# roysubhankar/dwt-domain-adaptation

Measured on NVIDIA H100. Metric: ResNet-50-DWT images/sec fwd+bwd, higher is better.
Workload: dtype f32

## Files before the change

dwt-domain-adaptation_b200/dwt_b200/_native.py:

```python
from __future__ import annotations

import ctypes
import os
import threading

import torch

_HERE = os.path.dirname(os.path.abspath(__file__))
LIB_PATH = os.environ.get("DWT_B200_LIB") or os.path.join(_HERE, "lib", "libdwt_b200.so")

ABI_VERSION = 6
MAX_DOMAINS = 4
MAX_GROUP_SIZE = 64
MODE_TRAIN, MODE_EVAL = 0, 1
EPI_NONE, EPI_AFFINE, EPI_RELU, EPI_RESIDUAL = 0, 1, 2, 4
LAYOUT_NHWC = 0x100
STATUS_NOT_PD, STATUS_BAD_LABEL = 1, 2
KIND_WHITEN, KIND_BN = 0, 1

_c_float_p = ctypes.c_void_p
_PtrArray = ctypes.c_void_p * MAX_DOMAINS


class TailSite(ctypes.Structure):
    _fields_ = [("x", ctypes.c_void_p), ("eps", ctypes.c_float), ("momentum", ctypes.c_float),
                ("update_running", ctypes.c_int), ("running_mean", ctypes.POINTER(ctypes.c_void_p)),
                ("running_cov", ctypes.POINTER(ctypes.c_void_p)), ("gamma", ctypes.c_void_p), ("beta", ctypes.c_void_p),
                ("save_mean", ctypes.c_void_p), ("save_w", ctypes.c_void_p), ("dx", ctypes.c_void_p),
                ("dgamma", ctypes.c_void_p), ("dbeta", ctypes.c_void_p)]

_SIGNATURES = {
    "dwt_abi_version": (ctypes.c_int, []),
    "dwt_last_error": (ctypes.c_char_p, []),
    "dwt_workspace_bytes": (ctypes.c_size_t, [ctypes.c_int64, ctypes.c_int64, ctypes.c_int64, ctypes.c_int, ctypes.c_int]),
    "dwt_whiten_fwd": (ctypes.c_int, [_c_float_p, _c_float_p, ctypes.c_int64, ctypes.c_int64, ctypes.c_int64,
                                      ctypes.c_int, ctypes.c_int, ctypes.c_int, ctypes.c_float, ctypes.c_float,
                                      ctypes.c_int, ctypes.POINTER(ctypes.c_void_p), ctypes.POINTER(ctypes.c_void_p),
                                      _c_float_p, _c_float_p, _c_float_p, ctypes.c_void_p, ctypes.c_int, _c_float_p,
                                      _c_float_p, ctypes.c_void_p, ctypes.c_size_t, ctypes.c_void_p]),
    "dwt_whiten_bwd": (ctypes.c_int, [_c_float_p, _c_float_p, _c_float_p, _c_float_p, ctypes.c_int64, ctypes.c_int64,
                                      ctypes.c_int64, ctypes.c_int, ctypes.c_int, ctypes.c_int, ctypes.c_float,
                                      _c_float_p, _c_float_p, _c_float_p, _c_float_p, ctypes.c_void_p, _c_float_p,
                                      ctypes.c_int, _c_float_p, _c_float_p, ctypes.c_void_p, ctypes.c_size_t,
                                      ctypes.c_void_p]),
    "dwt_bn_fwd": (ctypes.c_int, [_c_float_p, _c_float_p, ctypes.c_int64, ctypes.c_int64, ctypes.c_int64,
                                  ctypes.c_int, ctypes.c_int, ctypes.c_float, ctypes.c_float, ctypes.c_int,
                                  ctypes.POINTER(ctypes.c_void_p), ctypes.POINTER(ctypes.c_void_p), _c_float_p,
                                  _c_float_p, _c_float_p, ctypes.c_void_p, ctypes.c_int, _c_float_p, _c_float_p,
                                  ctypes.c_void_p, ctypes.c_size_t, ctypes.c_void_p]),
    "dwt_bn_bwd": (ctypes.c_int, [_c_float_p, _c_float_p, _c_float_p, _c_float_p, ctypes.c_int64, ctypes.c_int64, ctypes.c_int64,
                                  ctypes.c_int, ctypes.c_int, _c_float_p, _c_float_p, _c_float_p, _c_float_p,
                                  ctypes.c_void_p, _c_float_p, ctypes.c_int, _c_float_p, _c_float_p, ctypes.c_void_p,
                                  ctypes.c_size_t, ctypes.c_void_p]),
    "dwt_tail2_fwd": (ctypes.c_int, [ctypes.c_int, ctypes.POINTER(TailSite), _c_float_p, ctypes.c_void_p, ctypes.c_int64,
                                     ctypes.c_int64, ctypes.c_int64, ctypes.c_int, ctypes.c_int, ctypes.c_void_p,
                                     ctypes.c_size_t, ctypes.c_void_p]),
    "dwt_tail2_bwd": (ctypes.c_int, [ctypes.c_int, ctypes.POINTER(TailSite), _c_float_p, _c_float_p, ctypes.c_void_p,
                                     _c_float_p, ctypes.c_int64, ctypes.c_int64, ctypes.c_int64, ctypes.c_int, ctypes.c_int,
                                     ctypes.c_void_p, ctypes.c_size_t, ctypes.c_void_p]),
    "dwt_mec_fwd_bwd": (ctypes.c_int, [_c_float_p, _c_float_p, ctypes.c_int64, ctypes.c_int64, _c_float_p,
                                       _c_float_p, _c_float_p, ctypes.c_void_p]),
    "dwt_head_loss_fwd_bwd": (ctypes.c_int, [_c_float_p, ctypes.c_void_p, ctypes.c_int64, ctypes.c_int64, ctypes.c_float,
                                             _c_float_p, _c_float_p, ctypes.c_void_p, ctypes.c_void_p]),
    "dwt_augment_pair": (ctypes.c_int, [ctypes.c_void_p, ctypes.c_int64, ctypes.c_int, ctypes.c_int, ctypes.c_int,
                                        ctypes.c_void_p, ctypes.c_void_p, ctypes.c_void_p, _c_float_p,
                                        ctypes.POINTER(ctypes.c_float), ctypes.POINTER(ctypes.c_float), _c_float_p,
                                        _c_float_p, ctypes.c_int, ctypes.c_void_p]),
    "dwt_maxpool_fwd": (ctypes.c_int, [_c_float_p, _c_float_p, ctypes.c_void_p, ctypes.c_int64, ctypes.c_int64, ctypes.c_int64,
                                       ctypes.c_int64, ctypes.c_int, ctypes.c_int, ctypes.c_int, ctypes.c_void_p]),
    "dwt_maxpool_bwd": (ctypes.c_int, [_c_float_p, ctypes.c_void_p, _c_float_p, ctypes.c_int64, ctypes.c_int64, ctypes.c_int64,
                                       ctypes.c_int64, ctypes.c_int, ctypes.c_int, ctypes.c_int, ctypes.c_void_p]),
    "dwt_launch_count": (ctypes.c_int64, []),
    "dwt_profile_begin": (None, []),
    "dwt_profile_end": (ctypes.c_int, [ctypes.c_void_p, ctypes.c_int]),
}


class ProfileEntry(ctypes.Structure):
    _fields_ = [("name", ctypes.c_char * 48), ("launches", ctypes.c_int64), ("ms", ctypes.c_double),
                ("bytes", ctypes.c_double)]


def profile_begin():
    lib().dwt_profile_begin()


def profile_end():
    cap = 1024
    buf = (ProfileEntry * cap)()
    k = lib().dwt_profile_end(ctypes.cast(buf, ctypes.c_void_p), cap)
    return {buf[i].name.decode(): dict(launches=buf[i].launches, ms=buf[i].ms, bytes=buf[i].bytes) for i in range(k)}


def by_family(prof):
    out = {}
    for name, v in prof.items():
        f = out.setdefault(name.split("|")[0], dict(launches=0, ms=0.0, bytes=0.0))
        for k in f:
            f[k] += v[k]
    return out


def launch_count() -> int:
    return int(lib().dwt_launch_count())
EXPORTS = tuple(_SIGNATURES)

_lib = None
_lock = threading.Lock()


class NativeError(RuntimeError):
    pass


def lib() -> ctypes.CDLL:
    global _lib
    if _lib is None:
        with _lock:
            if _lib is None:
                if not os.path.exists(LIB_PATH):
                    raise NativeError(
                        f"{LIB_PATH} is missing: build it with `python {os.path.join(_HERE, 'build.py')}` "
                        "(dwt_b200 has no CPU or PyTorch fallback)")
                handle = ctypes.CDLL(LIB_PATH)
                for name, (res, args) in _SIGNATURES.items():
                    fn = getattr(handle, name)
                    fn.restype, fn.argtypes = res, args
                if handle.dwt_abi_version() != ABI_VERSION:
                    raise NativeError("libdwt_b200.so ABI version mismatch; rebuild it")
                _lib = handle
    return _lib


def channels_last_supported(channels: int, group_size: int) -> bool:
    if group_size not in (1, 2, 4) or channels % 4:
        return False
    c4 = channels // 4
    return c4 & (c4 - 1) == 0


def check(rc: int) -> None:
    if rc != 0:
        raise NativeError(f"libdwt_b200 error {rc}: {lib().dwt_last_error().decode()}")


def ptr(t):
    return None if t is None else ctypes.c_void_p(t.data_ptr())


def ptr_array(tensors):
    arr = _PtrArray()
    for i, t in enumerate(tensors):
        arr[i] = None if t is None else t.data_ptr()
    return ctypes.cast(arr, ctypes.POINTER(ctypes.c_void_p))


def require_cuda(*tensors, any_dtype=False) -> torch.device:
    dev = None
    for t in tensors:
        if t is None:
            continue
        if not t.is_cuda:
            raise NativeError("dwt_b200 runs on CUDA tensors only (no CPU fallback); got a tensor on " + str(t.device))
        if t.dtype != torch.float32 and not any_dtype:
            raise NativeError("dwt_b200 computes in float32; got " + str(t.dtype))
        if dev is None:
            dev = t.device
        elif t.device != dev:
            raise NativeError(f"tensors on different devices: {dev} vs {t.device}")
    return dev


def stream_ptr(device) -> ctypes.c_void_p:
    return ctypes.c_void_p(torch.cuda.current_stream(device).cuda_stream)


_workspaces: dict = {}


def workspace(device, n, c, hw, gs, nd):
    need = lib().dwt_workspace_bytes(n, c, hw, gs, nd)
    if need == 0:
        raise NativeError(f"invalid geometry for workspace: C={c} group_size={gs} domains={nd}")
    key = (device.index, torch.cuda.current_stream(device).cuda_stream)
    buf = _workspaces.get(key)
    if buf is None or buf.numel() < need:
        buf = torch.zeros(max(need, 8 << 20), dtype=torch.uint8, device=device)
        _workspaces[key] = buf
    return buf


def status(device=None) -> int:
    device = torch.device("cuda", torch.cuda.current_device()) if device is None else device
    buf = _workspaces.get((device.index, torch.cuda.current_stream(device).cuda_stream))
    return 0 if buf is None else int(buf[:4].view(torch.int32).item())


def status_all(device=None) -> int:
    device = torch.device("cuda", torch.cuda.current_device()) if device is None else device
    torch.cuda.synchronize(device)
    st = 0
    for (idx, _), buf in _workspaces.items():
        if idx == device.index:
            st |= int(buf[:4].view(torch.int32).item())
    return st


def status_ptr(device):
    return ctypes.c_void_p(workspace(device, 1, 4, 1, 1, 1).data_ptr())


def clear_status(device=None) -> None:
    device = torch.device("cuda", torch.cuda.current_device()) if device is None else device
    buf = _workspaces.get((device.index, torch.cuda.current_stream(device).cuda_stream))
    if buf is not None:
        buf[:4].zero_()


class NotPositiveDefiniteError(torch.linalg.LinAlgError):
    """What the reference's torch.cholesky raises at utils/whitening.py:53, raised late: the kernels never sync the
    host, so the failure is seen at the next poll (raise_on_status) or explicit check_status() call."""


_poll = {"every": 0, "count": 0}


def raise_on_status(every: int = 1) -> None:
    _poll["every"], _poll["count"] = max(0, int(every)), 0


def check_status(device=None) -> None:
    st = status(device)
    if st == 0:
        return
    clear_status(device)
    if st & STATUS_NOT_PD:
        raise NotPositiveDefiniteError(
            "cholesky: a whitening covariance was not positive definite (status word bit 0; the reference raises "
            "from torch.cholesky, utils/whitening.py:53); the affected group's output is NaN and its running-"
            "statistics update was skipped")
    if st & STATUS_BAD_LABEL:
        raise IndexError("head loss: a label was outside [0, num_classes) and is not ignore_index=-100 "
                         "(F.nll_loss asserts here); the row was dropped")
    raise NativeError(f"unknown status bits {st:#x}")


def poll_status(device) -> None:
    if _poll["every"]:
        _poll["count"] += 1
        if _poll["count"] >= _poll["every"]:
            _poll["count"] = 0
            check_status(device)
```

dwt-domain-adaptation_b200/dwt_b200/csrc/api.cu:

```cuda
#include <stdarg.h>
#include <stdio.h>
#include <stdlib.h>

#include <atomic>
#include <mutex>
#include <string>
#include <vector>
#include <string.h>

#include "norm_launch.h"

namespace {

thread_local char g_err[512] = "";

int fail(int code, const char* fmt, ...) {
  va_list ap;
  va_start(ap, fmt);
  vsnprintf(g_err, sizeof(g_err), fmt, ap);
  va_end(ap);
  return code;
}

int check_launch(const char* what) {
  cudaError_t e = cudaPeekAtLastError();
  if (e != cudaSuccess) {
    cudaGetLastError();
    return fail(DWT_E_LAUNCH, "%s: %s", what, cudaGetErrorString(e));
  }
  return DWT_OK;
}

int sm_count() {
  static int n = 0;
  if (n == 0) {
    int dev = 0;
    if (cudaGetDevice(&dev) != cudaSuccess ||
        cudaDeviceGetAttribute(&n, cudaDevAttrMultiProcessorCount, dev) != cudaSuccess || n <= 0)
      n = 132;
  }
  return n;
}

std::atomic<int64_t> g_launches{0};
std::mutex g_prof_mu;
bool g_prof_on = false;
struct ProfRec { char name[48]; cudaEvent_t a, b; double bytes; };
std::vector<ProfRec> g_prof;
std::vector<cudaEvent_t> g_event_pool;

cudaEvent_t take_event() {
  if (!g_event_pool.empty()) { cudaEvent_t e = g_event_pool.back(); g_event_pool.pop_back(); return e; }
  cudaEvent_t e = nullptr;
  cudaEventCreate(&e);
  return e;
}

struct Launch {
  cudaStream_t st; ProfRec rec; bool on;
  Launch(const char* family, const dwt::Geom* gm, double bytes, cudaStream_t s) : st(s), on(false) {
    rec.a = rec.b = nullptr; rec.bytes = bytes;
    if (gm) snprintf(rec.name, sizeof(rec.name), "%s|%d|%d|%d|%d|%d", family, gm->C, gm->HW, gm->GS, gm->D, gm->N);
    else snprintf(rec.name, sizeof(rec.name), "%s", family);
    g_launches.fetch_add(1, std::memory_order_relaxed);
    std::lock_guard<std::mutex> lk(g_prof_mu);
    if (g_prof_on && g_prof.size() < (1u << 18)) {
      on = true; rec.a = take_event(); rec.b = take_event();
      cudaEventRecord(rec.a, st);
    }
  }
  ~Launch() {
    if (!on) return;
    cudaEventRecord(rec.b, st);
    std::lock_guard<std::mutex> lk(g_prof_mu);
    g_prof.push_back(rec);
  }
};

std::once_flag g_tiled_once;
int g_tiled_rc = 0;
int ensure_tiled() {
  std::call_once(g_tiled_once, [] { g_tiled_rc = dwt::tiled_init(); });
  return g_tiled_rc;
}

std::once_flag g_tc_once;
int g_tc_rc = 0;
int ensure_tc() {
  std::call_once(g_tc_once, [] { g_tc_rc = dwt::tc_init(); });
  return g_tc_rc;
}

int tc_chunks(const dwt::Geom& g) {
  const int problems = dwt::tc_superblocks(g) * g.D;
  int n = 2 * sm_count() / problems;
  const int64_t tiles = (int64_t)g.N * ((g.HW + 31) / 32);
  if (n > tiles) n = (int)tiles;
  return n < 1 ? 1 : n;
}

int tc_apply_ctas(const dwt::Geom& g, int per_sm, int tile_px) {
  const int problems = dwt::tc_superblocks(g) * g.D;
  int n = per_sm * sm_count() / problems;
  const int64_t tiles = (int64_t)g.N * ((g.HW + tile_px - 1) / tile_px);
  if (n > tiles) n = (int)tiles;
  return n < 1 ? 1 : n;
}

int env_int(const char* name, int dflt) {
  const char* v = getenv(name);
  return (v && *v) ? atoi(v) : dflt;
}

struct ClPlan { int nred, new_, S, gridy, gz_red, gz_ew; };
ClPlan cl_plan(const dwt::Geom& g, int slots_red, int slots_ew, int unroll_red, int unroll_ew) {
  static const int seq_mb = env_int("DWT_CL_SEQ_MB", 1 << 30);
  const int C4 = g.C / 4, CW = C4 < 256 ? C4 : 256, rpi = 256 / CW, gridy = C4 / CW;
  const long long rows = (long long)g.N * g.HW;
  const double mbytes = 4.0 * (double)g.D * (double)rows * (double)g.C / 1048576.0;
  const bool seq = g.D > 1 && mbytes >= (double)seq_mb;
  ClPlan p;
  p.gridy = gridy;
  p.gz_red = p.gz_ew = seq ? 1 : g.D;
  auto shape = [&](int slots, int unroll, int gz) {
    long long by_work = rows / ((long long)rpi * unroll * 2);
    if (by_work < 1) by_work = 1;
    int cap = slots * sm_count() / (gridy * gz);
    if (cap < 1) cap = 1;
    return (int)(by_work < cap ? by_work : cap);
  };
  p.nred = shape(slots_red, unroll_red, p.gz_red);
  p.new_ = shape(slots_ew, unroll_ew, p.gz_ew);
  p.S = p.nred < 8 ? p.nred : 8;
  return p;
}

inline size_t align_up(size_t v, size_t a) { return (v + a - 1) / a * a; }

enum KernelKind { K_STATS, K_APPLY, K_BWD_REDUCE, K_BWD_APPLY };

int slots_per_sm(KernelKind k, int GS) {
  if (GS > 4) return 2;
  return ((k == K_STATS || k == K_APPLY) && GS < 4) ? 4 : 3;
}

int chunk_cap(int GS, int G, int D) {
  (void)GS;
  const int target = 16 * sm_count();
  int cap = (target + G * D - 1) / (G * D);
  return cap < 1 ? 1 : cap;
}

struct Workspace {
  int* status;
  int* counters;
  int* dom_counter;
  int* dom_counter2;
  float* partial;
  float* save_cov;
  float* coef;
  float* dgb_part;
  float* gram;
  float* shift;
  float* red;
  int* bad;
  size_t bytes;
};

constexpr size_t kMaxGroups = 65536;
constexpr size_t kOffCounters = 256;
constexpr size_t kOffDom1 = kOffCounters + sizeof(int) * DWT_MAX_DOMAINS * kMaxGroups;
constexpr size_t kOffDom2 = kOffDom1 + sizeof(int) * kMaxGroups;
constexpr size_t kOffScratch = kOffDom2 + sizeof(int) * kMaxGroups;

Workspace carve(void* base, int64_t C, int GS, int D, size_t start = kOffScratch) {
  const int G = (int)(C / GS);
  const int cap = chunk_cap(GS, G, D);
  size_t off = start;
  auto take = [&](size_t nbytes) { size_t o = off; off = align_up(off + nbytes, 256); return o; };
  char* b = static_cast<char*>(base);
  Workspace w;
  w.status = reinterpret_cast<int*>(b);
  w.counters = reinterpret_cast<int*>(b + kOffCounters);
  w.dom_counter = reinterpret_cast<int*>(b + kOffDom1);
  w.dom_counter2 = reinterpret_cast<int*>(b + kOffDom2);
  size_t partial_floats = (size_t)D * G * cap * (GS * GS + GS);
  if (GS >= 8 && 64 % GS == 0) {
    const size_t tc = ((size_t)2 * sm_count() + (size_t)((C + 63) / 64) * D) * (64 * 64 + 64);
    if (tc > partial_floats) partial_floats = tc;
  }
  size_t red_floats = 1;
  if (dwt::cl_supports((int)C, GS)) {
    const size_t W = (size_t)dwt::cl_bwd_width((int)C, GS);
    const int C4 = (int)C / 4, gridy = C4 <= 256 ? 1 : C4 / 256;
    const size_t cl = (size_t)D * (3 * sm_count() / gridy + 1) * W;
    if (cl > partial_floats) partial_floats = cl;
    red_floats = (size_t)D * 8 * W;
  }
  w.partial = reinterpret_cast<float*>(b + take(sizeof(float) * partial_floats));
  w.red = reinterpret_cast<float*>(b + take(sizeof(float) * red_floats));
  w.save_cov = reinterpret_cast<float*>(b + take(sizeof(float) * (size_t)D * G * GS * GS));
  w.coef = reinterpret_cast<float*>(b + take(sizeof(float) * (size_t)D * G * dwt::coef_stride(GS)));
  w.dgb_part = reinterpret_cast<float*>(b + take(sizeof(float) * (size_t)D * 2 * C));
  const size_t SBn = (size_t)((C + 63) / 64);
  w.gram = reinterpret_cast<float*>(b + take(sizeof(float) * (size_t)D * SBn * (64 * 64 + 64)));
  w.shift = reinterpret_cast<float*>(b + take(sizeof(float) * (size_t)D * SBn * 64));
  w.bad = reinterpret_cast<int*>(b + take(sizeof(int) * (size_t)D * G));
  w.bytes = off;
  return w;
}

struct Plan {
  dwt::Geom gm;
  dwt::Geom gm_ew;
  int vec;
  int chunks_ew;
  bool small;
};

void shape(dwt::Geom& g, int64_t work_units, KernelKind kind, bool small, int* chunks) {
  const bool reduce = (kind == K_STATS || kind == K_BWD_REDUCE);
  const int slots = slots_per_sm(kind, g.GS) * sm_count();
  const int target = reduce ? slots : 4 * slots;
  g.ppc = 1;
  if (small) {
    while (g.ppc < 8 && (int64_t)((g.G + g.ppc - 1) / g.ppc) * g.D > target) g.ppc <<= 1;
  }
  int n = 1;
  if (g.ppc == 1) {
    n = target / (g.G * g.D);
    const int cap = chunk_cap(g.GS, g.G, g.D);
    if (n > cap) n = cap;
    if (n > work_units) n = (int)work_units;
    if (n < 1) n = 1;
  }
  *chunks = n;
}

int make_plan(Plan& p, KernelKind reduce_kind, KernelKind ew_kind, const void* a0, const void* a1, const void* a2,
              int64_t N, int64_t C, int64_t HW, int GS, int D) {
  if (N <= 0 || C <= 0 || HW <= 0) return fail(DWT_E_INVALID, "empty tensor (N=%lld C=%lld HW=%lld)", (long long)N,
                                               (long long)C, (long long)HW);
  if (GS < 1 || GS > DWT_MAX_GROUP_SIZE) return fail(DWT_E_UNSUPPORTED, "group_size %d outside [1,%d]", GS,
                                                     DWT_MAX_GROUP_SIZE);
  if (C % GS != 0) return fail(DWT_E_INVALID, "channels %lld not divisible by group_size %d", (long long)C, GS);
  if (D < 1 || D > DWT_MAX_DOMAINS) return fail(DWT_E_INVALID, "n_domains %d outside [1,%d]", D, DWT_MAX_DOMAINS);
  if (N * C * HW >= (int64_t)1 << 31 || C / GS > 65535)
    return fail(DWT_E_UNSUPPORTED, "shape too large for 32-bit item indexing");
  dwt::Geom& g = p.gm;
  g.N = (int)N; g.C = (int)C; g.HW = (int)HW; g.GS = GS; g.G = (int)(C / GS); g.D = D;
  g.M = (float)((double)N * (double)HW);
  const uintptr_t bits = (uintptr_t)a0 | (uintptr_t)a1 | (uintptr_t)a2;
  p.vec = (HW % 4 == 0 && bits % 16 == 0) ? 4 : 1;
  p.small = dwt::small_supports(GS);
  int64_t work_units;
  if (p.small) work_units = (N * (HW / p.vec) + dwt::kThreads * 2 - 1) / (dwt::kThreads * 2);
  else work_units = (N * HW + 127) / 128;
  if (work_units < 1) work_units = 1;
  shape(g, work_units, reduce_kind, p.small, &g.nchunks);
  p.gm_ew = g;
  shape(p.gm_ew, work_units, ew_kind, p.small, &p.chunks_ew);
  p.gm_ew.nchunks = g.nchunks;
  return DWT_OK;
}

int check_running(bool need_running, float* const* rmean, float* const* rcov, int D) {
  if (!need_running) return DWT_OK;
  if (!rmean || !rcov) return fail(DWT_E_INVALID, "running buffers required");
  for (int d = 0; d < D; ++d)
    if (!rmean[d] || !rcov[d]) return fail(DWT_E_INVALID, "running buffer of domain %d is null", d);
  return DWT_OK;
}

dwt::FwdFin make_fwd_fin(float a, float b, float momentum, float unbias, int update_running, bool need_running,
                         float* const* rmean, float* const* rcov, float* save_mean, float* save_w, const Workspace& w, int D) {
  dwt::FwdFin fin{};
  fin.a = a; fin.b = b; fin.momentum = momentum; fin.unbias = unbias;
  fin.update_running = update_running;
  fin.save_mean = save_mean; fin.save_w = save_w; fin.save_cov = w.save_cov;
  for (int d = 0; d < D; ++d) { fin.rmean[d] = need_running ? rmean[d] : nullptr; fin.rcov[d] = need_running ? rcov[d] : nullptr; }
  fin.dom_counter = w.dom_counter; fin.status = w.status; fin.bad = w.bad;
  if (need_running && D > 1) {
    bool all_same = true, all_distinct = true;
    for (int d = 1; d < D; ++d) {
      if (rmean[d] != rmean[0] || rcov[d] != rcov[0]) all_same = false;
      for (int e = 0; e < d; ++e)
        if (rmean[d] == rmean[e] || rcov[d] == rcov[e]) all_distinct = false;
    }
    fin.aliased = all_same ? 1 : (all_distinct ? 0 : -1);
  }
  return fin;
}

dwt::BwdFin make_bwd_fin(float a, int mode, int epi, const float* save_mean, const float* save_w, const float* gamma,
                         float* dgamma, float* dbeta, const Workspace& w) {
  dwt::BwdFin fin{};
  fin.a = a; fin.mode = mode; fin.epi = epi;
  fin.save_mean = save_mean; fin.save_w = save_w; fin.gamma = gamma;
  fin.coef = w.coef; fin.dgb_part = w.dgb_part;
  fin.dgamma = (epi & DWT_EPI_AFFINE) ? dgamma : nullptr;
  fin.dbeta = (epi & DWT_EPI_AFFINE) ? dbeta : nullptr;
  fin.dom_counter = w.dom_counter2;
  return fin;
}

int whiten_like_fwd(const float* x, float* y, int64_t N, int64_t C, int64_t HW, int GS, int D, int mode, float a,
                    float b, float momentum, float unbias, int update_running, float* const* rmean,
                    float* const* rcov, const float* gamma, const float* beta, const float* residual,
                    uint8_t* relu_mask, int epi, float* save_mean, float* save_w, void* ws, size_t ws_bytes,
                    cudaStream_t st) {
  const bool nhwc = (mode & DWT_LAYOUT_NHWC) != 0;
  mode &= 0xFF;
  Plan p;
  if (int rc = make_plan(p, K_STATS, K_APPLY, x, y, nullptr, N, C, HW, GS, D)) return rc;
  if (!x || !y || !save_mean || !save_w || !ws) return fail(DWT_E_INVALID, "null pointer argument");
  if (nhwc && !dwt::cl_supports((int)C, GS))
    return fail(DWT_E_UNSUPPORTED, "channels-last layout is built for group_size 1, 2, 4 with C/4 a power of two (C=%lld gs=%d)", (long long)C, GS);
  if (nhwc && (((uintptr_t)x | (uintptr_t)y) % 16 != 0)) return fail(DWT_E_INVALID, "channels-last tensors must be 16-byte aligned");
  if (mode != DWT_MODE_TRAIN && mode != DWT_MODE_EVAL) return fail(DWT_E_INVALID, "bad mode %d", mode);
  if ((epi & DWT_EPI_RELU) && !(epi & DWT_EPI_AFFINE)) return fail(DWT_E_INVALID, "RELU epilogue needs AFFINE");
  if ((epi & DWT_EPI_AFFINE) && (!gamma || !beta)) return fail(DWT_E_INVALID, "AFFINE epilogue needs gamma and beta");
  if ((epi & DWT_EPI_RESIDUAL) && ((epi & 3) != 3 || !residual)) return fail(DWT_E_INVALID, "RESIDUAL epilogue needs AFFINE|RELU and a residual tensor");
  if ((epi & DWT_EPI_RESIDUAL) && (uintptr_t)residual % 16 != 0) return fail(DWT_E_INVALID, "residual must be 16-byte aligned");
  if (relu_mask && !((epi & DWT_EPI_RESIDUAL) && nhwc))
    return fail(DWT_E_UNSUPPORTED, "the ReLU byte map is written by the channels-last RESIDUAL epilogue only");
  if (epi != 0 && !p.small)
    return fail(DWT_E_UNSUPPORTED, "fused gamma/beta/ReLU epilogue is built for group_size 1, 2, 4 (got %d)", GS);
  const bool need_running = (mode == DWT_MODE_EVAL) || update_running;
  if (int rc = check_running(need_running, rmean, rcov, D)) return rc;
  Workspace w = carve(ws, C, GS, D);
  if (w.bytes > ws_bytes) return fail(DWT_E_WORKSPACE, "workspace too small: need %zu bytes, got %zu", w.bytes, ws_bytes);
  if ((uintptr_t)ws % 256 != 0) return fail(DWT_E_WORKSPACE, "workspace must be 256-byte aligned");
  if (!p.small && ensure_tiled() != 0) return fail(DWT_E_LAUNCH, "cudaFuncSetAttribute failed (%d)", g_tiled_rc);

  const dwt::FwdFin fin = make_fwd_fin(a, b, momentum, unbias, mode == DWT_MODE_TRAIN ? update_running : 0, need_running,
                                       rmean, rcov, save_mean, save_w, w, D);

  const double E = 4.0 * (double)D * (double)N * (double)C * (double)HW;
  if (nhwc) {
    const ClPlan cp = cl_plan(p.gm, 3, 3, 8, (epi & DWT_EPI_RESIDUAL) ? 4 : 8);
    if (mode == DWT_MODE_TRAIN) {
      {
        Launch l("cl_stats", &p.gm, E, st);
        dwt::cl_stats(x, p.gm, cp.nred, cp.gz_red, w.partial, w.shift, st);
      }
      if (int rc = check_launch("channels-last statistics kernel")) return rc;
      Launch l("cl_fwd_finalize", &p.gm, 0.0, st);
      dwt::cl_fwd_finalize(w.partial, cp.nred, w.shift, p.gm, fin, st);
    } else {
      Launch l("eval_prep", &p.gm, 0.0, st);
      dwt::small_eval_prep(p.gm, fin, st);
    }
    if (int rc = check_launch("channels-last finalize kernel")) return rc;
    {
      Launch l("cl_apply", &p.gm, ((epi & DWT_EPI_RESIDUAL) ? (relu_mask ? 3.0625 : 3.0) : 2.0) * E, st);
      dwt::cl_apply(x, y, p.gm, cp.new_, cp.gz_ew, epi, save_mean, save_w, gamma, beta, residual, relu_mask, st);
    }
    return check_launch("channels-last apply kernel");
  }
  const bool tc = !p.small && dwt::tc_supports(p.gm, p.vec) && ensure_tc() == 0;
  if (mode == DWT_MODE_TRAIN) {
    Launch l(p.small ? "small_stats" : (tc ? "tc_stats" : "tiled_stats"), &p.gm, E, st);
    if (p.small) dwt::small_stats(x, p.gm, p.vec, fin, w.partial, w.counters, st);
    else if (tc) {
      if (int cr = dwt::tc_stats(x, p.gm, tc_chunks(p.gm), w.shift, w.partial, st))
        return fail(DWT_E_LAUNCH, "cuTensorMapEncodeTiled failed (CUresult %d) x=%p N=%d C=%d HW=%d D=%d", cr, (const void*)x, p.gm.N, p.gm.C, p.gm.HW, p.gm.D);
    } else dwt::tiled_stats(x, p.gm, p.vec, fin, w.partial, w.counters, st);
  } else {
    Launch l("eval_prep", &p.gm, 0.0, st);
    if (p.small) dwt::small_eval_prep(p.gm, fin, st);
    else if (tc) dwt::dense_fwd_factor(nullptr, nullptr, p.gm, fin, st);
    else dwt::tiled_eval_prep(p.gm, fin, st);
  }
  if (tc && mode == DWT_MODE_TRAIN) {
    if (int rc = check_launch("tensor-core statistics kernel")) return rc;
    Launch l("dense_fwd_finalize", &p.gm, 0.0, st);
    dwt::dense_partial_reduce(w.partial, tc_chunks(p.gm), dwt::tc_superblocks(p.gm) * D, w.gram, st);
    dwt::dense_fwd_factor(w.gram, w.shift, p.gm, fin, st);
  }
  if (int rc = check_launch("whitening statistics kernel")) return rc;
  {
    Launch l(p.small ? "small_apply" : (tc ? "tc_apply" : "tiled_apply"), &p.gm, ((epi & DWT_EPI_RESIDUAL) ? 3 : 2) * E, st);
    if (p.small) dwt::small_apply(x, y, p.gm_ew, p.vec, p.chunks_ew, epi, save_mean, save_w, gamma, beta, residual, st);
    else if (tc) {
      if (int cr = dwt::tc_apply(x, y, p.gm, tc_apply_ctas(p.gm, 1, 64), save_mean, save_w, st))
        return fail(DWT_E_LAUNCH, "cuTensorMapEncodeTiled failed (CUresult %d)", cr);
    } else dwt::tiled_apply(x, y, p.gm_ew, p.vec, p.chunks_ew, save_mean, save_w, st);
  }
  return check_launch("whitening apply kernel");
}

int whiten_like_bwd(const float* x, const float* dout, const float* dout2, float* dx, int64_t N, int64_t C, int64_t HW, int GS, int D,
                    int mode, float a, const float* save_mean, const float* save_w, const float* gamma,
                    const float* beta, const uint8_t* relu_mask, float* dresidual, int epi, float* dgamma,
                    float* dbeta, void* ws, size_t ws_bytes, cudaStream_t st) {
  const bool nhwc = (mode & DWT_LAYOUT_NHWC) != 0;
  mode &= 0xFF;
  Plan p;
  if (int rc = make_plan(p, K_BWD_REDUCE, K_BWD_APPLY, x, dout, dx, N, C, HW, GS, D)) return rc;
  if (!x || !dout || !dx || !save_mean || !save_w || !ws) return fail(DWT_E_INVALID, "null pointer argument");
  if (dout2 && (!nhwc || (uintptr_t)dout2 % 16 != 0))
    return fail(nhwc ? DWT_E_INVALID : DWT_E_UNSUPPORTED, "a second gradient addend (dout2) is built for the channels-last "
                "kernels (16-byte aligned tensor); add it to dout otherwise");
  if (nhwc && !dwt::cl_supports((int)C, GS))
    return fail(DWT_E_UNSUPPORTED, "channels-last layout is built for group_size 1, 2, 4 with C/4 a power of two (C=%lld gs=%d)", (long long)C, GS);
  if (nhwc && (((uintptr_t)x | (uintptr_t)dout | (uintptr_t)dx) % 16 != 0)) return fail(DWT_E_INVALID, "channels-last tensors must be 16-byte aligned");
  if (mode != DWT_MODE_TRAIN && mode != DWT_MODE_EVAL) return fail(DWT_E_INVALID, "bad mode %d", mode);
  if ((epi & DWT_EPI_RELU) && !(epi & DWT_EPI_AFFINE)) return fail(DWT_E_INVALID, "RELU epilogue needs AFFINE");
  if ((epi & DWT_EPI_AFFINE) && (!gamma || !beta)) return fail(DWT_E_INVALID, "AFFINE epilogue needs gamma and beta");
  if (epi & DWT_EPI_RESIDUAL) {
    if (!nhwc || !relu_mask || (epi & 3) != 3 || !dresidual)
      return fail(DWT_E_INVALID, "backward of a RESIDUAL forward needs the channels-last layout, AFFINE|RELU, the forward's "
                                 "ReLU byte map and dresidual (or pass dout already masked by (out > 0) with epilogue AFFINE)");
    if ((uintptr_t)dresidual % 16 != 0) return fail(DWT_E_INVALID, "dresidual must be 16-byte aligned");
  } else if (relu_mask || dresidual) {
    return fail(DWT_E_INVALID, "relu_mask / dresidual belong to the RESIDUAL epilogue");
  }
  if ((dgamma == nullptr) != (dbeta == nullptr)) return fail(DWT_E_INVALID, "dgamma and dbeta go together");
  if (epi != 0 && !p.small)
    return fail(DWT_E_UNSUPPORTED, "fused gamma/beta/ReLU epilogue is built for group_size 1, 2, 4 (got %d)", GS);
  Workspace w = carve(ws, C, GS, D);
  if (w.bytes > ws_bytes) return fail(DWT_E_WORKSPACE, "workspace too small: need %zu bytes, got %zu", w.bytes, ws_bytes);
  if ((uintptr_t)ws % 256 != 0) return fail(DWT_E_WORKSPACE, "workspace must be 256-byte aligned");
  if (!p.small && ensure_tiled() != 0) return fail(DWT_E_LAUNCH, "cudaFuncSetAttribute failed (%d)", g_tiled_rc);

  const dwt::BwdFin fin = make_bwd_fin(a, mode, epi, save_mean, save_w, gamma, dgamma, dbeta, w);
  const bool masked = nhwc && (epi & DWT_EPI_RESIDUAL) != 0;

  const bool need_reduce = (mode == DWT_MODE_TRAIN) || (fin.dgamma != nullptr) || masked;
  const double E = 4.0 * (double)D * (double)N * (double)C * (double)HW;
  if (nhwc) {
    const ClPlan cp = cl_plan(p.gm, 2, 2, 4, 4);
    if (need_reduce) {
      {
        Launch l("cl_bwd_reduce", &p.gm, ((masked ? 3.0625 : 2.0) + (dout2 ? 1.0 : 0.0)) * E, st);
        dwt::cl_bwd_reduce(x, dout, dout2, p.gm, cp.nred, cp.gz_red, epi, save_mean, save_w, gamma, beta, relu_mask, dresidual, w.partial, st);
      }
      if (int rc = check_launch("channels-last backward reduction kernel")) return rc;
      Launch l("cl_bwd_finalize", &p.gm, 0.0, st);
      dwt::cl_bwd_finalize(w.partial, cp.nred, p.gm, fin, st);
    } else {
      Launch l("bwd_prep", &p.gm, 0.0, st);
      dwt::small_bwd_prep(p.gm, fin, st);
    }
    if (int rc = check_launch("channels-last backward finalize kernel")) return rc;
    {
      Launch l("cl_bwd_apply", &p.gm, (3.0 + (dout2 && !masked ? 1.0 : 0.0)) * E, st);
      if (masked) dwt::cl_bwd_apply(x, dresidual, nullptr, dx, p.gm, cp.new_, cp.gz_ew, DWT_EPI_AFFINE, w.coef, save_mean, save_w, gamma, beta, st);
      else dwt::cl_bwd_apply(x, dout, dout2, dx, p.gm, cp.new_, cp.gz_ew, epi, w.coef, save_mean, save_w, gamma, beta, st);
    }
    return check_launch("channels-last backward apply kernel");
  }
  const bool tc = !p.small && dwt::tc_supports(p.gm, p.vec) && ensure_tc() == 0;
  if (need_reduce) {
    Launch l(p.small ? "small_bwd_reduce" : (tc ? "tc_bwd_reduce" : "tiled_bwd_reduce"), &p.gm, 2 * E, st);
    if (p.small) dwt::small_bwd_reduce(x, dout, p.gm, p.vec, fin, beta, w.partial, w.counters, st);
    else if (tc) {
      if (int cr = dwt::tc_bwd_reduce(x, dout, p.gm, tc_chunks(p.gm), save_mean, w.partial, st))
        return fail(DWT_E_LAUNCH, "cuTensorMapEncodeTiled failed (CUresult %d) x=%p dout=%p N=%d C=%d HW=%d D=%d", cr, (const void*)x, (const void*)dout, p.gm.N, p.gm.C, p.gm.HW, p.gm.D);
    } else dwt::tiled_bwd_reduce(x, dout, p.gm, p.vec, fin, w.partial, w.counters, st);
  } else {
    Launch l("bwd_prep", &p.gm, 0.0, st);
    if (p.small) dwt::small_bwd_prep(p.gm, fin, st);
    else if (tc) dwt::dense_bwd_coef(nullptr, p.gm, fin, w.shift, st);
    else dwt::tiled_bwd_prep(p.gm, fin, st);
  }
  if (tc && need_reduce) {
    if (int rc = check_launch("tensor-core backward reduction kernel")) return rc;
    Launch l("dense_bwd_finalize", &p.gm, 0.0, st);
    dwt::dense_partial_reduce(w.partial, tc_chunks(p.gm), dwt::tc_superblocks(p.gm) * D, w.gram, st);
    dwt::dense_bwd_coef(w.gram, p.gm, fin, w.shift, st);
  }
  if (int rc = check_launch("whitening backward reduction kernel")) return rc;
  {
    Launch l(p.small ? "small_bwd_apply" : (tc ? "tc_bwd_apply" : "tiled_bwd_apply"), &p.gm, 3 * E, st);
    if (p.small) dwt::small_bwd_apply(x, dout, dx, p.gm_ew, p.vec, p.chunks_ew, epi, w.coef, save_mean, save_w, gamma, beta, st);
    else if (tc) {
      if (int cr = dwt::tc_bwd_apply(x, dout, dx, p.gm, tc_apply_ctas(p.gm, 1, 64), w.coef, save_mean, w.shift, st))
        return fail(DWT_E_LAUNCH, "cuTensorMapEncodeTiled failed (CUresult %d)", cr);
    } else dwt::tiled_bwd_apply(x, dout, dx, p.gm_ew, p.vec, p.chunks_ew, w.coef, st);
  }
  return check_launch("whitening backward apply kernel");
}

struct SiteConst { float a, b, unbias; };
SiteConst site_const(int kind, float eps, int64_t N, int64_t HW) {
  if (kind == DWT_KIND_BN) {
    const double M = (double)N * (double)HW;
    return {1.f, eps, M > 1.0 ? (float)(M / (M - 1.0)) : 1.f};
  }
  return {1.f - eps, eps, 1.f};
}

int tail2_plan(Plan& p, int kind, const dwt_tail_site* s, const void* out, int64_t N, int64_t C, int64_t HW, int GS, int D) {
  if (kind != DWT_KIND_WHITEN && kind != DWT_KIND_BN) return fail(DWT_E_INVALID, "bad kind %d", kind);
  if (kind == DWT_KIND_BN && GS != 1) return fail(DWT_E_INVALID, "batch norm has group_size 1 (got %d)", GS);
  if (!s) return fail(DWT_E_INVALID, "null pointer argument");
  if (int rc = make_plan(p, K_STATS, K_APPLY, s[0].x, s[1].x, out, N, C, HW, GS, D)) return rc;
  if (!dwt::cl_supports((int)C, GS))
    return fail(DWT_E_UNSUPPORTED, "the two-site tail runs on the channels-last kernels: group_size 1, 2, 4 with C/4 a power of two (C=%lld gs=%d)",
                (long long)C, GS);
  for (int k = 0; k < 2; ++k)
    if (!s[k].x || !s[k].gamma || !s[k].beta || !s[k].save_mean || !s[k].save_w || !out) return fail(DWT_E_INVALID, "null pointer argument");
  if ((((uintptr_t)s[0].x | (uintptr_t)s[1].x | (uintptr_t)out) % 16) != 0) return fail(DWT_E_INVALID, "channels-last tensors must be 16-byte aligned");
  return DWT_OK;
}

int tail2_workspace(Workspace (&w)[2], void* ws, size_t ws_bytes, int64_t C, int GS, int D) {
  if (!ws) return fail(DWT_E_INVALID, "null pointer argument");
  w[0] = carve(ws, C, GS, D);
  w[1] = carve(ws, C, GS, D, w[0].bytes);
  if (w[1].bytes > ws_bytes) return fail(DWT_E_WORKSPACE, "workspace too small: need %zu bytes, got %zu", w[1].bytes, ws_bytes);
  if ((uintptr_t)ws % 256 != 0) return fail(DWT_E_WORKSPACE, "workspace must be 256-byte aligned");
  return DWT_OK;
}

int tail2_fwd(int kind, const dwt_tail_site* s, float* y, uint8_t* relu_mask, int64_t N, int64_t C, int64_t HW, int GS, int D,
              void* ws, size_t ws_bytes, cudaStream_t st) {
  Plan p;
  if (int rc = tail2_plan(p, kind, s, y, N, C, HW, GS, D)) return rc;
  if (!relu_mask) return fail(DWT_E_INVALID, "the two-site tail writes the ReLU byte map its backward reads");
  for (int k = 0; k < 2; ++k)
    if (int rc = check_running(s[k].update_running != 0, s[k].running_mean, s[k].running_cov, D)) return rc;
  Workspace w[2];
  if (int rc = tail2_workspace(w, ws, ws_bytes, C, GS, D)) return rc;
  dwt::FwdFin fin[2];
  for (int k = 0; k < 2; ++k) {
    const SiteConst sc = site_const(kind, s[k].eps, N, HW);
    fin[k] = make_fwd_fin(sc.a, sc.b, s[k].momentum, sc.unbias, s[k].update_running, s[k].update_running != 0, s[k].running_mean,
                          s[k].running_cov, s[k].save_mean, s[k].save_w, w[k], D);
  }
  const double E = 4.0 * (double)D * (double)N * (double)C * (double)HW;
  const ClPlan cp = cl_plan(p.gm, 3, 3, 8, 4);
  for (int k = 0; k < 2; ++k) {
    Launch l("cl_stats", &p.gm, E, st);
    dwt::cl_stats(s[k].x, p.gm, cp.nred, cp.gz_red, w[k].partial, w[k].shift, st);
  }
  if (int rc = check_launch("channels-last statistics kernel")) return rc;
  {
    Launch l("cl_tail2_fwd_finalize", &p.gm, 0.0, st);
    dwt::cl_fwd_finalize(w[0].partial, cp.nred, w[0].shift, p.gm, fin[0], st, &fin[1], (size_t)(w[1].partial - w[0].partial),
                         (size_t)(w[1].shift - w[0].shift));
  }
  if (int rc = check_launch("channels-last finalize kernel")) return rc;
  {
    Launch l("cl_tail2_apply", &p.gm, 3.0625 * E, st);
    dwt::cl_tail2_apply(s[0].x, s[1].x, y, p.gm, cp.new_, cp.gz_ew, s[0].save_mean, s[0].save_w, s[0].gamma, s[0].beta,
                        s[1].save_mean, s[1].save_w, s[1].gamma, s[1].beta, relu_mask, st);
  }
  return check_launch("channels-last two-site apply kernel");
}

int tail2_bwd(int kind, const dwt_tail_site* s, const float* dout, const float* dout2, const uint8_t* relu_mask, float* dz,
              int64_t N, int64_t C, int64_t HW, int GS, int D, void* ws, size_t ws_bytes, cudaStream_t st) {
  Plan p;
  if (int rc = tail2_plan(p, kind, s, dz, N, C, HW, GS, D)) return rc;
  if (!dout || !relu_mask || !s[0].dx || !s[1].dx) return fail(DWT_E_INVALID, "null pointer argument");
  if ((((uintptr_t)dout | (uintptr_t)dout2 | (uintptr_t)s[0].dx | (uintptr_t)s[1].dx) % 16) != 0)
    return fail(DWT_E_INVALID, "channels-last tensors must be 16-byte aligned");
  for (int k = 0; k < 2; ++k)
    if ((s[k].dgamma == nullptr) != (s[k].dbeta == nullptr)) return fail(DWT_E_INVALID, "dgamma and dbeta go together");
  Workspace w[2];
  if (int rc = tail2_workspace(w, ws, ws_bytes, C, GS, D)) return rc;
  dwt::BwdFin fin[2];
  for (int k = 0; k < 2; ++k)
    fin[k] = make_bwd_fin(site_const(kind, s[k].eps, N, HW).a, DWT_MODE_TRAIN, k ? DWT_EPI_AFFINE : (DWT_EPI_AFFINE | DWT_EPI_RELU | DWT_EPI_RESIDUAL),
                          s[k].save_mean, s[k].save_w, s[k].gamma, s[k].dgamma, s[k].dbeta, w[k]);
  const double E = 4.0 * (double)D * (double)N * (double)C * (double)HW;
  const ClPlan cp = cl_plan(p.gm, 2, 2, 4, 4);
  {
    Launch l("cl_tail2_bwd_reduce", &p.gm, (4.0625 + (dout2 ? 1.0 : 0.0)) * E, st);
    dwt::cl_tail2_bwd_reduce(s[0].x, s[1].x, dout, dout2, p.gm, cp.nred, cp.gz_red, s[0].save_mean, s[1].save_mean, relu_mask, dz,
                             w[0].partial, (size_t)(w[1].partial - w[0].partial), st);
  }
  if (int rc = check_launch("channels-last two-site backward reduction kernel")) return rc;
  {
    Launch l("cl_tail2_bwd_finalize", &p.gm, 0.0, st);
    dwt::cl_bwd_finalize(w[0].partial, cp.nred, p.gm, fin[0], st, &fin[1], (size_t)(w[1].partial - w[0].partial));
  }
  if (int rc = check_launch("channels-last backward finalize kernel")) return rc;
  {
    Launch l("cl_tail2_bwd_apply", &p.gm, 5.0 * E, st);
    dwt::cl_tail2_bwd_apply(s[0].x, s[1].x, dz, s[0].dx, s[1].dx, p.gm, cp.new_, cp.gz_ew, w[0].coef, w[1].coef, st);
  }
  return check_launch("channels-last two-site backward apply kernel");
}

}

extern "C" {

int dwt_abi_version(void) { return DWT_B200_ABI_VERSION; }

const char* dwt_last_error(void) { return g_err; }

size_t dwt_workspace_bytes(int64_t N, int64_t C, int64_t HW, int group_size, int n_domains) {
  (void)N; (void)HW;
  if (C <= 0 || group_size < 1 || group_size > DWT_MAX_GROUP_SIZE || C % group_size != 0 || n_domains < 1 ||
      n_domains > DWT_MAX_DOMAINS)
    return 0;
  return carve(nullptr, C, group_size, n_domains, carve(nullptr, C, group_size, n_domains).bytes).bytes;
}

int dwt_whiten_fwd(const float* x, float* y, int64_t N, int64_t C, int64_t HW, int group_size, int n_domains,
                   int mode, float eps, float momentum, int update_running, float* const* running_mean,
                   float* const* running_cov, const float* gamma, const float* beta, const float* residual,
                   uint8_t* relu_mask, int epilogue, float* save_mean, float* save_w, void* workspace,
                   size_t workspace_bytes, dwt_stream_t stream) {
  return whiten_like_fwd(x, y, N, C, HW, group_size, n_domains, mode, 1.f - eps, eps, momentum, 1.f, update_running,
                         running_mean, running_cov, gamma, beta, residual, relu_mask, epilogue, save_mean, save_w,
                         workspace, workspace_bytes, (cudaStream_t)stream);
}

int dwt_whiten_bwd(const float* x, const float* dout, const float* dout2, float* dx, int64_t N, int64_t C, int64_t HW, int group_size,
                   int n_domains, int mode, float eps, const float* save_mean, const float* save_w,
                   const float* gamma, const float* beta, const uint8_t* relu_mask, float* dresidual, int epilogue,
                   float* dgamma, float* dbeta, void* workspace, size_t workspace_bytes, dwt_stream_t stream) {
  return whiten_like_bwd(x, dout, dout2, dx, N, C, HW, group_size, n_domains, mode, 1.f - eps, save_mean, save_w, gamma,
                         beta, relu_mask, dresidual, epilogue, dgamma, dbeta, workspace, workspace_bytes,
                         (cudaStream_t)stream);
}

int dwt_bn_fwd(const float* x, float* y, int64_t N, int64_t C, int64_t HW, int n_domains, int mode, float eps,
               float factor, int update_running, float* const* running_mean, float* const* running_var,
               const float* weight, const float* bias, const float* residual, uint8_t* relu_mask, int epilogue,
               float* save_mean, float* save_invstd, void* workspace, size_t workspace_bytes, dwt_stream_t stream) {
  const double M = (double)N * (double)HW;
  const float unbias = M > 1.0 ? (float)(M / (M - 1.0)) : 1.f;
  return whiten_like_fwd(x, y, N, C, HW, 1, n_domains, mode, 1.f, eps, factor, unbias, update_running, running_mean,
                         running_var, weight, bias, residual, relu_mask, epilogue, save_mean, save_invstd, workspace,
                         workspace_bytes, (cudaStream_t)stream);
}

int dwt_bn_bwd(const float* x, const float* dout, const float* dout2, float* dx, int64_t N, int64_t C, int64_t HW, int n_domains,
               int mode, const float* save_mean, const float* save_invstd, const float* weight, const float* bias,
               const uint8_t* relu_mask, float* dresidual, int epilogue, float* dweight, float* dbias, void* workspace,
               size_t workspace_bytes, dwt_stream_t stream) {
  return whiten_like_bwd(x, dout, dout2, dx, N, C, HW, 1, n_domains, mode, 1.f, save_mean, save_invstd, weight, bias,
                         relu_mask, dresidual, epilogue, dweight, dbias, workspace, workspace_bytes,
                         (cudaStream_t)stream);
}

int dwt_tail2_fwd(int kind, const dwt_tail_site* sites, float* y, uint8_t* relu_mask, int64_t N, int64_t C, int64_t HW,
                  int group_size, int n_domains, void* workspace, size_t workspace_bytes, dwt_stream_t stream) {
  return tail2_fwd(kind, sites, y, relu_mask, N, C, HW, group_size, n_domains, workspace, workspace_bytes, (cudaStream_t)stream);
}

int dwt_tail2_bwd(int kind, const dwt_tail_site* sites, const float* dout, const float* dout2, const uint8_t* relu_mask, float* dz,
                  int64_t N, int64_t C, int64_t HW, int group_size, int n_domains, void* workspace, size_t workspace_bytes,
                  dwt_stream_t stream) {
  return tail2_bwd(kind, sites, dout, dout2, relu_mask, dz, N, C, HW, group_size, n_domains, workspace, workspace_bytes,
                   (cudaStream_t)stream);
}

int dwt_mec_fwd_bwd(const float* x, const float* y, int64_t N, int64_t K, float* loss, float* gx, float* gy,
                    dwt_stream_t stream) {
  if (!x || !y || !loss || !gx || !gy) return fail(DWT_E_INVALID, "null pointer argument");
  if (N <= 0 || K <= 0 || N >= (1 << 24) || K >= (1 << 24)) return fail(DWT_E_INVALID, "bad logits shape [%lld,%lld]", (long long)N, (long long)K);
  {
    Launch l("mec", nullptr, 16.0 * (double)N * (double)K, (cudaStream_t)stream);
    dwt::mec_launch(x, y, (int)N, (int)K, loss, gx, gy, (cudaStream_t)stream);
  }
  return check_launch("MEC kernel");
}

int dwt_head_loss_fwd_bwd(const float* logits, const int64_t* labels, int64_t B, int64_t K, float lambda, float* losses,
                          float* grad, int* status, dwt_stream_t stream) {
  if (!logits || !labels || !losses || !grad) return fail(DWT_E_INVALID, "null pointer argument");
  if (B <= 0 || K <= 0 || B >= (1 << 22) || K >= (1 << 24)) return fail(DWT_E_INVALID, "bad logits shape [3*%lld,%lld]", (long long)B, (long long)K);
  {
    Launch l("head_loss", nullptr, 4.0 * 3 * (double)B * (double)K * 2, (cudaStream_t)stream);
    dwt::head_loss_launch(logits, reinterpret_cast<const long long*>(labels), (int)B, (int)K, lambda, losses, grad, status,
                          (cudaStream_t)stream);
  }
  return check_launch("head loss kernel");
}

int dwt_augment_pair(const uint8_t* images, int64_t B, int src_h, int src_w, int crop, const int32_t* crop_plain,
                     const int32_t* crop_aug, const uint8_t* flip, const float* affine, const float* mean,
                     const float* stdv, float* out_plain, float* out_aug, int layout, dwt_stream_t stream) {
  if (!images || !mean || !stdv) return fail(DWT_E_INVALID, "null pointer argument");
  if (!out_plain && !out_aug) return fail(DWT_E_INVALID, "at least one of out_plain / out_aug is needed");
  if (out_plain && !crop_plain) return fail(DWT_E_INVALID, "out_plain needs crop_plain");
  if (out_aug && (!crop_aug || !flip || !affine)) return fail(DWT_E_INVALID, "out_aug needs crop_aug, flip and affine");
  if (B <= 0 || B > 65535 || src_h <= 0 || src_w <= 0 || src_h > 16384 || src_w > 16384)
    return fail(DWT_E_INVALID, "bad image batch [%lld,%d,%d,3]", (long long)B, src_h, src_w);
  if (crop <= 0 || crop > src_h || crop > src_w) return fail(DWT_E_INVALID, "crop %d does not fit %dx%d", crop, src_h, src_w);
  if (layout != 0 && layout != DWT_LAYOUT_NHWC) return fail(DWT_E_INVALID, "layout must be 0 (NCHW) or DWT_LAYOUT_NHWC");
  for (int c = 0; c < 3; ++c)
    if (!(stdv[c] != 0.f)) return fail(DWT_E_INVALID, "std[%d] must be non-zero", c);
  {
    const double px = (double)B * crop * crop;
    Launch l("augment_pair", nullptr, px * 3 * ((out_plain ? 5.0 : 0.0) + (out_aug ? 5.0 : 0.0)), (cudaStream_t)stream);
    dwt::augment_pair_launch(images, (int)B, src_h, src_w, crop, crop_plain, crop_aug, flip, affine, mean, stdv, out_plain,
                             out_aug, layout != 0, (cudaStream_t)stream);
  }
  return check_launch("augmentation kernel");
}

namespace {
int pool_check(int64_t N, int64_t H, int64_t W, int64_t C, int k, int s, int p, int* OH, int* OW) {
  if (N <= 0 || H <= 0 || W <= 0 || C <= 0 || C % 4 != 0) return fail(DWT_E_INVALID, "bad pooling input [%lld,%lld,%lld,%lld] (C must be a multiple of 4)", (long long)N, (long long)H, (long long)W, (long long)C);
  if (k < 1 || k > 15 || s < 1 || p < 0 || 2 * p > k) return fail(DWT_E_INVALID, "bad pooling window k=%d s=%d p=%d (k <= 15, pad <= k/2)", k, s, p);
  if (H + 2 * p < k || W + 2 * p < k) return fail(DWT_E_INVALID, "pooling window larger than the padded image");
  *OH = (int)((H + 2 * p - k) / s + 1);
  *OW = (int)((W + 2 * p - k) / s + 1);
  if (N * H * W * C >= ((int64_t)1 << 40)) return fail(DWT_E_UNSUPPORTED, "tensor too large");
  return DWT_OK;
}
}

int dwt_maxpool_fwd(const float* x, float* y, uint8_t* argmax, int64_t N, int64_t H, int64_t W, int64_t C, int kernel,
                    int stride, int padding, dwt_stream_t stream) {
  int OH = 0, OW = 0;
  if (int rc = pool_check(N, H, W, C, kernel, stride, padding, &OH, &OW)) return rc;
  if (!x || !y || !argmax) return fail(DWT_E_INVALID, "null pointer argument");
  if ((((uintptr_t)x | (uintptr_t)y) % 16) != 0 || (uintptr_t)argmax % 4 != 0) return fail(DWT_E_INVALID, "pooling tensors must be 16-byte aligned");
  {
    const double in = (double)N * H * W * C, out = (double)N * OH * OW * C;
    Launch l("maxpool_fwd", nullptr, 4.0 * (in + out) + out, (cudaStream_t)stream);
    dwt::maxpool_fwd_launch(x, y, argmax, (int)N, (int)H, (int)W, (int)C, OH, OW, kernel, stride, padding, (cudaStream_t)stream);
  }
  return check_launch("max-pool forward kernel");
}

int dwt_maxpool_bwd(const float* dy, const uint8_t* argmax, float* dx, int64_t N, int64_t H, int64_t W, int64_t C, int kernel,
                    int stride, int padding, dwt_stream_t stream) {
  int OH = 0, OW = 0;
  if (int rc = pool_check(N, H, W, C, kernel, stride, padding, &OH, &OW)) return rc;
  if (!dy || !dx || !argmax) return fail(DWT_E_INVALID, "null pointer argument");
  if ((((uintptr_t)dy | (uintptr_t)dx) % 16) != 0 || (uintptr_t)argmax % 4 != 0) return fail(DWT_E_INVALID, "pooling tensors must be 16-byte aligned");
  {
    const double in = (double)N * H * W * C, out = (double)N * OH * OW * C;
    Launch l("maxpool_bwd", nullptr, 4.0 * (in + out) + out, (cudaStream_t)stream);
    dwt::maxpool_bwd_launch(dy, argmax, dx, (int)N, (int)H, (int)W, (int)C, OH, OW, kernel, stride, padding, (cudaStream_t)stream);
  }
  return check_launch("max-pool backward kernel");
}

int64_t dwt_launch_count(void) { return g_launches.load(); }

void dwt_profile_begin(void) {
  std::lock_guard<std::mutex> lk(g_prof_mu);
  for (auto& r : g_prof) { g_event_pool.push_back(r.a); g_event_pool.push_back(r.b); }
  g_prof.clear();
  g_prof_on = true;
}

int dwt_profile_end(dwt_profile_entry* out, int max_entries) {
  std::vector<ProfRec> recs;
  {
    std::lock_guard<std::mutex> lk(g_prof_mu);
    g_prof_on = false;
    recs.swap(g_prof);
  }
  int n = 0;
  for (auto& r : recs) {
    float ms = 0.f;
    if (cudaEventSynchronize(r.b) == cudaSuccess && cudaEventElapsedTime(&ms, r.a, r.b) == cudaSuccess) {
      int k = 0;
      for (; k < n; ++k)
        if (strcmp(out[k].name, r.name) == 0) break;
      if (k == n && n < max_entries) {
        memset(&out[n], 0, sizeof(out[n]));
        strncpy(out[n].name, r.name, sizeof(out[n].name) - 1);
        ++n;
      }
      if (k < n) { out[k].launches += 1; out[k].ms += ms; out[k].bytes += r.bytes; }
    }
    std::lock_guard<std::mutex> lk(g_prof_mu);
    g_event_pool.push_back(r.a); g_event_pool.push_back(r.b);
  }
  return n;
}

}
```

dwt-domain-adaptation_b200/dwt_b200/csrc/norm_cl.cu:

```cuda
#include <stdlib.h>

#include "dwt_common.cuh"
#include "norm_launch.h"
#include "small_algebra.cuh"

namespace dwt {
namespace {

constexpr int kT = 256;

__device__ __forceinline__ void pdl_wait() { asm volatile("griddepcontrol.wait;" ::: "memory"); }
__device__ __forceinline__ void pdl_launch_dependents() { asm volatile("griddepcontrol.launch_dependents;" ::: "memory"); }

template <int GS> struct ClShape {
  static constexpr int NSUB = 4 / GS;
  static constexpr int NM = GS * (GS + 1) / 2;
  static constexpr int FWD1 = GS + NM;
  static constexpr int BWD1 = GS * GS + GS;
  static constexpr int FWD = NSUB * FWD1;
  static constexpr int BWD = NSUB * BWD1;
};

struct ClThread {
  int C4, CW, rpi, col, rsub, q;
  __device__ __forceinline__ ClThread(const Geom& gm) {
    C4 = gm.C >> 2;
    CW = C4 < kT ? C4 : kT;
    rpi = kT / CW;
    col = threadIdx.x % CW;
    rsub = threadIdx.x / CW;
    q = blockIdx.y * CW + col;
  }
};

template <int UNROLL, bool DESC, class F>
__device__ __forceinline__ void sweep_rows(const ClThread& t, unsigned rows, F&& body) {
  const unsigned krows = (unsigned)t.rpi * UNROLL, nch = (rows + krows - 1) / krows;
  for (unsigned i = blockIdx.x; i < nch; i += gridDim.x) body((DESC ? nch - 1 - i : i) * krows + t.rsub);
}
#define CL_FOR_DOMAINS(d, gm, DESC) \
  for (int di_ = blockIdx.z, d = (DESC) ? (gm).D - 1 - di_ : di_; di_ < (gm).D; di_ += gridDim.z, d = (DESC) ? (gm).D - 1 - di_ : di_)

__device__ __forceinline__ float4 ldg4(const float* p) { return __ldg(reinterpret_cast<const float4*>(p)); }

template <int NACC>
__device__ __forceinline__ void column_reduce(const ClThread& t, float (&acc)[NACC], float* sRed) {
  if (t.rpi == 1) return;
#pragma unroll
  for (int i = 0; i < NACC; ++i) sRed[i * kT + threadIdx.x] = acc[i];
  __syncthreads();
  if (t.rsub == 0) {
#pragma unroll
    for (int i = 0; i < NACC; ++i) {
      float s = acc[i];
      for (int r = 1; r < t.rpi; ++r) s += sRed[i * kT + r * t.CW + t.col];
      acc[i] = s;
    }
  }
}

template <int GS>
__global__ void __launch_bounds__(kT, 3) cl_stats_kernel(const float* __restrict__ x, const Geom gm,
                                                         float* __restrict__ partial, float* __restrict__ shift) {
  using S = ClShape<GS>;
  constexpr int UNROLL = 8;
  __shared__ float sRed[kT * S::FWD];
  const ClThread t(gm);
  const unsigned rows = (unsigned)gm.N * gm.HW;
  pdl_launch_dependents();
  CL_FOR_DOMAINS(d, gm, true) {
    const float* xd = x + (size_t)d * rows * gm.C + 4 * t.q;
    float K[4] = {0.f, 0.f, 0.f, 0.f};
    {
      const unsigned np = rows < 8 ? rows : 8;
      for (unsigned r = 0; r < np; ++r) {
        const float4 v = ldg4(xd + (size_t)r * gm.C);
        K[0] += v.x; K[1] += v.y; K[2] += v.z; K[3] += v.w;
      }
#pragma unroll
      for (int c = 0; c < 4; ++c) K[c] /= (float)np;
      if (blockIdx.x == 0 && t.rsub == 0) *reinterpret_cast<float4*>(shift + (size_t)d * gm.C + 4 * t.q) = make_float4(K[0], K[1], K[2], K[3]);
    }
    float acc[S::FWD];
#pragma unroll
    for (int i = 0; i < S::FWD; ++i) acc[i] = 0.f;
    sweep_rows<UNROLL, true>(t, rows, [&](unsigned r) {
      float4 v[UNROLL];
#pragma unroll
      for (int u = 0; u < UNROLL; ++u) {
        const unsigned rr = r + u * t.rpi;
        v[u] = rr < rows ? ldg4(xd + (size_t)rr * gm.C) : make_float4(K[0], K[1], K[2], K[3]);
      }
#pragma unroll
      for (int u = 0; u < UNROLL; ++u) {
        const float e[4] = {v[u].x - K[0], v[u].y - K[1], v[u].z - K[2], v[u].w - K[3]};
#pragma unroll
        for (int s = 0; s < S::NSUB; ++s) {
#pragma unroll
          for (int c = 0; c < GS; ++c) {
            acc[s * S::FWD1 + c] += e[s * GS + c];
#pragma unroll
            for (int j = 0; j <= c; ++j)
              acc[s * S::FWD1 + GS + c * (c + 1) / 2 + j] = fmaf(e[s * GS + c], e[s * GS + j], acc[s * S::FWD1 + GS + c * (c + 1) / 2 + j]);
          }
        }
      }
    });
    column_reduce<S::FWD>(t, acc, sRed);
    if (t.rsub == 0) {
      float* dst = partial + (((size_t)d * gridDim.x + blockIdx.x) * t.C4 + t.q) * S::FWD;
#pragma unroll
      for (int i = 0; i < S::FWD; ++i) dst[i] = acc[i];
    }
    if (gridDim.z == 1) __syncthreads();
  }
}

template <int GS, int PER>
__device__ __forceinline__ int acc_index(int g, int a) {
  constexpr int NSUB = 4 / GS;
  return (g / NSUB) * (NSUB * PER) + (g % NSUB) * PER + a;
}

constexpr int kFinQ = 2;

template <int NACC>
__device__ __forceinline__ void column_row_sum(const float* __restrict__ col, int nrows, int W, float (&a)[NACC]) {
  static_assert(NACC % 2 == 0, "accumulators are read as float2");
#pragma unroll
  for (int i = 0; i < NACC; ++i) a[i] = 0.f;
#pragma unroll 4
  for (int r = threadIdx.x; r < nrows; r += 32) {
    const float2* p = reinterpret_cast<const float2*>(col + (size_t)r * W);
#pragma unroll
    for (int i = 0; i < NACC / 2; ++i) {
      const float2 v = __ldcg(p + i);
      a[2 * i] += v.x; a[2 * i + 1] += v.y;
    }
  }
#pragma unroll
  for (int o = 1; o < 32; o <<= 1)
#pragma unroll
    for (int i = 0; i < NACC; ++i) a[i] += __shfl_xor_sync(0xffffffffu, a[i], o);
}

template <int NSUB, int PER>
__device__ __forceinline__ void take_group(const float (&a)[NSUB * PER], int s, float (&v)[PER]) {
#pragma unroll
  for (int i = 0; i < PER; ++i) {
    v[i] = a[i];
#pragma unroll
    for (int k = 1; k < NSUB; ++k)
      if (s == k) v[i] = a[k * PER + i];
  }
}

template <int GS>
__device__ __forceinline__ void cl_fwd_finalize_site(const float* __restrict__ partial, int nrows, const float* __restrict__ shift,
                                                     const Geom& gm, const FwdFin& fin) {
  using SH = ClShape<GS>;
  constexpr int NST = GS + GS * GS;
  __shared__ float sStat[DWT_MAX_DOMAINS][kFinQ][SH::NSUB][NST + 1];
  __shared__ unsigned char sBad[DWT_MAX_DOMAINS][kFinQ][SH::NSUB];
  const int s = threadIdx.x, ql = threadIdx.y, d = threadIdx.z, q = blockIdx.x * blockDim.y + ql;
  const int W = (gm.C >> 2) * SH::FWD;
  const float invM = 1.f / gm.M;
  const bool lead = s < SH::NSUB;
  const int g = q * SH::NSUB + (lead ? s : 0);
  const bool direct = gm.D == 1 || fin.aliased == 0;
  const int dbuf = direct ? d : 0;
  const bool upd = fin.update_running && lead && (direct || (fin.aliased == 1 && d == 0));
  float rc_old[GS * GS], rm_old[GS];
  if (upd) {
#pragma unroll
    for (int e = 0; e < GS * GS; ++e) rc_old[e] = fin.rcov[dbuf][(size_t)g * GS * GS + e];
#pragma unroll
    for (int e = 0; e < GS; ++e) rm_old[e] = fin.rmean[dbuf][g * GS + e];
  }
  pdl_launch_dependents();
  pdl_wait();
  float a[SH::FWD];
  column_row_sum<SH::FWD>(partial + (size_t)d * nrows * W + (size_t)q * SH::FWD, nrows, W, a);
  if (lead) {
    float v[SH::FWD1];
    take_group<SH::NSUB, SH::FWD1>(a, s, v);
    float mean[GS], cov[GS][GS];
#pragma unroll
    for (int i = 0; i < GS; ++i) mean[i] = shift[(size_t)d * gm.C + g * GS + i] + v[i] * invM;
#pragma unroll
    for (int i = 0; i < GS; ++i)
#pragma unroll
      for (int j = 0; j <= i; ++j) {
        const float c = v[GS + i * (i + 1) / 2 + j] * invM - (v[i] * invM) * (v[j] * invM);
        cov[i][j] = c; cov[j][i] = c;
      }
    const bool bad = factor_thread<GS>(gm, fin, d, g, mean, cov, false);
    if (fin.update_running) {
      if (direct) {
        if (!bad) {
          const float m = fin.momentum, kk = 1.f - fin.momentum;
#pragma unroll
          for (int i = 0; i < GS; ++i) {
            fin.rmean[d][g * GS + i] = m * mean[i] + kk * rm_old[i];
#pragma unroll
            for (int j = 0; j < GS; ++j)
              fin.rcov[d][(size_t)g * GS * GS + i * GS + j] = m * (cov[i][j] * fin.unbias) + kk * rc_old[i * GS + j];
          }
        }
      } else {
        sBad[d][ql][s] = bad ? 1 : 0;
#pragma unroll
        for (int i = 0; i < GS; ++i) {
          sStat[d][ql][s][i] = mean[i];
#pragma unroll
          for (int j = 0; j < GS; ++j) sStat[d][ql][s][GS + i * GS + j] = cov[i][j];
        }
      }
    }
  }
  if (!fin.update_running || direct) return;
  __syncthreads();
  if (!(lead && d == 0)) return;
  if (fin.aliased == 1) {
    const float m = fin.momentum, kk = 1.f - fin.momentum;
    float* rc = fin.rcov[0] + (size_t)g * GS * GS;
    float* rm = fin.rmean[0] + g * GS;
    for (int dd = 0; dd < gm.D; ++dd) {
      if (sBad[dd][ql][s]) continue;
#pragma unroll
      for (int e = 0; e < GS * GS; ++e) rc_old[e] = m * (sStat[dd][ql][s][GS + e] * fin.unbias) + kk * rc_old[e];
#pragma unroll
      for (int e = 0; e < GS; ++e) rm_old[e] = m * sStat[dd][ql][s][e] + kk * rm_old[e];
    }
#pragma unroll
    for (int e = 0; e < GS * GS; ++e) rc[e] = rc_old[e];
#pragma unroll
    for (int e = 0; e < GS; ++e) rm[e] = rm_old[e];
  } else {
    for (int dd = 0; dd < gm.D; ++dd)
      if (!sBad[dd][ql][s]) ema_direct<GS>(gm, fin, dd, g, &sStat[dd][ql][s][0], &sStat[dd][ql][s][GS]);
  }
}

template <int GS>
__global__ void __launch_bounds__(32 * kFinQ * DWT_MAX_DOMAINS) cl_fwd_finalize_kernel(const float* __restrict__ partial, size_t pstride, int nrows,
                                                                                      const float* __restrict__ shift, size_t sstride, const Geom gm,
                                                                                      const __grid_constant__ FwdFin fin, const __grid_constant__ FwdFin fin2) {
  const bool second = blockIdx.y != 0;
  cl_fwd_finalize_site<GS>(partial + (second ? pstride : 0), nrows, shift + (second ? sstride : 0), gm, second ? fin2 : fin);
}

template <int GS, int EPI, bool DS>
__global__ void __launch_bounds__(kT, 3) cl_apply_kernel(const float* __restrict__ x, float* __restrict__ y, const Geom gm,
                                                         const float* __restrict__ save_mean, const float* __restrict__ save_w,
                                                         const float* __restrict__ gamma, const float* __restrict__ beta,
                                                         const float* __restrict__ res, uint8_t* __restrict__ mask,
                                                         const float* __restrict__ save_mean_d, const float* __restrict__ save_w_d,
                                                         const float* __restrict__ gamma_d, const float* __restrict__ beta_d) {
  using S = ClShape<GS>;
  constexpr bool RES = (EPI & DWT_EPI_RESIDUAL) != 0;
  static_assert(!DS || RES, "the two-site tail is a residual epilogue");
  constexpr int UNROLL = DS ? 2 : (RES ? 4 : 8);
  const ClThread t(gm);
  const unsigned rows = (unsigned)gm.N * gm.HW;
  pdl_wait();
  CL_FOR_DOMAINS(d, gm, false) {
    float Wp[S::NSUB][S::NM], bp[S::NSUB][GS], Wd[DS ? S::NSUB : 1][S::NM], bd[DS ? S::NSUB : 1][GS];
#pragma unroll
    for (int s = 0; s < S::NSUB; ++s) {
      const int g = t.q * S::NSUB + s;
      load_forward_map<GS, EPI>(save_w + ((size_t)d * gm.G + g) * GS * GS, save_mean + (size_t)d * gm.C + g * GS,
                                gamma + g * GS, beta + g * GS, Wp[s], bp[s]);
      if constexpr (DS)
        load_forward_map<GS, DWT_EPI_AFFINE>(save_w_d + ((size_t)d * gm.G + g) * GS * GS, save_mean_d + (size_t)d * gm.C + g * GS,
                                             gamma_d + g * GS, beta_d + g * GS, Wd[s], bd[s]);
    }
    const size_t base = (size_t)d * rows * gm.C + 4 * t.q;
    const float* xd = x + base;
    const float* rd = res + base;
    float* yd = y + base;
    uint8_t* md = mask + (size_t)d * rows * t.C4 + t.q;
    sweep_rows<UNROLL, false>(t, rows, [&](unsigned r) {
      float4 v[UNROLL], rs[UNROLL];
#pragma unroll
      for (int u = 0; u < UNROLL; ++u) {
        const unsigned rr = r + u * t.rpi;
        if (rr < rows) {
          v[u] = ldg4(xd + (size_t)rr * gm.C);
          if constexpr (RES) rs[u] = ldg4(rd + (size_t)rr * gm.C);
        }
      }
#pragma unroll
      for (int u = 0; u < UNROLL; ++u) {
        const unsigned rr = r + u * t.rpi;
        if (rr < rows) {
          const float e[4] = {v[u].x, v[u].y, v[u].z, v[u].w};
          float o[4], ra[4] = {0.f, 0.f, 0.f, 0.f};
          if constexpr (RES) { ra[0] = rs[u].x; ra[1] = rs[u].y; ra[2] = rs[u].z; ra[3] = rs[u].w; }
          unsigned bits = 0;
#pragma unroll
          for (int s = 0; s < S::NSUB; ++s) {
            float xi[GS], oi[GS];
            if constexpr (DS) {
              float xdi[GS], odi[GS];
#pragma unroll
              for (int c = 0; c < GS; ++c) xdi[c] = ra[s * GS + c];
              apply_group<GS>(Wd[s], bd[s], xdi, odi);
#pragma unroll
              for (int c = 0; c < GS; ++c) ra[s * GS + c] = odi[c];
            }
#pragma unroll
            for (int c = 0; c < GS; ++c) xi[c] = e[s * GS + c];
            apply_group<GS>(Wp[s], bp[s], xi, oi);
#pragma unroll
            for (int c = 0; c < GS; ++c) {
              const float z = RES ? oi[c] + ra[s * GS + c] : oi[c];
              if constexpr (RES) bits |= (z > 0.f ? 1u : 0u) << (s * GS + c);
              o[s * GS + c] = (EPI & DWT_EPI_RELU) ? fmaxf(z, 0.f) : z;
            }
          }
          *reinterpret_cast<float4*>(yd + (size_t)rr * gm.C) = make_float4(o[0], o[1], o[2], o[3]);
          if constexpr (RES) { if (mask != nullptr) md[(size_t)rr * t.C4] = (uint8_t)bits; }
        }
      }
    });
  }
}

template <int GS>
__device__ __forceinline__ void bwd_accumulate(float* acc, const float (&dz)[GS], const float (&xi)[GS], const float* mu) {
#pragma unroll
  for (int i = 0; i < GS; ++i) {
    acc[GS * GS + i] += dz[i];
#pragma unroll
    for (int j = 0; j < GS; ++j) acc[i * GS + j] = fmaf(dz[i], xi[j] - mu[j], acc[i * GS + j]);
  }
}

template <int GS, int EPI, bool D2, bool DS>
__global__ void __launch_bounds__(kT, 2) cl_bwd_reduce_kernel(const float* __restrict__ x, const float* __restrict__ dout, const float* __restrict__ dout2,
                                                              const Geom gm, const float* __restrict__ save_mean,
                                                              const float* __restrict__ save_w, const float* __restrict__ gamma,
                                                              const float* __restrict__ beta, const uint8_t* __restrict__ mask,
                                                              float* __restrict__ dzout, float* __restrict__ partial,
                                                              const float* __restrict__ xds, const float* __restrict__ save_mean_d,
                                                              size_t pstride) {
  using S = ClShape<GS>;
  constexpr int UNROLL = 4;
  constexpr bool MASK = (EPI & DWT_EPI_RESIDUAL) != 0;
  constexpr bool RELU = (EPI & DWT_EPI_RELU) != 0 && !MASK;
  static_assert(!DS || MASK, "the two-site tail is a residual epilogue");
  constexpr int NS = DS ? 2 : 1;
  __shared__ float sRed[kT * S::BWD];
  const ClThread t(gm);
  const unsigned rows = (unsigned)gm.N * gm.HW;
  pdl_launch_dependents();
  CL_FOR_DOMAINS(d, gm, true) {
    float Wp[S::NSUB][S::NM], bp[S::NSUB][GS], mu[NS][4];
#pragma unroll
    for (int s = 0; s < S::NSUB; ++s) {
      const int g = t.q * S::NSUB + s;
      if constexpr (RELU)
        load_forward_map<GS, EPI>(save_w + ((size_t)d * gm.G + g) * GS * GS, save_mean + (size_t)d * gm.C + g * GS,
                                  gamma + g * GS, beta + g * GS, Wp[s], bp[s]);
    }
#pragma unroll
    for (int k = 0; k < NS; ++k) {
      const float4 m4 = ldg4((k ? save_mean_d : save_mean) + (size_t)d * gm.C + 4 * t.q);
      mu[k][0] = m4.x; mu[k][1] = m4.y; mu[k][2] = m4.z; mu[k][3] = m4.w;
    }
    float acc[NS][S::BWD];
#pragma unroll
    for (int k = 0; k < NS; ++k)
#pragma unroll
      for (int i = 0; i < S::BWD; ++i) acc[k][i] = 0.f;
    const size_t base = (size_t)d * rows * gm.C + 4 * t.q;
    const float* xp[NS];
    xp[0] = x + base;
    if constexpr (DS) xp[NS - 1] = xds + base;
    const float* gd = dout + base;
    const float* gd2 = D2 ? dout2 + base : nullptr;
    float* zd = MASK ? dzout + base : nullptr;
    const uint8_t* md = mask + (size_t)d * rows * t.C4 + t.q;
    constexpr int H = DS ? UNROLL / 2 : UNROLL;
    sweep_rows<UNROLL, true>(t, rows, [&](unsigned r0) {
#pragma unroll
     for (int h = 0; h < UNROLL; h += H) {
      const unsigned r = r0 + h * t.rpi;
      float4 v[NS][H], q[H], q2[D2 ? H : 1];
      unsigned mb[H];
#pragma unroll
      for (int u = 0; u < H; ++u) {
        const unsigned rr = r + u * t.rpi;
        if (rr < rows) {
#pragma unroll
          for (int k = 0; k < NS; ++k) v[k][u] = ldg4(xp[k] + (size_t)rr * gm.C);
          q[u] = ldg4(gd + (size_t)rr * gm.C);
          if constexpr (MASK) mb[u] = __ldg(md + (size_t)rr * t.C4);
          if constexpr (D2) q2[u] = ldg4(gd2 + (size_t)rr * gm.C);
        } else {
#pragma unroll
          for (int k = 0; k < NS; ++k) v[k][u] = make_float4(mu[k][0], mu[k][1], mu[k][2], mu[k][3]);
          q[u] = make_float4(0.f, 0.f, 0.f, 0.f);
          if constexpr (MASK) mb[u] = 0u;
          if constexpr (D2) q2[u] = make_float4(0.f, 0.f, 0.f, 0.f);
        }
      }
      if constexpr (D2) {
#pragma unroll
        for (int u = 0; u < H; ++u) { q[u].x += q2[u].x; q[u].y += q2[u].y; q[u].z += q2[u].z; q[u].w += q2[u].w; }
      }
#pragma unroll
      for (int u = 0; u < H; ++u) {
        const float ge[4] = {q[u].x, q[u].y, q[u].z, q[u].w};
        const float e[4] = {v[0][u].x, v[0][u].y, v[0][u].z, v[0][u].w};
        const float ed[4] = {v[NS - 1][u].x, v[NS - 1][u].y, v[NS - 1][u].z, v[NS - 1][u].w};
        float zm[4];
#pragma unroll
        for (int s = 0; s < S::NSUB; ++s) {
          float xi[GS], dz[GS];
#pragma unroll
          for (int c = 0; c < GS; ++c) { xi[c] = e[s * GS + c]; dz[c] = ge[s * GS + c]; }
          if constexpr (RELU) {
            float oi[GS];
            apply_group<GS>(Wp[s], bp[s], xi, oi);
#pragma unroll
            for (int c = 0; c < GS; ++c) dz[c] = oi[c] > 0.f ? dz[c] : 0.f;
          }
          if constexpr (MASK) {
#pragma unroll
            for (int c = 0; c < GS; ++c) { dz[c] = ((mb[u] >> (s * GS + c)) & 1u) ? dz[c] : 0.f; zm[s * GS + c] = dz[c]; }
          }
          bwd_accumulate<GS>(acc[0] + s * S::BWD1, dz, xi, &mu[0][s * GS]);
          if constexpr (DS) {
#pragma unroll
            for (int c = 0; c < GS; ++c) xi[c] = ed[s * GS + c];
            bwd_accumulate<GS>(acc[NS - 1] + s * S::BWD1, dz, xi, &mu[NS - 1][s * GS]);
          }
        }
        if constexpr (MASK) {
          const unsigned rr = r + u * t.rpi;
          if (rr < rows) *reinterpret_cast<float4*>(zd + (size_t)rr * gm.C) = make_float4(zm[0], zm[1], zm[2], zm[3]);
        }
      }
     }
    });
#pragma unroll
    for (int k = 0; k < NS; ++k) {
      if (k) __syncthreads();
      column_reduce<S::BWD>(t, acc[k], sRed);
      if (t.rsub == 0) {
        float* dst = partial + k * pstride + (((size_t)d * gridDim.x + blockIdx.x) * t.C4 + t.q) * S::BWD;
#pragma unroll
        for (int i = 0; i < S::BWD; ++i) dst[i] = acc[k][i];
      }
    }
    if (gridDim.z == 1) __syncthreads();
  }
}

template <int GS>
__device__ __forceinline__ void cl_bwd_finalize_site(const float* __restrict__ partial, int nrows, const Geom& gm, const BwdFin& fin) {
  using SH = ClShape<GS>;
  const int s = threadIdx.x, d = threadIdx.z, q = blockIdx.x * blockDim.y + threadIdx.y;
  const int W = (gm.C >> 2) * SH::BWD;
  pdl_launch_dependents();
  pdl_wait();
  float a[SH::BWD];
  column_row_sum<SH::BWD>(partial + (size_t)d * nrows * W + (size_t)q * SH::BWD, nrows, W, a);
  if (s < SH::NSUB) {
    float v[SH::BWD1], R[GS][GS], sdz[GS];
    take_group<SH::NSUB, SH::BWD1>(a, s, v);
#pragma unroll
    for (int i = 0; i < SH::BWD1; ++i) {
      if (i < GS * GS) R[i / GS][i % GS] = v[i]; else sdz[i - GS * GS] = v[i];
    }
    bwd_finalize_thread<GS>(gm, fin, d, q * SH::NSUB + s, R, sdz, false);
  }
  if (!((fin.epi & DWT_EPI_AFFINE) && fin.dgamma != nullptr)) return;
  __syncthreads();
  if (d == 0 && s < 4) {
    const int ch = 4 * q + s;
    float sg = 0.f, sb = 0.f;
    for (int dd = 0; dd < gm.D; ++dd) {
      sg += fin.dgb_part[((size_t)dd * 2 + 0) * gm.C + ch];
      sb += fin.dgb_part[((size_t)dd * 2 + 1) * gm.C + ch];
    }
    fin.dgamma[ch] = sg;
    fin.dbeta[ch] = sb;
  }
}

template <int GS>
__global__ void __launch_bounds__(32 * kFinQ * DWT_MAX_DOMAINS) cl_bwd_finalize_kernel(const float* __restrict__ partial, size_t pstride, int nrows,
                                                                                      const Geom gm, const __grid_constant__ BwdFin fin,
                                                                                      const __grid_constant__ BwdFin fin2) {
  const bool second = blockIdx.y != 0;
  cl_bwd_finalize_site<GS>(partial + (second ? pstride : 0), nrows, gm, second ? fin2 : fin);
}

template <int GS>
struct BwdCoef {
  float A1[GS * (GS + 1) / 2], Bm[GS * (GS + 1) / 2], cv[GS];
  __device__ __forceinline__ void load(const float* cf) {
#pragma unroll
    for (int i = 0; i < GS; ++i) {
      cv[i] = __ldg(cf + 2 * GS * GS + i);
#pragma unroll
      for (int j = 0; j <= i; ++j) {
        A1[i * (i + 1) / 2 + j] = __ldg(cf + j * GS + i);
        Bm[i * (i + 1) / 2 + j] = __ldg(cf + GS * GS + i * GS + j);
      }
    }
  }
  __device__ __forceinline__ void apply(const float (&dz)[GS], const float (&xi)[GS], float* o) const {
#pragma unroll
    for (int i = 0; i < GS; ++i) {
      float a = cv[i];
#pragma unroll
      for (int j = i; j < GS; ++j) a = fmaf(A1[j * (j + 1) / 2 + i], dz[j], a);
#pragma unroll
      for (int j = 0; j < GS; ++j) {
        const int hi = i > j ? i : j, lo = i > j ? j : i;
        a = fmaf(Bm[hi * (hi + 1) / 2 + lo], xi[j], a);
      }
      o[i] = a;
    }
  }
};

template <int GS, int EPI, bool D2, bool DS>
__global__ void __launch_bounds__(kT, 2) cl_bwd_apply_kernel(const float* __restrict__ x, const float* __restrict__ dout, const float* __restrict__ dout2,
                                                             float* __restrict__ dx, const Geom gm, const float* __restrict__ coef,
                                                             const float* __restrict__ save_mean, const float* __restrict__ save_w,
                                                             const float* __restrict__ gamma, const float* __restrict__ beta,
                                                             const float* __restrict__ xds, float* __restrict__ dxds,
                                                             const float* __restrict__ coef_d) {
  using S = ClShape<GS>;
  constexpr int UNROLL = 4;
  constexpr bool RELU = (EPI & DWT_EPI_RELU) != 0;
  static_assert((EPI & DWT_EPI_RESIDUAL) == 0, "the residual tail's apply runs with EPI = AFFINE on dz");
  static_assert(!DS || (!D2 && !RELU), "the two-site tail's apply reads dz");
  constexpr int NS = DS ? 2 : 1;
  const ClThread t(gm);
  const unsigned rows = (unsigned)gm.N * gm.HW;
  pdl_wait();
  CL_FOR_DOMAINS(d, gm, false) {
    float Wp[S::NSUB][S::NM], bp[S::NSUB][GS];
    BwdCoef<GS> cf[NS][S::NSUB];
#pragma unroll
    for (int s = 0; s < S::NSUB; ++s) {
      const int g = t.q * S::NSUB + s;
      if constexpr (RELU)
        load_forward_map<GS, EPI>(save_w + ((size_t)d * gm.G + g) * GS * GS, save_mean + (size_t)d * gm.C + g * GS,
                                  gamma + g * GS, beta + g * GS, Wp[s], bp[s]);
#pragma unroll
      for (int k = 0; k < NS; ++k) cf[k][s].load((k ? coef_d : coef) + ((size_t)d * gm.G + g) * coef_stride(GS));
    }
    const size_t base = (size_t)d * rows * gm.C + 4 * t.q;
    const float* xp[NS];
    float* op[NS];
    xp[0] = x + base; op[0] = dx + base;
    if constexpr (DS) { xp[NS - 1] = xds + base; op[NS - 1] = dxds + base; }
    const float* gd = dout + base;
    const float* gd2 = D2 ? dout2 + base : nullptr;
    sweep_rows<UNROLL, false>(t, rows, [&](unsigned r) {
      float4 v[NS][UNROLL], q[UNROLL], q2[D2 ? UNROLL : 1];
#pragma unroll
      for (int u = 0; u < UNROLL; ++u) {
        const unsigned rr = r + u * t.rpi;
        if (rr < rows) {
#pragma unroll
          for (int k = 0; k < NS; ++k) v[k][u] = ldg4(xp[k] + (size_t)rr * gm.C);
          q[u] = ldg4(gd + (size_t)rr * gm.C);
          if constexpr (D2) q2[u] = ldg4(gd2 + (size_t)rr * gm.C);
        }
      }
      if constexpr (D2) {
#pragma unroll
        for (int u = 0; u < UNROLL; ++u)
          if (r + u * t.rpi < rows) { q[u].x += q2[u].x; q[u].y += q2[u].y; q[u].z += q2[u].z; q[u].w += q2[u].w; }
      }
#pragma unroll
      for (int u = 0; u < UNROLL; ++u) {
        const unsigned rr = r + u * t.rpi;
        if (rr < rows) {
          const float ge[4] = {q[u].x, q[u].y, q[u].z, q[u].w};
#pragma unroll
          for (int k = 0; k < NS; ++k) {
            const float e[4] = {v[k][u].x, v[k][u].y, v[k][u].z, v[k][u].w};
            float o[4];
#pragma unroll
            for (int s = 0; s < S::NSUB; ++s) {
              float xi[GS], dz[GS];
#pragma unroll
              for (int c = 0; c < GS; ++c) { xi[c] = e[s * GS + c]; dz[c] = ge[s * GS + c]; }
              if constexpr (RELU) {
                float oi[GS];
                apply_group<GS>(Wp[s], bp[s], xi, oi);
#pragma unroll
                for (int c = 0; c < GS; ++c) dz[c] = oi[c] > 0.f ? dz[c] : 0.f;
              }
              cf[k][s].apply(dz, xi, o + s * GS);
            }
            *reinterpret_cast<float4*>(op[k] + (size_t)rr * gm.C) = make_float4(o[0], o[1], o[2], o[3]);
          }
        }
      }
    });
  }
}

#define CL_GS(GS_, ...)                                  \
  switch (GS_) {                                         \
    case 1: { constexpr int kGS = 1; __VA_ARGS__; break; } \
    case 2: { constexpr int kGS = 2; __VA_ARGS__; break; } \
    case 4: { constexpr int kGS = 4; __VA_ARGS__; break; } \
    default: break;                                      \
  }
#define CL_EPI(E_, ...)                                                   \
  if ((E_) == 3) { constexpr int kEPI = 3; __VA_ARGS__; }                 \
  else if ((E_) == 1) { constexpr int kEPI = 1; __VA_ARGS__; }            \
  else { constexpr int kEPI = 0; __VA_ARGS__; }
#define CL_EPI_BWD(E_, ...)                                               \
  if ((E_) == 7) { constexpr int kEPI = 7; __VA_ARGS__; }                 \
  else CL_EPI(E_, __VA_ARGS__)
#define CL_D2(P_, ...)                                                    \
  if (P_) { constexpr bool kD2 = true; __VA_ARGS__; }                     \
  else { constexpr bool kD2 = false; __VA_ARGS__; }

inline bool use_pdl() {
  static const bool on = [] { const char* v = getenv("DWT_PDL"); return v != nullptr && v[0] == '1'; }();
  return on;
}

template <class... KArgs, class... Args>
inline void launch_k(void (*kernel)(KArgs...), dim3 grid, dim3 block, cudaStream_t st, bool pdl, Args... args) {
  cudaLaunchConfig_t cfg = {};
  cfg.gridDim = grid; cfg.blockDim = block; cfg.dynamicSmemBytes = 0; cfg.stream = st;
  cudaLaunchAttribute attr[1];
  attr[0].id = cudaLaunchAttributeProgrammaticStreamSerialization;
  attr[0].val.programmaticStreamSerializationAllowed = 1;
  cfg.attrs = attr; cfg.numAttrs = pdl ? 1 : 0;
  cudaLaunchKernelEx(&cfg, kernel, KArgs(args)...);
}

inline dim3 cl_grid(const Geom& gm, int nctas, int gz) {
  const int C4 = gm.C / 4, CW = C4 < kT ? C4 : kT;
  return dim3(nctas, C4 / CW, gz);
}

}

bool cl_supports(int C, int GS) {
  if (!(GS == 1 || GS == 2 || GS == 4) || C % 4 != 0) return false;
  const int c4 = C / 4;
  return (c4 & (c4 - 1)) == 0 && c4 <= 16384;
}
int cl_fwd_width(int C, int GS) { return (C / 4) * (4 / GS) * (GS + GS * (GS + 1) / 2); }
int cl_bwd_width(int C, int GS) { return (C / 4) * (4 / GS) * (GS * GS + GS); }


void cl_stats(const float* x, const Geom& gm, int nctas, int gz, float* partial, float* shift, cudaStream_t st) {
  CL_GS(gm.GS, (cl_stats_kernel<kGS><<<cl_grid(gm, nctas, gz), kT, 0, st>>>(x, gm, partial, shift)));
}
inline dim3 fin_block(const Geom& gm) { const int c4 = gm.C / 4; return dim3(32, c4 < kFinQ ? c4 : kFinQ, gm.D); }
void cl_fwd_finalize(const float* partial, int nrows, const float* shift, const Geom& gm, const FwdFin& fin, cudaStream_t st,
                     const FwdFin* fin2, size_t pstride, size_t sstride) {
  const dim3 b = fin_block(gm), g((gm.C / 4) / b.y, fin2 ? 2 : 1);
  CL_GS(gm.GS, (launch_k(cl_fwd_finalize_kernel<kGS>, g, b, st, use_pdl(), partial, pstride, nrows, shift, sstride, gm, fin, fin2 ? *fin2 : fin)));
}
void cl_apply(const float* x, float* y, const Geom& gm, int nctas, int gz, int epi, const float* mean, const float* w,
              const float* gamma, const float* beta, const float* residual, uint8_t* mask, cudaStream_t st) {
  const float* nul = nullptr;
  if (epi == 7) {
    CL_GS(gm.GS, (launch_k(cl_apply_kernel<kGS, 7, false>, cl_grid(gm, nctas, gz), dim3(kT), st, use_pdl(), x, y, gm, mean, w, gamma, beta, residual, mask,
                           nul, nul, nul, nul)));
    return;
  }
  CL_GS(gm.GS, CL_EPI(epi, (launch_k(cl_apply_kernel<kGS, kEPI, false>, cl_grid(gm, nctas, gz), dim3(kT), st, use_pdl(), x, y, gm, mean, w, gamma, beta,
                                     nul, (uint8_t*)nullptr, nul, nul, nul, nul))));
}
void cl_tail2_apply(const float* x, const float* xd, float* y, const Geom& gm, int nctas, int gz, const float* mean, const float* w,
                    const float* gamma, const float* beta, const float* mean_d, const float* w_d, const float* gamma_d,
                    const float* beta_d, uint8_t* mask, cudaStream_t st) {
  CL_GS(gm.GS, (launch_k(cl_apply_kernel<kGS, 7, true>, cl_grid(gm, nctas, gz), dim3(kT), st, use_pdl(), x, y, gm, mean, w, gamma, beta, xd, mask,
                         mean_d, w_d, gamma_d, beta_d)));
}
void cl_bwd_reduce(const float* x, const float* dout, const float* dout2, const Geom& gm, int nctas, int gz, int epi, const float* mean, const float* w,
                   const float* gamma, const float* beta, const uint8_t* mask, float* dz, float* partial, cudaStream_t st) {
  const float* nul = nullptr;
  CL_GS(gm.GS, CL_D2(dout2, CL_EPI_BWD(epi, (cl_bwd_reduce_kernel<kGS, kEPI, kD2, false><<<cl_grid(gm, nctas, gz), kT, 0, st>>>(
                                                x, dout, dout2, gm, mean, w, gamma, beta, mask, dz, partial, nul, nul, 0)))));
}
void cl_tail2_bwd_reduce(const float* x, const float* xd, const float* dout, const float* dout2, const Geom& gm, int nctas, int gz,
                         const float* mean, const float* mean_d, const uint8_t* mask, float* dz, float* partial, size_t pstride,
                         cudaStream_t st) {
  const float* nul = nullptr;
  CL_GS(gm.GS, CL_D2(dout2, (cl_bwd_reduce_kernel<kGS, 7, kD2, true><<<cl_grid(gm, nctas, gz), kT, 0, st>>>(
                                x, dout, dout2, gm, mean, nul, nul, nul, mask, dz, partial, xd, mean_d, pstride))));
}
void cl_bwd_finalize(const float* partial, int nrows, const Geom& gm, const BwdFin& fin, cudaStream_t st, const BwdFin* fin2, size_t pstride) {
  const dim3 b = fin_block(gm), g((gm.C / 4) / b.y, fin2 ? 2 : 1);
  CL_GS(gm.GS, (launch_k(cl_bwd_finalize_kernel<kGS>, g, b, st, use_pdl(), partial, pstride, nrows, gm, fin, fin2 ? *fin2 : fin)));
}
void cl_bwd_apply(const float* x, const float* dout, const float* dout2, float* dx, const Geom& gm, int nctas, int gz, int epi, const float* coef,
                  const float* mean, const float* w, const float* gamma, const float* beta, cudaStream_t st) {
  const float* nul = nullptr;
  CL_GS(gm.GS, CL_D2(dout2, CL_EPI(epi, (launch_k(cl_bwd_apply_kernel<kGS, kEPI, kD2, false>, cl_grid(gm, nctas, gz), dim3(kT), st, use_pdl(), x, dout,
                                                  dout2, dx, gm, coef, mean, w, gamma, beta, nul, (float*)nullptr, nul)))));
}
void cl_tail2_bwd_apply(const float* x, const float* xd, const float* dz, float* dx, float* dxd, const Geom& gm, int nctas, int gz,
                        const float* coef, const float* coef_d, cudaStream_t st) {
  const float* nul = nullptr;
  CL_GS(gm.GS, (launch_k(cl_bwd_apply_kernel<kGS, 1, false, true>, cl_grid(gm, nctas, gz), dim3(kT), st, use_pdl(), x, dz, nul, dx, gm, coef,
                         nul, nul, nul, nul, xd, dxd, coef_d)));
}

}
```

dwt-domain-adaptation_b200/dwt_b200/csrc/norm_launch.h:

```cpp
#pragma once
#include <stdint.h>

#include "dwt_common.cuh"

namespace dwt {

inline void bind_context() {
  thread_local bool bound = false;
  if (!bound) { cudaFree(nullptr); bound = true; }
}

bool small_supports(int GS);
void small_stats(const float* x, const Geom& gm, int vec, const FwdFin& fin, float* partial, int* counters,
                 cudaStream_t st);
void small_eval_prep(const Geom& gm, const FwdFin& fin, cudaStream_t st);
void small_apply(const float* x, float* y, const Geom& gm, int vec, int chunks, int epi, const float* mean,
                 const float* w, const float* gamma, const float* beta, const float* residual, cudaStream_t st);
void small_bwd_reduce(const float* x, const float* dout, const Geom& gm, int vec, const BwdFin& fin,
                      const float* beta, float* partial, int* counters, cudaStream_t st);
void small_bwd_prep(const Geom& gm, const BwdFin& fin, cudaStream_t st);
void small_bwd_apply(const float* x, const float* dout, float* dx, const Geom& gm, int vec, int chunks, int epi,
                     const float* coef, const float* mean, const float* w, const float* gamma, const float* beta,
                     cudaStream_t st);

int tiled_smem_bytes(int GS);
int tiled_init();
void tiled_stats(const float* x, const Geom& gm, int vec, const FwdFin& fin, float* partial, int* counters,
                 cudaStream_t st);
void tiled_eval_prep(const Geom& gm, const FwdFin& fin, cudaStream_t st);
void tiled_apply(const float* x, float* y, const Geom& gm, int vec, int chunks, const float* mean, const float* w,
                 cudaStream_t st);
void tiled_bwd_reduce(const float* x, const float* dout, const Geom& gm, int vec, const BwdFin& fin, float* partial,
                      int* counters, cudaStream_t st);
void tiled_bwd_prep(const Geom& gm, const BwdFin& fin, cudaStream_t st);
void tiled_bwd_apply(const float* x, const float* dout, float* dx, const Geom& gm, int vec, int chunks,
                     const float* coef, cudaStream_t st);

int tc_init();
bool tc_supports(const Geom& gm, int vec);
int tc_superblocks(const Geom& gm);
int tc_stats(const float* x, const Geom& gm, int nchunks, float* shift, float* partial, cudaStream_t st);
int tc_bwd_reduce(const float* x, const float* dout, const Geom& gm, int nchunks, const float* save_mean,
                  float* partial, cudaStream_t st);

int dense_init();
void dense_partial_reduce(const float* partial, int nchunks, int problems, float* gram, cudaStream_t st);
void dense_fwd_factor(const float* gram, const float* shift, const Geom& gm, const FwdFin& fin, cudaStream_t st);
void dense_bwd_coef(const float* rgram, const Geom& gm, const BwdFin& fin, float* dybar, cudaStream_t st);

int tc_apply_init();
int tc_apply(const float* x, float* y, const Geom& gm, int nctas, const float* save_mean, const float* save_w,
             cudaStream_t st);
int tc_bwd_apply(const float* x, const float* dout, float* dx, const Geom& gm, int nctas, const float* coef,
                 const float* save_mean, const float* dybar, cudaStream_t st);

bool cl_supports(int C, int GS);
int cl_fwd_width(int C, int GS);
int cl_bwd_width(int C, int GS);
void cl_stats(const float* x, const Geom& gm, int nctas, int gz, float* partial, float* shift, cudaStream_t st);
void cl_fwd_finalize(const float* partial, int nrows, const float* shift, const Geom& gm, const FwdFin& fin, cudaStream_t st,
                     const FwdFin* fin2 = nullptr, size_t pstride = 0, size_t sstride = 0);
void cl_apply(const float* x, float* y, const Geom& gm, int nctas, int gz, int epi, const float* mean, const float* w,
              const float* gamma, const float* beta, const float* residual, uint8_t* mask, cudaStream_t st);
void cl_bwd_reduce(const float* x, const float* dout, const float* dout2, const Geom& gm, int nctas, int gz, int epi, const float* mean, const float* w,
                   const float* gamma, const float* beta, const uint8_t* mask, float* dz, float* partial, cudaStream_t st);
void cl_bwd_finalize(const float* partial, int nrows, const Geom& gm, const BwdFin& fin, cudaStream_t st,
                     const BwdFin* fin2 = nullptr, size_t pstride = 0);
void cl_bwd_apply(const float* x, const float* dout, const float* dout2, float* dx, const Geom& gm, int nctas, int gz, int epi, const float* coef,
                  const float* mean, const float* w, const float* gamma, const float* beta, cudaStream_t st);
void cl_tail2_apply(const float* x, const float* xd, float* y, const Geom& gm, int nctas, int gz, const float* mean, const float* w,
                    const float* gamma, const float* beta, const float* mean_d, const float* w_d, const float* gamma_d,
                    const float* beta_d, uint8_t* mask, cudaStream_t st);
void cl_tail2_bwd_reduce(const float* x, const float* xd, const float* dout, const float* dout2, const Geom& gm, int nctas, int gz,
                         const float* mean, const float* mean_d, const uint8_t* mask, float* dz, float* partial, size_t pstride,
                         cudaStream_t st);
void cl_tail2_bwd_apply(const float* x, const float* xd, const float* dz, float* dx, float* dxd, const Geom& gm, int nctas, int gz,
                        const float* coef, const float* coef_d, cudaStream_t st);

void maxpool_fwd_launch(const float* x, float* y, uint8_t* idx, int N, int H, int W, int C, int OH, int OW, int k, int s, int p,
                        cudaStream_t st);
void maxpool_bwd_launch(const float* dy, const uint8_t* idx, float* dx, int N, int H, int W, int C, int OH, int OW, int k, int s,
                        int p, cudaStream_t st);

void augment_pair_launch(const uint8_t* images, int B, int SH, int SW, int CR, const int* crop_plain, const int* crop_aug,
                         const uint8_t* flip, const float* affine, const float* mean, const float* stdv,
                         float* out_plain, float* out_aug, int nhwc, cudaStream_t st);
void head_loss_launch(const float* logits, const long long* labels, int B, int K, float lambda, float* losses,
                      float* grad, int* status, cudaStream_t st);
void mec_launch(const float* x, const float* y, int N, int K, float* loss, float* gx, float* gy, cudaStream_t st);

}
```

dwt-domain-adaptation_b200/dwt_b200/csrc/pool.cu:

```cuda
#include "dwt_common.cuh"
#include "norm_launch.h"

namespace dwt {
namespace {

struct PoolGeom {
  int N, H, W, C4, OH, OW, k, s, p, c4shift;
};

template <int K, int S, int P>
__device__ __forceinline__ PoolGeom fixed(PoolGeom g) {
  if constexpr (K > 0) { g.k = K; g.s = S; g.p = P; }
  return g;
}

__device__ __forceinline__ bool takes(float v, float best) { return (v > best) || (v != v); }

template <int K, int S, int P, bool POW2>
__global__ void __launch_bounds__(256) maxpool_fwd_kernel(const float* __restrict__ x, float* __restrict__ y,
                                                          uint8_t* __restrict__ idx, const PoolGeom g0) {
  const PoolGeom g = fixed<K, S, P>(g0);
  const int n = blockIdx.x / g.OH, oh = blockIdx.x - n * g.OH;
  const int h0 = oh * g.s - g.p;
  const float4* xn = reinterpret_cast<const float4*>(x) + (size_t)n * g.H * g.W * g.C4;
  const size_t obase = ((size_t)n * g.OH + oh) * g.OW * g.C4;
  for (int t = threadIdx.x; t < g.OW * g.C4; t += blockDim.x) {
    const int ow = POW2 ? (t >> g.c4shift) : t / g.C4, c4 = t - ow * g.C4;
    const int w0 = ow * g.s - g.p;
    float best[4] = {-INFINITY, -INFINITY, -INFINITY, -INFINITY};
    unsigned bi[4] = {0u, 0u, 0u, 0u};
#pragma unroll
    for (int kh = 0; kh < g.k; ++kh) {
      const int h = h0 + kh;
      if (h < 0 || h >= g.H) continue;
      const float4* xr = xn + (size_t)h * g.W * g.C4 + c4;
#pragma unroll
      for (int kw = 0; kw < g.k; ++kw) {
        const int w = w0 + kw;
        if (w < 0 || w >= g.W) continue;
        const float4 v = __ldg(xr + (size_t)w * g.C4);
        const float e[4] = {v.x, v.y, v.z, v.w};
        const unsigned code = (unsigned)(kh * g.k + kw);
#pragma unroll
        for (int c = 0; c < 4; ++c)
          if (takes(e[c], best[c])) { best[c] = e[c]; bi[c] = code; }
      }
    }
    reinterpret_cast<float4*>(y)[obase + t] = make_float4(best[0], best[1], best[2], best[3]);
    reinterpret_cast<uint32_t*>(idx)[obase + t] = bi[0] | (bi[1] << 8) | (bi[2] << 16) | (bi[3] << 24);
  }
}

template <int K, int S, int P, bool POW2>
__global__ void __launch_bounds__(256) maxpool_bwd_kernel(const float* __restrict__ dy, const uint8_t* __restrict__ idx,
                                                          float* __restrict__ dx, const PoolGeom g0) {
  const PoolGeom g = fixed<K, S, P>(g0);
  const int n = blockIdx.x / g.H, h = blockIdx.x - n * g.H;
  int oh0 = h + g.p - g.k + 1;
  oh0 = oh0 <= 0 ? 0 : (oh0 + g.s - 1) / g.s;
  int oh1 = (h + g.p) / g.s;
  if (oh1 > g.OH - 1) oh1 = g.OH - 1;
  const float4* dyn = reinterpret_cast<const float4*>(dy) + (size_t)n * g.OH * g.OW * g.C4;
  const uint32_t* ixn = reinterpret_cast<const uint32_t*>(idx) + (size_t)n * g.OH * g.OW * g.C4;
  float4* dxr = reinterpret_cast<float4*>(dx) + ((size_t)n * g.H + h) * g.W * g.C4;
  for (int t = threadIdx.x; t < g.W * g.C4; t += blockDim.x) {
    const int w = POW2 ? (t >> g.c4shift) : t / g.C4, c4 = t - w * g.C4;
    int ow0 = w + g.p - g.k + 1;
    ow0 = ow0 <= 0 ? 0 : (ow0 + g.s - 1) / g.s;
    int ow1 = (w + g.p) / g.s;
    if (ow1 > g.OW - 1) ow1 = g.OW - 1;
    float acc[4] = {0.f, 0.f, 0.f, 0.f};
    for (int oh = oh0; oh <= oh1; ++oh) {
      const unsigned kh = (unsigned)(h - (oh * g.s - g.p));
      for (int ow = ow0; ow <= ow1; ++ow) {
        const unsigned code = kh * g.k + (unsigned)(w - (ow * g.s - g.p));
        const size_t o = ((size_t)oh * g.OW + ow) * g.C4 + c4;
        const uint32_t m = __ldg(ixn + o);
        const bool h0 = (m & 0xFFu) == code, h1 = ((m >> 8) & 0xFFu) == code, h2 = ((m >> 16) & 0xFFu) == code, h3 = (m >> 24) == code;
        if (h0 || h1 || h2 || h3) {
          const float4 gq = __ldg(dyn + o);
          if (h0) acc[0] += gq.x;
          if (h1) acc[1] += gq.y;
          if (h2) acc[2] += gq.z;
          if (h3) acc[3] += gq.w;
        }
      }
    }
    dxr[t] = make_float4(acc[0], acc[1], acc[2], acc[3]);
  }
}

__global__ void __launch_bounds__(256) maxpool_fwd_3s2_kernel(const float* __restrict__ x, float* __restrict__ y,
                                                              uint8_t* __restrict__ idx, const PoolGeom g) {
  const int OH2 = g.OH >> 1, OW2 = g.OW >> 1;
  const int n = blockIdx.y / OH2, a = blockIdx.y - n * OH2;
  const int i = blockIdx.x * blockDim.x + threadIdx.x;
  if (i >= OW2 * g.C4) return;
  const int b = i >> g.c4shift, c4 = i & (g.C4 - 1);
  const float4* xn = reinterpret_cast<const float4*>(x) + (size_t)n * g.H * g.W * g.C4 + c4;
  float best[2][2][4];
  unsigned bi[2][2][4];
#pragma unroll
  for (int oa = 0; oa < 2; ++oa)
#pragma unroll
    for (int ob = 0; ob < 2; ++ob)
#pragma unroll
      for (int c = 0; c < 4; ++c) { best[oa][ob][c] = -INFINITY; bi[oa][ob][c] = 0u; }
  const int h0 = 4 * a - 1, w0 = 4 * b - 1;
#pragma unroll
  for (int r = 0; r < 5; ++r) {
    const int h = h0 + r;
    if (h < 0 || h >= g.H) continue;
    float4 row[5];
    bool in[5];
#pragma unroll
    for (int cc = 0; cc < 5; ++cc) {
      const int w = w0 + cc;
      in[cc] = w >= 0 && w < g.W;
      row[cc] = in[cc] ? __ldg(xn + ((size_t)h * g.W + w) * g.C4) : make_float4(0.f, 0.f, 0.f, 0.f);
    }
#pragma unroll
    for (int oa = 0; oa < 2; ++oa) {
      const int kh = r - 2 * oa;
      if (kh < 0 || kh > 2) continue;
#pragma unroll
      for (int ob = 0; ob < 2; ++ob)
#pragma unroll
        for (int kw = 0; kw < 3; ++kw) {
          const int cc = 2 * ob + kw;
          if (!in[cc]) continue;
          const float e[4] = {row[cc].x, row[cc].y, row[cc].z, row[cc].w};
          const unsigned code = (unsigned)(kh * 3 + kw);
#pragma unroll
          for (int c = 0; c < 4; ++c)
            if (takes(e[c], best[oa][ob][c])) { best[oa][ob][c] = e[c]; bi[oa][ob][c] = code; }
        }
    }
  }
#pragma unroll
  for (int oa = 0; oa < 2; ++oa)
#pragma unroll
    for (int ob = 0; ob < 2; ++ob) {
      const size_t o = (((size_t)n * g.OH + 2 * a + oa) * g.OW + 2 * b + ob) * g.C4 + c4;
      reinterpret_cast<float4*>(y)[o] = make_float4(best[oa][ob][0], best[oa][ob][1], best[oa][ob][2], best[oa][ob][3]);
      reinterpret_cast<uint32_t*>(idx)[o] = bi[oa][ob][0] | (bi[oa][ob][1] << 8) | (bi[oa][ob][2] << 16) | (bi[oa][ob][3] << 24);
    }
}

__device__ __forceinline__ void take(float4& acc, const float4& gq, uint32_t m, unsigned code) {
  if ((m & 0xFFu) == code) acc.x += gq.x;
  if (((m >> 8) & 0xFFu) == code) acc.y += gq.y;
  if (((m >> 16) & 0xFFu) == code) acc.z += gq.z;
  if ((m >> 24) == code) acc.w += gq.w;
}

__global__ void __launch_bounds__(256) maxpool_bwd_3s2_kernel(const float* __restrict__ dy, const uint8_t* __restrict__ idx,
                                                              float* __restrict__ dx, const PoolGeom g) {
  const int H2 = g.H >> 1, W2 = g.W >> 1;
  const int n = blockIdx.y / H2, k = blockIdx.y - n * H2;
  const int i = blockIdx.x * blockDim.x + threadIdx.x;
  if (i >= W2 * g.C4) return;
  const int j = i >> g.c4shift, c4 = i & (g.C4 - 1);
  const float4* dyn = reinterpret_cast<const float4*>(dy) + (size_t)n * g.OH * g.OW * g.C4;
  const uint32_t* ixn = reinterpret_cast<const uint32_t*>(idx) + (size_t)n * g.OH * g.OW * g.C4;
  uint32_t m[2][2];
  float4 gq[2][2];
#pragma unroll
  for (int a = 0; a < 2; ++a)
#pragma unroll
    for (int b = 0; b < 2; ++b) {
      const bool ok = (k + a < g.OH) && (j + b < g.OW);
      const size_t o = ((size_t)(k + a) * g.OW + (j + b)) * g.C4 + c4;
      m[a][b] = ok ? __ldg(ixn + o) : 0xFFFFFFFFu;
      gq[a][b] = ok ? __ldg(dyn + o) : make_float4(0.f, 0.f, 0.f, 0.f);
    }
  float4 o00 = make_float4(0.f, 0.f, 0.f, 0.f), o01 = o00, o10 = o00, o11 = o00;
  take(o00, gq[0][0], m[0][0], 4u);
  take(o01, gq[0][0], m[0][0], 5u); take(o01, gq[0][1], m[0][1], 3u);
  take(o10, gq[0][0], m[0][0], 7u); take(o10, gq[1][0], m[1][0], 1u);
  take(o11, gq[0][0], m[0][0], 8u); take(o11, gq[0][1], m[0][1], 6u); take(o11, gq[1][0], m[1][0], 2u); take(o11, gq[1][1], m[1][1], 0u);
  float4* r0 = reinterpret_cast<float4*>(dx) + (((size_t)n * g.H + 2 * k) * g.W + 2 * j) * g.C4 + c4;
  float4* r1 = r0 + (size_t)g.W * g.C4;
  r0[0] = o00; r0[g.C4] = o01;
  r1[0] = o10; r1[g.C4] = o11;
}

}

namespace {
int pow2_shift(int v) {
  int sh = 0;
  while ((1 << sh) < v) ++sh;
  return (1 << sh) == v ? sh : -1;
}
}

void maxpool_fwd_launch(const float* x, float* y, uint8_t* idx, int N, int H, int W, int C, int OH, int OW, int k, int s, int p,
                        cudaStream_t st) {
  const int sh = pow2_shift(C / 4);
  const PoolGeom g{N, H, W, C / 4, OH, OW, k, s, p, sh < 0 ? 0 : sh};
  if (k == 3 && s == 2 && p == 1 && sh >= 0 && H % 4 == 0 && W % 4 == 0 && (long long)N * (OH / 2) <= 65535) {
    const int items = (OW / 2) * (C / 4), threads = items >= 256 ? 256 : ((items + 31) / 32) * 32;
    maxpool_fwd_3s2_kernel<<<dim3((items + threads - 1) / threads, N * (OH / 2)), threads, 0, st>>>(x, y, idx, g);
  } else if (k == 3 && s == 2 && p == 1 && sh >= 0) maxpool_fwd_kernel<3, 2, 1, true><<<N * OH, 256, 0, st>>>(x, y, idx, g);
  else maxpool_fwd_kernel<0, 0, 0, false><<<N * OH, 256, 0, st>>>(x, y, idx, g);
}

void maxpool_bwd_launch(const float* dy, const uint8_t* idx, float* dx, int N, int H, int W, int C, int OH, int OW, int k, int s,
                        int p, cudaStream_t st) {
  const int sh = pow2_shift(C / 4);
  const PoolGeom g{N, H, W, C / 4, OH, OW, k, s, p, sh < 0 ? 0 : sh};
  if (k == 3 && s == 2 && p == 1 && sh >= 0 && H % 2 == 0 && W % 2 == 0 && (long long)N * (H / 2) <= 65535) {
    const int items = (W / 2) * (C / 4), threads = items >= 256 ? 256 : ((items + 31) / 32) * 32;
    maxpool_bwd_3s2_kernel<<<dim3((items + threads - 1) / threads, N * (H / 2)), threads, 0, st>>>(dy, idx, dx, g);
  } else if (k == 3 && s == 2 && p == 1 && sh >= 0) maxpool_bwd_kernel<3, 2, 1, true><<<N * H, 256, 0, st>>>(dy, idx, dx, g);
  else maxpool_bwd_kernel<0, 0, 0, false><<<N * H, 256, 0, st>>>(dy, idx, dx, g);
}

}
```

dwt-domain-adaptation_b200/dwt_b200/functional.py:

```python
from __future__ import annotations

import torch

from . import _native as nv


def _dense(x: torch.Tensor, group_size: int):
    n, c = x.shape[0], x.shape[1]
    hw = 1
    for s in x.shape[2:]:
        hw *= s
    nhwc = (x.dim() == 4 and not x.is_contiguous() and x.is_contiguous(memory_format=torch.channels_last)
            and nv.channels_last_supported(c, group_size))
    if not nhwc and not x.is_contiguous():
        x = x.contiguous()
    return x, n, c, hw, nhwc


def _check_param(name, t, numel):
    if t is None:
        return
    if t.numel() != numel:
        raise ValueError(f"{name} has {t.numel()} elements, expected {numel}")
    if not t.is_contiguous():
        raise ValueError(f"{name} must be contiguous (it is written / read through a raw pointer)")


class _NormFunction(torch.autograd.Function):

    @staticmethod
    def forward(ctx, x, gamma, beta, residual, kind, group_size, n_domains, mode, eps, momentum, update_running,
                running, relu):
        lib = nv.lib()
        gs = group_size if kind == "whiten" else 1
        x, n_all, c, hw, nhwc = _dense(x, gs)
        layout = nv.LAYOUT_NHWC if nhwc else 0
        if n_all % n_domains != 0:
            raise ValueError(f"batch of {n_all} does not split into {n_domains} domains")
        n = n_all // n_domains
        dev = nv.require_cuda(x, gamma, beta, residual, *[t for pair in running for t in pair])
        for d, (rm_t, rv_t) in enumerate(running):
            _check_param(f"running mean of domain {d}", rm_t, c)
            _check_param(f"running second moment of domain {d}", rv_t, c * gs)
        _check_param("gamma / weight", gamma, c)
        _check_param("beta / bias", beta, c)
        epi = nv.EPI_NONE
        if residual is not None:
            if gamma is None or not relu or residual.shape != x.shape:
                raise ValueError("a fused residual needs gamma/beta, relu=True and a tensor shaped like x")
            residual = residual.contiguous(memory_format=torch.channels_last) if nhwc else residual.contiguous()
        if gamma is not None:
            epi = nv.EPI_AFFINE | (nv.EPI_RELU if relu else 0) | (nv.EPI_RESIDUAL if residual is not None else 0)
            gamma_c, beta_c = gamma.detach().reshape(-1).contiguous(), beta.detach().reshape(-1).contiguous()
        else:
            gamma_c = beta_c = None
        y = torch.empty_like(x)
        mask = torch.empty(x.numel() // 4, dtype=torch.uint8, device=dev) if (residual is not None and nhwc) else None
        save_mean = torch.empty(n_domains, c, dtype=torch.float32, device=dev)
        save_w = torch.empty(n_domains, c // gs, gs, gs, dtype=torch.float32, device=dev)
        ws = nv.workspace(dev, n, c, hw, gs, n_domains)
        need_running = (mode == nv.MODE_EVAL) or update_running
        rm = nv.ptr_array([p[0] for p in running]) if need_running else None
        rv = nv.ptr_array([p[1] for p in running]) if need_running else None
        with torch.cuda.device(dev):
            if kind == "whiten":
                rc = lib.dwt_whiten_fwd(nv.ptr(x), nv.ptr(y), n, c, hw, gs, n_domains, mode | layout, eps, momentum,
                                        int(update_running), rm, rv, nv.ptr(gamma_c), nv.ptr(beta_c), nv.ptr(residual),
                                        nv.ptr(mask), epi, nv.ptr(save_mean), nv.ptr(save_w), nv.ptr(ws), ws.numel(),
                                        nv.stream_ptr(dev))
            else:
                rc = lib.dwt_bn_fwd(nv.ptr(x), nv.ptr(y), n, c, hw, n_domains, mode | layout, eps, momentum,
                                    int(update_running), rm, rv, nv.ptr(gamma_c), nv.ptr(beta_c), nv.ptr(residual),
                                    nv.ptr(mask), epi, nv.ptr(save_mean), nv.ptr(save_w), nv.ptr(ws), ws.numel(),
                                    nv.stream_ptr(dev))
        nv.check(rc)
        nv.poll_status(dev)
        if update_running and mode == nv.MODE_TRAIN:
            seen = set()
            for pair in running:
                for buf in pair:
                    if buf is not None and id(buf) not in seen:
                        seen.add(id(buf))
                        torch.autograd.graph.increment_version(buf)
        ctx.residual_mode = None
        if mask is not None:
            ctx.save_for_backward(x, save_mean, save_w, gamma_c, beta_c, mask)
            ctx.residual_mode = "mask"
        elif residual is not None:
            ctx.save_for_backward(x, save_mean, save_w, gamma_c, beta_c, y)
            epi = nv.EPI_AFFINE
            ctx.residual_mode = "aten"
        else:
            ctx.save_for_backward(x, save_mean, save_w, gamma_c, beta_c)
        ctx.cfg = (kind, gs, n_domains, mode | layout, eps, epi, n, c, hw, None if gamma is None else gamma.shape)
        return y

    @staticmethod
    def backward(ctx, dout):
        lib = nv.lib()
        mask = None
        if ctx.residual_mode == "mask":
            x, save_mean, save_w, gamma_c, beta_c, mask = ctx.saved_tensors
        elif ctx.residual_mode == "aten":
            x, save_mean, save_w, gamma_c, beta_c, out = ctx.saved_tensors
            extra = ctx.__dict__.pop("_dwt_extra_grad", None)
            if extra is not None:
                dout = dout + extra
            dout = torch.ops.aten.threshold_backward(dout, out, 0)
        else:
            x, save_mean, save_w, gamma_c, beta_c = ctx.saved_tensors
        kind, gs, n_domains, mode, eps, epi, n, c, hw, gshape = ctx.cfg
        dout2 = ctx.__dict__.pop("_dwt_extra_grad", None)
        if dout2 is not None and not ((mode & nv.LAYOUT_NHWC) and dout2.shape == dout.shape and dout2.dtype == torch.float32
                                      and dout2.is_contiguous(memory_format=torch.channels_last)):
            dout, dout2 = dout + dout2, None
        dout = dout.contiguous(memory_format=torch.channels_last) if (mode & nv.LAYOUT_NHWC) else dout.contiguous()
        dev = nv.require_cuda(dout)
        dx = torch.empty_like(x)
        want_affine = gamma_c is not None and (ctx.needs_input_grad[1] or ctx.needs_input_grad[2])
        d_res = None
        if ctx.residual_mode == "mask":
            d_res = torch.empty_like(x)
        elif ctx.residual_mode == "aten" and ctx.needs_input_grad[3]:
            d_res = dout
        dgamma = torch.empty(c, dtype=torch.float32, device=dev) if want_affine else None
        dbeta = torch.empty(c, dtype=torch.float32, device=dev) if want_affine else None
        ws = nv.workspace(dev, n, c, hw, gs, n_domains)
        with torch.cuda.device(dev):
            if kind == "whiten":
                rc = lib.dwt_whiten_bwd(nv.ptr(x), nv.ptr(dout), nv.ptr(dout2), nv.ptr(dx), n, c, hw, gs, n_domains, mode, eps,
                                        nv.ptr(save_mean), nv.ptr(save_w), nv.ptr(gamma_c), nv.ptr(beta_c), nv.ptr(mask),
                                        nv.ptr(d_res) if mask is not None else None, epi,
                                        nv.ptr(dgamma), nv.ptr(dbeta), nv.ptr(ws), ws.numel(), nv.stream_ptr(dev))
            else:
                rc = lib.dwt_bn_bwd(nv.ptr(x), nv.ptr(dout), nv.ptr(dout2), nv.ptr(dx), n, c, hw, n_domains, mode,
                                    nv.ptr(save_mean), nv.ptr(save_w), nv.ptr(gamma_c), nv.ptr(beta_c), nv.ptr(mask),
                                    nv.ptr(d_res) if mask is not None else None, epi,
                                    nv.ptr(dgamma), nv.ptr(dbeta), nv.ptr(ws), ws.numel(), nv.stream_ptr(dev))
        nv.check(rc)
        if want_affine:
            dgamma, dbeta = dgamma.view(gshape), dbeta.view(gshape)
        return (dx, dgamma, dbeta, d_res if ctx.needs_input_grad[3] else None) + (None,) * 9


class _TailPairFunction(torch.autograd.Function):

    @staticmethod
    def forward(ctx, x, xd, gamma, beta, gamma_d, beta_d, kind, group_size, n_domains, sites):
        lib = nv.lib()
        gs = group_size if kind == "whiten" else 1
        if not (x.dim() == 4 and x.shape == xd.shape and _dense(x, gs)[4] and _dense(xd, gs)[4]):
            raise ValueError("the two-site tail takes two channels-last tensors of one shape with a channels-last build")
        if x.shape[0] % n_domains != 0:
            raise ValueError(f"batch of {x.shape[0]} does not split into {n_domains} domains")
        n_all, c = x.shape[0], x.shape[1]
        hw = x.shape[2] * x.shape[3]
        n = n_all // n_domains
        dev = nv.require_cuda(x, xd, gamma, beta, gamma_d, beta_d, *[t for run, *_ in sites for pair in run for t in pair])
        params = [(gamma, beta), (gamma_d, beta_d)]
        c_sites = (nv.TailSite * 2)()
        keep = []
        saved = []
        for k, (inp, (g, b), (running, eps, momentum, update)) in enumerate(zip((x, xd), params, sites)):
            for d, (rm_t, rv_t) in enumerate(running):
                _check_param(f"running mean of domain {d}", rm_t, c)
                _check_param(f"running second moment of domain {d}", rv_t, c * gs)
            _check_param("gamma / weight", g, c)
            _check_param("beta / bias", b, c)
            g_c, b_c = g.detach().reshape(-1).contiguous(), b.detach().reshape(-1).contiguous()
            save_mean = torch.empty(n_domains, c, dtype=torch.float32, device=dev)
            save_w = torch.empty(n_domains, c // gs, gs, gs, dtype=torch.float32, device=dev)
            rm = nv.ptr_array([pr[0] for pr in running]) if update else None
            rv = nv.ptr_array([pr[1] for pr in running]) if update else None
            c_sites[k] = nv.TailSite(inp.data_ptr(), eps, momentum, int(update), rm, rv, g_c.data_ptr(), b_c.data_ptr(),
                                     save_mean.data_ptr(), save_w.data_ptr(), None, None, None)
            keep += [g_c, b_c, rm, rv]
            saved += [save_mean, save_w, g_c]
        y = torch.empty_like(x)
        mask = torch.empty(x.numel() // 4, dtype=torch.uint8, device=dev)
        ws = nv.workspace(dev, n, c, hw, gs, n_domains)
        nv_kind = nv.KIND_WHITEN if kind == "whiten" else nv.KIND_BN
        with torch.cuda.device(dev):
            rc = lib.dwt_tail2_fwd(nv_kind, c_sites, nv.ptr(y), nv.ptr(mask), n, c, hw, gs, n_domains, nv.ptr(ws), ws.numel(),
                                   nv.stream_ptr(dev))
        nv.check(rc)
        nv.poll_status(dev)
        seen = set()
        for running, _, _, update in sites:
            for buf in (t for pair in running for t in pair) if update else ():
                if id(buf) not in seen:
                    seen.add(id(buf))
                    torch.autograd.graph.increment_version(buf)
        ctx.save_for_backward(x, xd, mask, *saved)
        ctx.cfg = (nv_kind, gs, n_domains, n, c, hw, [s[1] for s in sites], gamma.shape, gamma_d.shape)
        return y

    @staticmethod
    def backward(ctx, dout):
        lib = nv.lib()
        x, xd, mask, mean0, w0, g0, mean1, w1, g1 = ctx.saved_tensors
        nv_kind, gs, n_domains, n, c, hw, eps, gshape, gshape_d = ctx.cfg
        dout2 = ctx.__dict__.pop("_dwt_extra_grad", None)
        if dout2 is not None and not (dout2.shape == dout.shape and dout2.dtype == torch.float32
                                      and dout2.is_contiguous(memory_format=torch.channels_last)):
            dout, dout2 = dout + dout2, None
        dout = dout.contiguous(memory_format=torch.channels_last)
        dev = nv.require_cuda(dout)
        dz = torch.empty_like(x)
        dx, dxd = torch.empty_like(x), torch.empty_like(xd)
        grads = [torch.empty(2, c, dtype=torch.float32, device=dev) for _ in range(2)]
        c_sites = (nv.TailSite * 2)()
        for k, (inp, mean, w, g, d_in, gr) in enumerate(zip((x, xd), (mean0, mean1), (w0, w1), (g0, g1), (dx, dxd), grads)):
            c_sites[k] = nv.TailSite(inp.data_ptr(), eps[k], 0.0, 0, None, None, g.data_ptr(), g.data_ptr(), mean.data_ptr(),
                                     w.data_ptr(), d_in.data_ptr(), gr[0].data_ptr(), gr[1].data_ptr())
        ws = nv.workspace(dev, n, c, hw, gs, n_domains)
        with torch.cuda.device(dev):
            rc = lib.dwt_tail2_bwd(nv_kind, c_sites, nv.ptr(dout), nv.ptr(dout2), nv.ptr(mask), nv.ptr(dz), n, c, hw, gs, n_domains,
                                   nv.ptr(ws), ws.numel(), nv.stream_ptr(dev))
        nv.check(rc)
        return (dx, dxd, grads[0][0].view(gshape), grads[0][1].view(gshape), grads[1][0].view(gshape_d),
                grads[1][1].view(gshape_d)) + (None,) * 4


def tail_pair(x, xd, gamma, beta, gamma_d, beta_d, *, kind, group_size, n_domains, sites):
    return _TailPairFunction.apply(x, xd, gamma, beta, gamma_d, beta_d, kind, group_size, n_domains,
                                   [(r, float(e), float(m), bool(u)) for r, e, m, u in sites])


class _ForkForSum(torch.autograd.Function):

    @staticmethod
    def forward(ctx, y):
        ctx.producer = y.grad_fn
        return y.view_as(y), y.view_as(y)

    @staticmethod
    def backward(ctx, ga, gb):
        producer, ctx.producer = ctx.producer, None
        if ga is None or gb is None:
            return ga if gb is None else gb
        if producer is None or "_dwt_extra_grad" in producer.__dict__:
            return ga + gb
        producer.__dict__["_dwt_extra_grad"] = gb
        return ga


def fork_for_sum(y):
    fn = getattr(y, "grad_fn", None)
    if not torch.is_grad_enabled() or fn is None or not isinstance(fn, (_NormFunction._backward_cls, _TailPairFunction._backward_cls)):
        return y, y
    return _ForkForSum.apply(y)


def norm(x, gamma, beta, *, kind, group_size, n_domains, training_stats, eps, momentum, update_running,
         running, relu=False, residual=None):
    mode = nv.MODE_TRAIN if training_stats else nv.MODE_EVAL
    return _NormFunction.apply(x, gamma, beta, residual, kind, group_size, n_domains, mode, float(eps),
                               float(momentum), bool(update_running), running, bool(relu))


class _MecFunction(torch.autograd.Function):
    @staticmethod
    def forward(ctx, x, y):
        lib = nv.lib()
        if x.dim() != 2 or x.shape != y.shape:
            raise ValueError(f"expected two [N, K] logit tensors, got {tuple(x.shape)} and {tuple(y.shape)}")
        x, y = x.contiguous(), y.contiguous()
        dev = nv.require_cuda(x, y)
        loss = torch.empty((), dtype=torch.float32, device=dev)
        gx, gy = torch.empty_like(x), torch.empty_like(y)
        with torch.cuda.device(dev):
            rc = lib.dwt_mec_fwd_bwd(nv.ptr(x), nv.ptr(y), x.shape[0], x.shape[1], nv.ptr(loss), nv.ptr(gx),
                                     nv.ptr(gy), nv.stream_ptr(dev))
        nv.check(rc)
        ctx.save_for_backward(gx, gy)
        return loss

    @staticmethod
    def backward(ctx, g):
        gx, gy = ctx.saved_tensors
        return g * gx, g * gy


def mec_loss(x, y):
    return _MecFunction.apply(x, y)


class _HeadLossFunction(torch.autograd.Function):
    @staticmethod
    def forward(ctx, logits, labels, lam):
        lib = nv.lib()
        if logits.dim() != 2 or logits.shape[0] % 3 != 0 or labels.dim() != 1 or labels.shape[0] * 3 != logits.shape[0]:
            raise ValueError(f"expected logits [3B, K] and labels [B], got {tuple(logits.shape)} and {tuple(labels.shape)}")
        logits = logits.contiguous()
        dev = nv.require_cuda(logits)
        if not labels.is_cuda or labels.dtype != torch.int64:
            raise nv.NativeError("labels must be an int64 CUDA tensor")
        labels = labels.contiguous()
        losses = torch.empty(3, dtype=torch.float32, device=dev)
        grad = torch.empty_like(logits)
        with torch.cuda.device(dev):
            rc = lib.dwt_head_loss_fwd_bwd(nv.ptr(logits), nv.ptr(labels), labels.shape[0], logits.shape[1], float(lam),
                                           nv.ptr(losses), nv.ptr(grad), nv.status_ptr(dev), nv.stream_ptr(dev))
        nv.check(rc)
        nv.poll_status(dev)
        ctx.save_for_backward(grad)
        ctx.mark_non_differentiable(losses)
        return losses[0], losses

    @staticmethod
    def backward(ctx, g, _unused):
        (grad,) = ctx.saved_tensors
        return g * grad, None, None


def head_loss(logits, labels, lambda_mec):
    return _HeadLossFunction.apply(logits, labels, lambda_mec)
```

dwt-domain-adaptation_b200/dwt_b200/fused.py:

```python
from __future__ import annotations

import torch
import torch.nn as nn

from . import _native as nv
from . import functional as F


class DomainTripleNorm(nn.Module):
    def __init__(self, kind, num_features, group_size=4, n_domains=3):
        super().__init__()
        if kind not in ("whiten", "bn"):
            raise ValueError("kind must be 'whiten' or 'bn'")
        self.kind, self.num_features, self.n_domains = kind, num_features, n_domains
        self.group_size = min(num_features, group_size) if kind == "whiten" else 1
        self.kernel_epilogue = self.group_size in (1, 2, 4)

    def forward(self, x, domain_modules, gamma, beta, relu=False, residual=None, replicated=False, count_batches=True):
        mods = list(domain_modules)
        if len(mods) != self.n_domains:
            raise ValueError(f"expected {self.n_domains} domain modules")
        if x.dim() != 4:
            raise ValueError('expected 4D input (got {}D input)'.format(x.dim()))
        if replicated:
            return self._forward_replicated(x, mods, gamma, beta, relu, residual, count_batches)
        running, eps, momentum, update = self._running_args(mods, count_batches)
        if not self.kernel_epilogue:
            y = F.norm(x, None, None, kind=self.kind, group_size=self.group_size, n_domains=self.n_domains,
                       training_stats=True, eps=eps, momentum=momentum, update_running=update, running=running)
            return self._tensor_epilogue(y, gamma, beta, relu, residual)
        return F.norm(x, gamma, beta, kind=self.kind, group_size=self.group_size, n_domains=self.n_domains,
                      training_stats=True, eps=eps, momentum=momentum, update_running=update,
                      running=running, relu=relu, residual=residual)

    def _running_args(self, mods, count_batches):
        m0 = mods[0]
        if self.kind == "whiten":
            running = [(m.running_mean, m.running_variance) for m in mods]
            eps, momentum = m0.eps, m0.momentum
        else:
            if count_batches:
                counters = [m.num_batches_tracked for m in mods if m.training and m.track_running_stats]
                if counters:
                    torch._foreach_add_(counters, 1)
            running = [(m.running_mean, m.running_var) for m in mods]
            eps = m0.eps
            momentum = m0.momentum if m0.momentum is not None else 1.0 / m0.num_batches_tracked.item()
        return running, eps, momentum, m0.training and m0.track_running_stats

    def forward_with_downsample(self, x, domain_modules, gamma, beta, xd, down, down_modules, down_gamma, down_beta,
                                count_batches=True):
        mods, down_mods = list(domain_modules), list(down_modules)
        pair = (self.kernel_epilogue and down.kernel_epilogue and self.kind == down.kind
                and self.group_size == down.group_size and self.n_domains == down.n_domains
                and len(mods) == len(down_mods) == self.n_domains and x.dim() == 4 and x.shape == xd.shape
                and all(t.is_contiguous(memory_format=torch.channels_last) and not t.is_contiguous() for t in (x, xd))
                and nv.channels_last_supported(x.shape[1], self.group_size))
        if not pair:
            identity = down(xd, down_mods, down_gamma, down_beta, relu=False, count_batches=count_batches)
            return self(x, mods, gamma, beta, True, residual=identity, count_batches=count_batches)
        down_args = down._running_args(down_mods, count_batches)
        site_args = self._running_args(mods, count_batches)
        return F.tail_pair(x, xd, gamma, beta, down_gamma, down_beta, kind=self.kind, group_size=self.group_size,
                           n_domains=self.n_domains, sites=(site_args, down_args))

    @staticmethod
    def _tensor_epilogue(y, gamma, beta, relu, residual):
        if residual is not None and not relu:
            raise ValueError("a fused residual needs relu=True")
        if gamma is not None:
            y = y * gamma + beta
        if residual is not None:
            y = y + residual
        return torch.relu(y) if relu else y

    def _forward_replicated(self, x, mods, gamma, beta, relu, residual, count_batches=True):
        second = "running_variance" if self.kind == "whiten" else "running_var"
        keep = {}
        for m in mods:
            if not (m.training and m.track_running_stats):
                continue
            if self.kind == "bn":
                if count_batches:
                    m.num_batches_tracked += 1
                f = m.momentum if m.momentum is not None else 1.0 / m.num_batches_tracked.item()
            else:
                f = m.momentum
            rm, rv = m.running_mean, getattr(m, second)
            key = (rm.data_ptr(), rv.data_ptr())
            prod, _ = keep.get(key, (1.0, None))
            keep[key] = (prod * (1.0 - f), (rm, rv))
        means = {k[0] for k in keep}
        seconds = {k[1] for k in keep}
        if len(means) != len(keep) or len(seconds) != len(keep):
            raise ValueError("replicated statistics need each running_mean paired with one second-moment buffer")
        m0 = mods[0]
        common = dict(kind=self.kind, group_size=self.group_size, n_domains=1, training_stats=True, eps=m0.eps)
        if self.kernel_epilogue:
            common.update(relu=relu, residual=residual)
            g_arg, b_arg = gamma, beta
        else:
            g_arg = b_arg = None
        if not keep:
            out = F.norm(x, g_arg, b_arg, momentum=0.0, update_running=False,
                         running=[(m0.running_mean, getattr(m0, second))], **common)
        else:
            out = None
            for prod, pair in keep.values():
                y = F.norm(x, g_arg, b_arg, momentum=1.0 - prod, update_running=True, running=[pair], **common)
                out = y if out is None else out
        return out if self.kernel_epilogue else self._tensor_epilogue(out, gamma, beta, relu, residual)
```

harness/resnet50_dwt.py:

```python
from __future__ import annotations

import torch
import torch.nn as nn

_STAGES = ((64, 3, 1), (128, 4, 2), (256, 6, 2), (512, 3, 2))
_DOMAINS = ("s", "t", "t_aug")
EXPANSION = 4


_REPLICATED = [False]
_BATCHED_COUNTERS = [False]


class WhitenScaleShift(nn.Module):

    def __init__(self, layers, planes, group_size, running_mean, running_variance,
                 track_running_stats=True, affine=True):
        super().__init__()
        self.planes, self.group_size, self.affine = planes, group_size, affine
        self.wh = layers.WTransform2d(planes, group_size, running_m=running_mean,
                                      running_var=running_variance,
                                      track_running_stats=track_running_stats)
        if affine:
            self.gamma = nn.Parameter(torch.ones(planes, 1, 1))
            self.beta = nn.Parameter(torch.zeros(planes, 1, 1))

    def forward(self, x):
        y = self.wh(x)
        return y * self.gamma + self.beta if self.affine else y


class _SiteOwner(nn.Module):

    def _add_site(self, layers, tag, key, planes, whiten, group_size, stats, site_mode):
        pre, post = ("downsample_", "") if tag == "downsample" else ("", tag)
        names = [f"{pre}bn{d}{post}" if d != "t_aug" else f"{pre}bnt{post}_aug" for d in _DOMAINS]
        if whiten:
            rm, rv = stats[key + ".wh.running_mean"], stats[key + ".wh.running_variance"]
            gamma, beta = stats[key + ".gamma"], stats[key + ".beta"]
            mods = [WhitenScaleShift(layers, planes, group_size, rm, rv, affine=False) for _ in names]
        else:
            rm, rv = stats[key + ".running_mean"], stats[key + ".running_var"]
            gamma, beta = stats[key + ".weight"].view(-1, 1, 1), stats[key + ".bias"].view(-1, 1, 1)
            mods = [layers.BatchNorm2d(num_features=planes, running_m=rm, running_v=rv, affine=False)
                    for _ in names]
        for n, m in zip(names, mods):
            setattr(self, n, m)
        gname = f"{pre}gamma{post}" if pre == "" else "downsample_gamma"
        bname = f"{pre}beta{post}" if pre == "" else "downsample_beta"
        setattr(self, gname, nn.Parameter(gamma))
        setattr(self, bname, nn.Parameter(beta))
        if not hasattr(self, "_sites"):
            self._sites = {}
        self._sites[tag] = (names, gname, bname, whiten)
        if site_mode == "fused":
            object.__setattr__(self, f"_fused_{tag}", layers.DomainTripleNorm(
                kind="whiten" if whiten else "bn", num_features=planes,
                group_size=group_size if whiten else 1))

    def _site(self, tag, x, relu, residual=None):
        names, gname, bname, whiten = self._sites[tag]
        gamma, beta = getattr(self, gname), getattr(self, bname)
        if residual is not None:
            fused = getattr(self, f"_fused_{tag}", None) if self.training else None
            if fused is not None:
                mods = [getattr(self, n) for n in names]
                return fused(x, [m.wh if whiten else m for m in mods], gamma, beta, True, residual=residual,
                             replicated=_REPLICATED[0], count_batches=not _BATCHED_COUNTERS[0])
            return torch.relu_(self._site(tag, x, relu=False) + residual)
        if self.training:
            fused = getattr(self, f"_fused_{tag}", None)
            mods = [getattr(self, n) for n in names]
            if fused is not None:
                return fused(x, [m.wh if whiten else m for m in mods], gamma, beta, relu, replicated=_REPLICATED[0],
                             count_batches=not _BATCHED_COUNTERS[0])
            if _REPLICATED[0]:
                raise RuntimeError("replicated statistics collection needs site_mode='fused'")
            parts = torch.split(x, x.shape[0] // 3, dim=0)
            s, t, a = (m(p) for m, p in zip(mods, parts))
            out = torch.cat((s, torch.cat((t, a), dim=0)), dim=0) * gamma + beta
        else:
            out = getattr(self, names[1])(x) * gamma + beta
        return torch.relu_(out) if relu else out


class Bottleneck(_SiteOwner):
    def __init__(self, layers, inplanes, planes, layer, sub_layer, stats, group_size, stride,
                 downsample, site_mode):
        super().__init__()
        whiten = layer == 1
        key = f"layer{layer}.{sub_layer}"
        self.conv1 = nn.Conv2d(inplanes, planes, 1, bias=False)
        self._add_site(layers, "1", key + ".bn1", planes, whiten, group_size, stats, site_mode)
        self.conv2 = nn.Conv2d(planes, planes, 3, stride=stride, padding=1, bias=False)
        self._add_site(layers, "2", key + ".bn2", planes, whiten, group_size, stats, site_mode)
        self.conv3 = nn.Conv2d(planes, planes * EXPANSION, 1, bias=False)
        self._add_site(layers, "3", key + ".bn3", planes * EXPANSION, whiten, group_size, stats, site_mode)
        self.downsample = downsample
        if downsample is not None:
            self._add_site(layers, "downsample", f"layer{layer}.0.downsample_bn", planes * EXPANSION,
                           whiten, group_size, stats, site_mode)
        object.__setattr__(self, "_fork", getattr(layers, "fork_for_sum", None) if site_mode == "fused" else None)

    def forward(self, x):
        xa, xb = self._fork(x) if (self._fork is not None and self.training) else (x, x)
        out = self._site("1", self.conv1(xa), relu=True)
        out = self._site("2", self.conv2(out), relu=True)
        if self.downsample is None:
            return self._site("3", self.conv3(out), relu=True, residual=xb)
        tail = getattr(self, "_fused_3", None) if (self.training and not _REPLICATED[0]) else None
        if tail is None:
            identity = self._site("downsample", self.downsample(xb), relu=False)
            return self._site("3", self.conv3(out), relu=True, residual=identity)
        xd = self.downsample(xb)
        names, gname, bname, whiten = self._sites["3"]
        dnames, dgname, dbname, _ = self._sites["downsample"]
        unwrap = (lambda m: m.wh) if whiten else (lambda m: m)
        return tail.forward_with_downsample(
            self.conv3(out), [unwrap(getattr(self, n)) for n in names], getattr(self, gname), getattr(self, bname),
            xd, self._fused_downsample, [unwrap(getattr(self, n)) for n in dnames], getattr(self, dgname),
            getattr(self, dbname), count_batches=not _BATCHED_COUNTERS[0])


class ResNet50DWT(_SiteOwner):
    def __init__(self, layers, state_dict, num_classes=65, group_size=4, site_mode="modules", stem_pad=0, stem_nchw=False,
                 stem_s2d=False):
        super().__init__()
        self.stem_s2d = stem_s2d
        self.stem_nchw = stem_nchw
        self.stem_pad = stem_pad
        if site_mode not in ("modules", "fused"):
            raise ValueError("site_mode must be 'modules' or 'fused'")
        stats = {k: v for k, v in state_dict.items() if "bn" in k or "downsample" in k}
        self.site_mode = site_mode
        self.conv1 = nn.Conv2d(3, 64, 7, stride=2, padding=3, bias=False)
        self._add_site(layers, "1", "bn1", 64, True, group_size, stats, site_mode)
        self.maxpool = nn.MaxPool2d(3, stride=2, padding=1)
        inplanes = 64
        for li, (planes, blocks, stride) in enumerate(_STAGES, start=1):
            seq = []
            for b in range(blocks):
                down = None
                if b == 0 and (stride != 1 or inplanes != planes * EXPANSION):
                    down = nn.Sequential(nn.Conv2d(inplanes, planes * EXPANSION, 1, stride=stride, bias=False))
                seq.append(Bottleneck(layers, inplanes, planes, li, b, stats, 4, stride if b == 0 else 1,
                                      down, site_mode))
                inplanes = planes * EXPANSION
            setattr(self, f"layer{li}", nn.Sequential(*seq))
        self.avgpool = nn.AdaptiveAvgPool2d((1, 1))
        self.fc_out = nn.Linear(512 * EXPANSION, num_classes)
        for m in self.modules():
            if isinstance(m, nn.Conv2d):
                nn.init.kaiming_normal_(m.weight, mode="fan_out", nonlinearity="relu")

    def _stem_s2d(self, x):
        n, c, h, w = x.shape
        if h % 2 or w % 2:
            return self.conv1(x)
        cl = x.is_contiguous(memory_format=torch.channels_last) and not x.is_contiguous()
        xp = torch.nn.functional.pad(x, (3, 3, 3, 3))
        hp, wp = (h + 6) // 2, (w + 6) // 2
        wt = torch.nn.functional.pad(self.conv1.weight, (0, 1, 0, 1))
        o = wt.shape[0]
        if cl:
            xs = xp.view(n, c, hp, 2, wp, 2).permute(0, 2, 4, 1, 3, 5).reshape(n, hp, wp, 4 * c).permute(0, 3, 1, 2)
            w4 = wt.view(o, c, 4, 2, 4, 2).permute(0, 2, 4, 1, 3, 5).reshape(o, 4, 4, 4 * c).permute(0, 3, 1, 2)
        else:
            xs = xp.view(n, c, hp, 2, wp, 2).permute(0, 1, 3, 5, 2, 4).reshape(n, 4 * c, hp, wp)
            w4 = wt.view(o, c, 4, 2, 4, 2).permute(0, 1, 3, 5, 2, 4).reshape(o, 4 * c, 4, 4)
        return torch.nn.functional.conv2d(xs, w4)

    def _stem(self, x):
        if self.stem_s2d:
            return self._stem_s2d(x)
        if self.stem_nchw:
            return self.conv1(x.contiguous()).contiguous(memory_format=torch.channels_last)
        if not self.stem_pad or x.shape[1] >= self.stem_pad:
            return self.conv1(x)
        extra = self.stem_pad - x.shape[1]
        fmt = torch.channels_last if (x.is_contiguous(memory_format=torch.channels_last) and not x.is_contiguous()) \
            else torch.contiguous_format
        xp = torch.zeros((x.shape[0], self.stem_pad) + tuple(x.shape[2:]), dtype=x.dtype, device=x.device).contiguous(memory_format=fmt)
        xp[:, :x.shape[1]] = x
        w = torch.nn.functional.pad(self.conv1.weight, (0, 0, 0, 0, 0, extra))
        if fmt == torch.channels_last:
            w = w.contiguous(memory_format=torch.channels_last)
        c = self.conv1
        return torch.nn.functional.conv2d(xp, w, None, c.stride, c.padding, c.dilation, c.groups)

    def _bump_counters(self):
        cs = getattr(self, "_bn_counters", None)
        if cs is None:
            cs = [m.num_batches_tracked for m in self.modules()
                  if hasattr(m, "num_batches_tracked") and m.num_batches_tracked is not None and getattr(m, "track_running_stats", False)]
            object.__setattr__(self, "_bn_counters", cs)
        if cs:
            torch._foreach_add_(cs, 1)

    def forward(self, x):
        batched = self.training and self.site_mode == "fused"
        if batched:
            self._bump_counters()
        _BATCHED_COUNTERS[0] = batched
        try:
            x = self.maxpool(self._site("1", self._stem(x), relu=True))
            x = self.layer4(self.layer3(self.layer2(self.layer1(x))))
        finally:
            _BATCHED_COUNTERS[0] = False
        return self.fc_out(torch.flatten(self.avgpool(x), 1))


def build_resnet50_dwt(state_dict, layers, site_mode="modules", num_classes=65, channels_last=False, stem_pad=0,
                       stem_nchw=False, stem_s2d=False):
    model = ResNet50DWT(layers, state_dict, num_classes=num_classes, site_mode=site_mode, stem_pad=stem_pad,
                        stem_nchw=stem_nchw and channels_last, stem_s2d=stem_s2d)
    model.load_state_dict(state_dict, strict=False)
    if channels_last and hasattr(layers, "MaxPool2d"):
        model.maxpool = layers.MaxPool2d(3, stride=2, padding=1)
    if channels_last:
        for m in model.modules():
            if isinstance(m, nn.Conv2d) and not (model.stem_nchw and m is model.conv1):
                m.weight.data = m.weight.data.contiguous(memory_format=torch.channels_last)
    return model


def collect_stats(model, batches, passes=1, replicated=True):
    was_training = model.training
    model.train(True)
    out = None
    try:
        with torch.no_grad():
            for _ in range(passes):
                for data in batches:
                    if replicated:
                        _REPLICATED[0] = True
                        out = model(data)
                    else:
                        out = model(torch.cat((data, data, data), dim=0))
    finally:
        _REPLICATED[0] = False
        model.train(was_training)
    return out
```

include/dwt_b200.h:

```cpp
#ifndef DWT_B200_H_
#define DWT_B200_H_

#include <stddef.h>
#include <stdint.h>

#ifdef __cplusplus
extern "C" {
#endif

#define DWT_B200_ABI_VERSION 6
#define DWT_MAX_DOMAINS 4
#define DWT_MAX_GROUP_SIZE 64

#define DWT_OK 0
#define DWT_E_INVALID (-1)
#define DWT_E_WORKSPACE (-2)
#define DWT_E_LAUNCH (-3)
#define DWT_E_UNSUPPORTED (-4)

#define DWT_MODE_TRAIN 0
#define DWT_MODE_EVAL 1

#define DWT_LAYOUT_NHWC 0x100

#define DWT_EPI_NONE 0
#define DWT_EPI_AFFINE 1
#define DWT_EPI_RELU 2
#define DWT_EPI_RESIDUAL 4

typedef struct CUstream_st *dwt_stream_t;

#if defined(__GNUC__)
#define DWT_API __attribute__((visibility("default")))
#else
#define DWT_API
#endif

DWT_API int dwt_abi_version(void);
DWT_API const char *dwt_last_error(void);

DWT_API size_t dwt_workspace_bytes(int64_t N, int64_t C, int64_t HW, int group_size, int n_domains);

#define DWT_STATUS_NOT_PD 1
#define DWT_STATUS_BAD_LABEL 2

DWT_API int dwt_whiten_fwd(const float *x, float *y, int64_t N, int64_t C, int64_t HW, int group_size,
                   int n_domains, int mode, float eps, float momentum, int update_running,
                   float *const *running_mean, float *const *running_cov, const float *gamma,
                   const float *beta, const float *residual, uint8_t *relu_mask, int epilogue, float *save_mean,
                   float *save_w, void *workspace, size_t workspace_bytes, dwt_stream_t stream);

DWT_API int dwt_whiten_bwd(const float *x, const float *dout, const float *dout2, float *dx, int64_t N, int64_t C, int64_t HW,
                   int group_size, int n_domains, int mode, float eps, const float *save_mean,
                   const float *save_w, const float *gamma, const float *beta, const uint8_t *relu_mask,
                   float *dresidual, int epilogue, float *dgamma, float *dbeta, void *workspace,
                   size_t workspace_bytes, dwt_stream_t stream);

DWT_API int dwt_bn_fwd(const float *x, float *y, int64_t N, int64_t C, int64_t HW, int n_domains, int mode,
               float eps, float factor, int update_running, float *const *running_mean,
               float *const *running_var, const float *weight, const float *bias, const float *residual,
               uint8_t *relu_mask, int epilogue, float *save_mean, float *save_invstd, void *workspace,
               size_t workspace_bytes, dwt_stream_t stream);

DWT_API int dwt_bn_bwd(const float *x, const float *dout, const float *dout2, float *dx, int64_t N, int64_t C, int64_t HW,
               int n_domains, int mode, const float *save_mean, const float *save_invstd,
               const float *weight, const float *bias, const uint8_t *relu_mask, float *dresidual, int epilogue,
               float *dweight, float *dbias, void *workspace, size_t workspace_bytes, dwt_stream_t stream);

#define DWT_KIND_WHITEN 0
#define DWT_KIND_BN 1
typedef struct {
  const float *x;
  float eps, momentum;
  int update_running;
  float *const *running_mean;
  float *const *running_cov;
  const float *gamma, *beta;
  float *save_mean, *save_w;
  float *dx;
  float *dgamma, *dbeta;
} dwt_tail_site;

DWT_API int dwt_tail2_fwd(int kind, const dwt_tail_site *sites, float *y, uint8_t *relu_mask, int64_t N, int64_t C,
                  int64_t HW, int group_size, int n_domains, void *workspace, size_t workspace_bytes,
                  dwt_stream_t stream);
DWT_API int dwt_tail2_bwd(int kind, const dwt_tail_site *sites, const float *dout, const float *dout2,
                  const uint8_t *relu_mask, float *dz, int64_t N, int64_t C, int64_t HW, int group_size,
                  int n_domains, void *workspace, size_t workspace_bytes, dwt_stream_t stream);

DWT_API int dwt_mec_fwd_bwd(const float *x, const float *y, int64_t N, int64_t K, float *loss, float *gx,
                    float *gy, dwt_stream_t stream);

DWT_API int dwt_head_loss_fwd_bwd(const float *logits, const int64_t *labels, int64_t B, int64_t K, float lambda,
                          float *losses, float *grad, int *status, dwt_stream_t stream);

DWT_API int dwt_augment_pair(const uint8_t *images, int64_t B, int src_h, int src_w, int crop, const int32_t *crop_plain,
                     const int32_t *crop_aug, const uint8_t *flip, const float *affine, const float *mean,
                     const float *stdv, float *out_plain, float *out_aug, int layout, dwt_stream_t stream);

DWT_API int dwt_maxpool_fwd(const float *x, float *y, uint8_t *argmax, int64_t N, int64_t H, int64_t W, int64_t C,
                    int kernel, int stride, int padding, dwt_stream_t stream);
DWT_API int dwt_maxpool_bwd(const float *dy, const uint8_t *argmax, float *dx, int64_t N, int64_t H, int64_t W, int64_t C,
                    int kernel, int stride, int padding, dwt_stream_t stream);

typedef struct {
  char name[48];
  int64_t launches;
  double ms;
  double bytes;
} dwt_profile_entry;

DWT_API int64_t dwt_launch_count(void);
DWT_API void dwt_profile_begin(void);
DWT_API int dwt_profile_end(dwt_profile_entry *out, int max_entries);

#ifdef __cplusplus
}
#endif
#endif
```

Baseline: 3432.

## Fuse stem whitening/BN apply, ReLU and max-pool into one site-pool kernel

Adds a fused path for the stem normalization site: the forward apply kernel normalizes, applies ReLU and does the 3x3/s2 max-pool in one pass, writing only the pooled output plus a packed argmax map. The backward pass routes pooled gradients through the argmax directly inside the normalization backward reduce and apply kernels. This avoids materializing and re-reading the full-resolution post-ReLU activation and drops the separate pool kernels. In exchange, each pooled output recomputes the overlapping normalized inputs, and the path is restricted to specific shapes and channels-last layouts.

Result: faster. 3487 (median of 6 runs) (+1.6%).

```diff
diff --git a/dwt-domain-adaptation_b200/dwt_b200/_native.py b/dwt-domain-adaptation_b200/dwt_b200/_native.py
--- a/dwt-domain-adaptation_b200/dwt_b200/_native.py
+++ b/dwt-domain-adaptation_b200/dwt_b200/_native.py
@@ -9,7 +9,7 @@
 _HERE = os.path.dirname(os.path.abspath(__file__))
 LIB_PATH = os.environ.get("DWT_B200_LIB") or os.path.join(_HERE, "lib", "libdwt_b200.so")
 
-ABI_VERSION = 6
+ABI_VERSION = 7
 MAX_DOMAINS = 4
 MAX_GROUP_SIZE = 64
 MODE_TRAIN, MODE_EVAL = 0, 1
@@ -58,6 +58,12 @@
     "dwt_tail2_bwd": (ctypes.c_int, [ctypes.c_int, ctypes.POINTER(TailSite), _c_float_p, _c_float_p, ctypes.c_void_p,
                                      _c_float_p, ctypes.c_int64, ctypes.c_int64, ctypes.c_int64, ctypes.c_int, ctypes.c_int,
                                      ctypes.c_void_p, ctypes.c_size_t, ctypes.c_void_p]),
+    "dwt_site_pool_fwd": (ctypes.c_int, [ctypes.c_int, ctypes.POINTER(TailSite), _c_float_p, ctypes.c_void_p, ctypes.c_int64,
+                                         ctypes.c_int64, ctypes.c_int64, ctypes.c_int64, ctypes.c_int, ctypes.c_int, ctypes.c_int,
+                                         ctypes.c_int, ctypes.c_int, ctypes.c_void_p, ctypes.c_size_t, ctypes.c_void_p]),
+    "dwt_site_pool_bwd": (ctypes.c_int, [ctypes.c_int, ctypes.POINTER(TailSite), _c_float_p, _c_float_p, ctypes.c_void_p,
+                                         ctypes.c_int64, ctypes.c_int64, ctypes.c_int64, ctypes.c_int64, ctypes.c_int, ctypes.c_int,
+                                         ctypes.c_int, ctypes.c_int, ctypes.c_int, ctypes.c_void_p, ctypes.c_size_t, ctypes.c_void_p]),
     "dwt_mec_fwd_bwd": (ctypes.c_int, [_c_float_p, _c_float_p, ctypes.c_int64, ctypes.c_int64, _c_float_p,
                                        _c_float_p, _c_float_p, ctypes.c_void_p]),
     "dwt_head_loss_fwd_bwd": (ctypes.c_int, [_c_float_p, ctypes.c_void_p, ctypes.c_int64, ctypes.c_int64, ctypes.c_float,
@@ -139,6 +145,18 @@
     return c4 & (c4 - 1) == 0
 
 
+def site_pool_supported(n_all: int, channels: int, h: int, w: int, group_size: int, pool) -> bool:
+    def one(v):
+        return v if isinstance(v, int) else (v[0] if len(set(v)) == 1 else None)
+    k, s, p = (one(getattr(pool, a, None) or 0) for a in ("kernel_size", "stride", "padding"))
+    if (k, s, p) != (3, 2, 1) or getattr(pool, "ceil_mode", False) or one(getattr(pool, "dilation", 1)) != 1:
+        return False
+    if getattr(pool, "return_indices", False):
+        return False
+    return (channels_last_supported(channels, group_size) and h % 4 == 0 and w % 4 == 0
+            and n_all * (h // 2) <= 65535)
+
+
 def check(rc: int) -> None:
     if rc != 0:
         raise NativeError(f"libdwt_b200 error {rc}: {lib().dwt_last_error().decode()}")
diff --git a/dwt-domain-adaptation_b200/dwt_b200/csrc/api.cu b/dwt-domain-adaptation_b200/dwt_b200/csrc/api.cu
--- a/dwt-domain-adaptation_b200/dwt_b200/csrc/api.cu
+++ b/dwt-domain-adaptation_b200/dwt_b200/csrc/api.cu
@@ -586,6 +586,93 @@
   return check_launch("channels-last two-site backward apply kernel");
 }
 
+int site_pool_plan(Plan& p, int kind, const dwt_tail_site* s, const void* out, int64_t N, int64_t C, int64_t H, int64_t W, int GS,
+                   int D, int kernel, int stride, int padding) {
+  if (kind != DWT_KIND_WHITEN && kind != DWT_KIND_BN) return fail(DWT_E_INVALID, "bad kind %d", kind);
+  if (kind == DWT_KIND_BN && GS != 1) return fail(DWT_E_INVALID, "batch norm has group_size 1 (got %d)", GS);
+  if (!s || !s->x || !s->gamma || !s->beta || !s->save_mean || !s->save_w || !out) return fail(DWT_E_INVALID, "null pointer argument");
+  if (H <= 0 || W <= 0) return fail(DWT_E_INVALID, "bad image size %lldx%lld", (long long)H, (long long)W);
+  if (int rc = make_plan(p, K_STATS, K_APPLY, s->x, out, nullptr, N, C, H * W, GS, D)) return rc;
+  if (!dwt::cl_supports((int)C, GS))
+    return fail(DWT_E_UNSUPPORTED, "the pooled site runs on the channels-last kernels: group_size 1, 2, 4 with C/4 a power of two (C=%lld gs=%d)",
+                (long long)C, GS);
+  if (kernel != 3 || stride != 2 || padding != 1 || H % 4 != 0 || W % 4 != 0)
+    return fail(DWT_E_UNSUPPORTED, "the pooled site is built for a 3x3 / stride 2 / pad 1 max-pool of an image with H and W multiples of 4 "
+                "(got k=%d s=%d p=%d on %lldx%lld)", kernel, stride, padding, (long long)H, (long long)W);
+  if ((int64_t)D * N * (H / 4) > 65535 || (int64_t)D * N * (H / 2) > 65535)
+    return fail(DWT_E_UNSUPPORTED, "too many image rows for the pooled site's grid (%lld images of height %lld)", (long long)(D * N), (long long)H);
+  if ((((uintptr_t)s->x | (uintptr_t)out) % 16) != 0) return fail(DWT_E_INVALID, "channels-last tensors must be 16-byte aligned");
+  return DWT_OK;
+}
+
+int site_pool_fwd(int kind, const dwt_tail_site* s, float* pooled, uint8_t* argmax, int64_t N, int64_t C, int64_t H, int64_t W, int GS,
+                  int D, int kernel, int stride, int padding, void* ws, size_t ws_bytes, cudaStream_t st) {
+  Plan p;
+  if (int rc = site_pool_plan(p, kind, s, pooled, N, C, H, W, GS, D, kernel, stride, padding)) return rc;
+  if (!argmax || !ws) return fail(DWT_E_INVALID, "null pointer argument");
+  if ((uintptr_t)argmax % 4 != 0) return fail(DWT_E_INVALID, "the argmax map must be 4-byte aligned");
+  if (int rc = check_running(s->update_running != 0, s->running_mean, s->running_cov, D)) return rc;
+  Workspace w = carve(ws, C, GS, D);
+  if (w.bytes > ws_bytes) return fail(DWT_E_WORKSPACE, "workspace too small: need %zu bytes, got %zu", w.bytes, ws_bytes);
+  if ((uintptr_t)ws % 256 != 0) return fail(DWT_E_WORKSPACE, "workspace must be 256-byte aligned");
+  const SiteConst sc = site_const(kind, s->eps, N, H * W);
+  const dwt::FwdFin fin = make_fwd_fin(sc.a, sc.b, s->momentum, sc.unbias, s->update_running, s->update_running != 0, s->running_mean,
+                                       s->running_cov, s->save_mean, s->save_w, w, D);
+  const double E = 4.0 * (double)D * (double)N * (double)C * (double)(H * W);
+  const ClPlan cp = cl_plan(p.gm, 3, 3, 8, 8);
+  {
+    Launch l("cl_stats", &p.gm, E, st);
+    dwt::cl_stats(s->x, p.gm, cp.nred, cp.gz_red, w.partial, w.shift, st);
+  }
+  if (int rc = check_launch("channels-last statistics kernel")) return rc;
+  {
+    Launch l("cl_fwd_finalize", &p.gm, 0.0, st);
+    dwt::cl_fwd_finalize(w.partial, cp.nred, w.shift, p.gm, fin, st);
+  }
+  if (int rc = check_launch("channels-last finalize kernel")) return rc;
+  {
+    Launch l("cl_pool_apply", &p.gm, (1.0 + 0.25 + 0.0625) * E, st);
+    dwt::cl_pool_apply(s->x, pooled, argmax, p.gm, (int)H, (int)W, s->save_mean, s->save_w, s->gamma, s->beta, st);
+  }
+  return check_launch("channels-last pooled apply kernel");
+}
+
+int site_pool_bwd(int kind, const dwt_tail_site* s, const float* dpooled, const float* dpooled2, const uint8_t* argmax, int64_t N,
+                  int64_t C, int64_t H, int64_t W, int GS, int D, int kernel, int stride, int padding, void* ws, size_t ws_bytes,
+                  cudaStream_t st) {
+  Plan p;
+  if (int rc = site_pool_plan(p, kind, s, s ? s->dx : nullptr, N, C, H, W, GS, D, kernel, stride, padding)) return rc;
+  if (!dpooled || !argmax || !ws) return fail(DWT_E_INVALID, "null pointer argument");
+  if ((((uintptr_t)dpooled | (uintptr_t)dpooled2) % 16) != 0 || (uintptr_t)argmax % 4 != 0)
+    return fail(DWT_E_INVALID, "the pooled gradients must be 16-byte aligned, the argmax map 4-byte aligned");
+  if ((s->dgamma == nullptr) != (s->dbeta == nullptr)) return fail(DWT_E_INVALID, "dgamma and dbeta go together");
+  Workspace w = carve(ws, C, GS, D);
+  if (w.bytes > ws_bytes) return fail(DWT_E_WORKSPACE, "workspace too small: need %zu bytes, got %zu", w.bytes, ws_bytes);
+  if ((uintptr_t)ws % 256 != 0) return fail(DWT_E_WORKSPACE, "workspace must be 256-byte aligned");
+  const int epi = DWT_EPI_AFFINE | DWT_EPI_RELU;
+  const dwt::BwdFin fin = make_bwd_fin(site_const(kind, s->eps, N, H * W).a, DWT_MODE_TRAIN, epi, s->save_mean, s->save_w, s->gamma,
+                                       s->dgamma, s->dbeta, w);
+  const dwt::PoolGrad pg{dpooled, dpooled2, argmax, (int)W, (int)(H / 2), (int)(W / 2)};
+  const double E = 4.0 * (double)D * (double)N * (double)C * (double)(H * W);
+  const double gsrc = (dpooled2 ? 0.5 : 0.25) + 0.0625;
+  const ClPlan cp = cl_plan(p.gm, 2, 2, 4, 4);
+  {
+    Launch l("cl_pool_bwd_reduce", &p.gm, (1.0 + gsrc) * E, st);
+    dwt::cl_pool_bwd_reduce(s->x, pg, p.gm, cp.nred, cp.gz_red, s->save_mean, s->save_w, s->gamma, s->beta, w.partial, st);
+  }
+  if (int rc = check_launch("channels-last pooled backward reduction kernel")) return rc;
+  {
+    Launch l("cl_bwd_finalize", &p.gm, 0.0, st);
+    dwt::cl_bwd_finalize(w.partial, cp.nred, p.gm, fin, st);
+  }
+  if (int rc = check_launch("channels-last backward finalize kernel")) return rc;
+  {
+    Launch l("cl_pool_bwd_apply", &p.gm, (2.0 + gsrc) * E, st);
+    dwt::cl_pool_bwd_apply(s->x, pg, s->dx, p.gm, w.coef, s->save_mean, s->save_w, s->gamma, s->beta, st);
+  }
+  return check_launch("channels-last pooled backward apply kernel");
+}
+
 }
 
 extern "C" {
@@ -651,6 +738,20 @@
                   dwt_stream_t stream) {
   return tail2_bwd(kind, sites, dout, dout2, relu_mask, dz, N, C, HW, group_size, n_domains, workspace, workspace_bytes,
                    (cudaStream_t)stream);
+}
+
+int dwt_site_pool_fwd(int kind, const dwt_tail_site* site, float* pooled, uint8_t* argmax, int64_t N, int64_t C, int64_t H, int64_t W,
+                      int group_size, int n_domains, int kernel, int stride, int padding, void* workspace, size_t workspace_bytes,
+                      dwt_stream_t stream) {
+  return site_pool_fwd(kind, site, pooled, argmax, N, C, H, W, group_size, n_domains, kernel, stride, padding, workspace, workspace_bytes,
+                       (cudaStream_t)stream);
+}
+
+int dwt_site_pool_bwd(int kind, const dwt_tail_site* site, const float* dpooled, const float* dpooled2, const uint8_t* argmax, int64_t N,
+                      int64_t C, int64_t H, int64_t W, int group_size, int n_domains, int kernel, int stride, int padding, void* workspace,
+                      size_t workspace_bytes, dwt_stream_t stream) {
+  return site_pool_bwd(kind, site, dpooled, dpooled2, argmax, N, C, H, W, group_size, n_domains, kernel, stride, padding, workspace,
+                       workspace_bytes, (cudaStream_t)stream);
 }
 
 int dwt_mec_fwd_bwd(const float* x, const float* y, int64_t N, int64_t K, float* loss, float* gx, float* gy,
diff --git a/dwt-domain-adaptation_b200/dwt_b200/csrc/norm_cl.cu b/dwt-domain-adaptation_b200/dwt_b200/csrc/norm_cl.cu
--- a/dwt-domain-adaptation_b200/dwt_b200/csrc/norm_cl.cu
+++ b/dwt-domain-adaptation_b200/dwt_b200/csrc/norm_cl.cu
@@ -2,6 +2,7 @@
 
 #include "dwt_common.cuh"
 #include "norm_launch.h"
+#include "pool_rule.cuh"
 #include "small_algebra.cuh"
 
 namespace dwt {
@@ -328,6 +329,140 @@
 }
 
 template <int GS>
+__device__ __forceinline__ float4 site_relu(const float (&Wp)[4 / GS][GS * (GS + 1) / 2], const float (&bp)[4 / GS][GS], const float4& v) {
+  const float e[4] = {v.x, v.y, v.z, v.w};
+  float o[4];
+#pragma unroll
+  for (int s = 0; s < 4 / GS; ++s) {
+    float xi[GS], oi[GS];
+#pragma unroll
+    for (int c = 0; c < GS; ++c) xi[c] = e[s * GS + c];
+    apply_group<GS>(Wp[s], bp[s], xi, oi);
+#pragma unroll
+    for (int c = 0; c < GS; ++c) o[s * GS + c] = fmaxf(oi[c], 0.f);
+  }
+  return make_float4(o[0], o[1], o[2], o[3]);
+}
+
+template <int GS>
+__global__ void __launch_bounds__(256) cl_pool_apply_kernel(const float* __restrict__ x, float* __restrict__ y, uint8_t* __restrict__ idx,
+                                                            const Geom gm, int H, int W, int c4shift, const float* __restrict__ save_mean,
+                                                            const float* __restrict__ save_w, const float* __restrict__ gamma,
+                                                            const float* __restrict__ beta) {
+  using S = ClShape<GS>;
+  const int C4 = gm.C >> 2, OH = H >> 1, OW = W >> 1, OH2 = OH >> 1, OW2 = OW >> 1;
+  const int n = blockIdx.y / OH2, a = blockIdx.y - n * OH2;
+  const int i = blockIdx.x * blockDim.x + threadIdx.x;
+  pdl_wait();
+  if (i >= OW2 * C4) return;
+  const int b = i >> c4shift, q = i & (C4 - 1), d = n / gm.N;
+  float Wp[S::NSUB][S::NM], bp[S::NSUB][GS];
+#pragma unroll
+  for (int s = 0; s < S::NSUB; ++s) {
+    const int g = q * S::NSUB + s;
+    load_forward_map<GS, DWT_EPI_AFFINE | DWT_EPI_RELU>(save_w + ((size_t)d * gm.G + g) * GS * GS, save_mean + (size_t)d * gm.C + g * GS,
+                                                        gamma + g * GS, beta + g * GS, Wp[s], bp[s]);
+  }
+  const float4* xn = reinterpret_cast<const float4*>(x) + (size_t)n * H * W * C4 + q;
+  float best[2][2][4];
+  unsigned bi[2][2][4];
+#pragma unroll
+  for (int oa = 0; oa < 2; ++oa)
+#pragma unroll
+    for (int ob = 0; ob < 2; ++ob)
+#pragma unroll
+      for (int c = 0; c < 4; ++c) { best[oa][ob][c] = -INFINITY; bi[oa][ob][c] = 0u; }
+  const int h0 = 4 * a - 1, w0 = 4 * b - 1;
+#pragma unroll
+  for (int r = 0; r < 5; ++r) {
+    const int h = h0 + r;
+    if (h < 0 || h >= H) continue;
+    float4 row[5];
+    bool in[5];
+#pragma unroll
+    for (int cc = 0; cc < 5; ++cc) {
+      const int w = w0 + cc;
+      in[cc] = w >= 0 && w < W;
+      row[cc] = in[cc] ? __ldg(xn + ((size_t)h * W + w) * C4) : make_float4(0.f, 0.f, 0.f, 0.f);
+    }
+#pragma unroll
+    for (int cc = 0; cc < 5; ++cc) row[cc] = site_relu<GS>(Wp, bp, row[cc]);
+#pragma unroll
+    for (int oa = 0; oa < 2; ++oa) {
+      const int kh = r - 2 * oa;
+      if (kh < 0 || kh > 2) continue;
+#pragma unroll
+      for (int ob = 0; ob < 2; ++ob)
+#pragma unroll
+        for (int kw = 0; kw < 3; ++kw) {
+          const int cc = 2 * ob + kw;
+          if (!in[cc]) continue;
+          const float e[4] = {row[cc].x, row[cc].y, row[cc].z, row[cc].w};
+          const unsigned code = (unsigned)(kh * 3 + kw);
+#pragma unroll
+          for (int c = 0; c < 4; ++c)
+            if (takes(e[c], best[oa][ob][c])) { best[oa][ob][c] = e[c]; bi[oa][ob][c] = code; }
+        }
+    }
+  }
+#pragma unroll
+  for (int oa = 0; oa < 2; ++oa)
+#pragma unroll
+    for (int ob = 0; ob < 2; ++ob) {
+      const size_t o = (((size_t)n * OH + 2 * a + oa) * OW + 2 * b + ob) * C4 + q;
+      reinterpret_cast<float4*>(y)[o] = make_float4(best[oa][ob][0], best[oa][ob][1], best[oa][ob][2], best[oa][ob][3]);
+      reinterpret_cast<uint32_t*>(idx)[o] = bi[oa][ob][0] | (bi[oa][ob][1] << 8) | (bi[oa][ob][2] << 16) | (bi[oa][ob][3] << 24);
+    }
+}
+
+struct PoolPos {
+  unsigned n, h, w;
+  __device__ __forceinline__ void start(const PoolGrad& pg, const Geom& gm, int d, unsigned r) {
+    const unsigned ni = r / (unsigned)gm.HW, px = r - ni * (unsigned)gm.HW;
+    n = (unsigned)d * gm.N + ni;
+    h = px / (unsigned)pg.W;
+    w = px - h * (unsigned)pg.W;
+  }
+  __device__ __forceinline__ void advance(const PoolGrad& pg, unsigned step) {
+    w += step;
+    while (w >= (unsigned)pg.W) {
+      w -= pg.W;
+      if (++h == 2u * pg.OH) { h = 0; ++n; }
+    }
+  }
+};
+
+template <int PG>
+__device__ __forceinline__ float4 pooled_dout(const PoolGrad& pg, const PoolPos& pp, int C4, int q) {
+  const unsigned k = pp.h >> 1, j = pp.w >> 1;
+  const int oh = pp.h & 1, ow = pp.w & 1;
+  const unsigned o00 = ((pp.n * pg.OH + k) * pg.OW + j) * C4 + q;
+  const float4* dp = reinterpret_cast<const float4*>(pg.dp);
+  const float4* dp2 = reinterpret_cast<const float4*>(pg.dp2);
+  const uint32_t* ix = reinterpret_cast<const uint32_t*>(pg.idx);
+  float4 acc = make_float4(0.f, 0.f, 0.f, 0.f);
+#pragma unroll
+  for (int a = 0; a < 2; ++a)
+#pragma unroll
+    for (int b = 0; b < 2; ++b) {
+      const bool ok = (a == 0 || (oh && k + 1 < (unsigned)pg.OH)) && (b == 0 || (ow && j + 1 < (unsigned)pg.OW));
+      const unsigned o = o00 + (a ? pg.OW * C4 : 0) + (b ? C4 : 0);
+      uint32_t m = 0xFFFFFFFFu;
+      float4 g = make_float4(0.f, 0.f, 0.f, 0.f);
+      if (ok) {
+        m = __ldg(ix + o);
+        g = __ldg(dp + o);
+        if constexpr (PG == 2) {
+          const float4 g2 = __ldg(dp2 + o);
+          g.x += g2.x; g.y += g2.y; g.z += g2.z; g.w += g2.w;
+        }
+      }
+      take(acc, g, m, s2_code(oh, a, ow, b));
+    }
+  return acc;
+}
+
+template <int GS>
 __device__ __forceinline__ void bwd_accumulate(float* acc, const float (&dz)[GS], const float (&xi)[GS], const float* mu) {
 #pragma unroll
   for (int i = 0; i < GS; ++i) {
@@ -337,19 +472,20 @@
   }
 }
 
-template <int GS, int EPI, bool D2, bool DS>
+template <int GS, int EPI, bool D2, bool DS, int PG>
 __global__ void __launch_bounds__(kT, 2) cl_bwd_reduce_kernel(const float* __restrict__ x, const float* __restrict__ dout, const float* __restrict__ dout2,
                                                               const Geom gm, const float* __restrict__ save_mean,
                                                               const float* __restrict__ save_w, const float* __restrict__ gamma,
                                                               const float* __restrict__ beta, const uint8_t* __restrict__ mask,
                                                               float* __restrict__ dzout, float* __restrict__ partial,
                                                               const float* __restrict__ xds, const float* __restrict__ save_mean_d,
-                                                              size_t pstride) {
+                                                              size_t pstride, const PoolGrad pg) {
   using S = ClShape<GS>;
   constexpr int UNROLL = 4;
   constexpr bool MASK = (EPI & DWT_EPI_RESIDUAL) != 0;
   constexpr bool RELU = (EPI & DWT_EPI_RELU) != 0 && !MASK;
   static_assert(!DS || MASK, "the two-site tail is a residual epilogue");
+  static_assert(PG == 0 || (RELU && !D2 && !DS), "the pooled site is AFFINE|RELU with its own second addend");
   constexpr int NS = DS ? 2 : 1;
   __shared__ float sRed[kT * S::BWD];
   const ClThread t(gm);
@@ -389,13 +525,16 @@
       const unsigned r = r0 + h * t.rpi;
       float4 v[NS][H], q[H], q2[D2 ? H : 1];
       unsigned mb[H];
+      PoolPos pp;
+      if constexpr (PG != 0) pp.start(pg, gm, d, r);
 #pragma unroll
       for (int u = 0; u < H; ++u) {
         const unsigned rr = r + u * t.rpi;
         if (rr < rows) {
 #pragma unroll
           for (int k = 0; k < NS; ++k) v[k][u] = ldg4(xp[k] + (size_t)rr * gm.C);
-          q[u] = ldg4(gd + (size_t)rr * gm.C);
+          if constexpr (PG != 0) q[u] = pooled_dout<PG>(pg, pp, t.C4, t.q);
+          else q[u] = ldg4(gd + (size_t)rr * gm.C);
           if constexpr (MASK) mb[u] = __ldg(md + (size_t)rr * t.C4);
           if constexpr (D2) q2[u] = ldg4(gd2 + (size_t)rr * gm.C);
         } else {
@@ -405,6 +544,7 @@
           if constexpr (MASK) mb[u] = 0u;
           if constexpr (D2) q2[u] = make_float4(0.f, 0.f, 0.f, 0.f);
         }
+        if constexpr (PG != 0) pp.advance(pg, t.rpi);
       }
       if constexpr (D2) {
 #pragma unroll
@@ -611,6 +751,81 @@
   }
 }
 
+template <int GS, int PG>
+__global__ void __launch_bounds__(256) cl_pool_bwd_apply_kernel(const float* __restrict__ x, const PoolGrad pg, float* __restrict__ dx,
+                                                                const Geom gm, int c4shift, const float* __restrict__ coef,
+                                                                const float* __restrict__ save_mean, const float* __restrict__ save_w,
+                                                                const float* __restrict__ gamma, const float* __restrict__ beta) {
+  using S = ClShape<GS>;
+  const int C4 = gm.C >> 2, OH = pg.OH, OW = pg.OW, W = pg.W;
+  const int n = blockIdx.y / OH, k = blockIdx.y - n * OH;
+  const int i = blockIdx.x * blockDim.x + threadIdx.x;
+  pdl_wait();
+  if (i >= OW * C4) return;
+  const int j = i >> c4shift, q = i & (C4 - 1), d = n / gm.N;
+  float Wp[S::NSUB][S::NM], bp[S::NSUB][GS];
+  BwdCoef<GS> cf[S::NSUB];
+#pragma unroll
+  for (int s = 0; s < S::NSUB; ++s) {
+    const int g = q * S::NSUB + s;
+    load_forward_map<GS, DWT_EPI_AFFINE | DWT_EPI_RELU>(save_w + ((size_t)d * gm.G + g) * GS * GS, save_mean + (size_t)d * gm.C + g * GS,
+                                                        gamma + g * GS, beta + g * GS, Wp[s], bp[s]);
+    cf[s].load(coef + ((size_t)d * gm.G + g) * coef_stride(GS));
+  }
+  const float4* dp = reinterpret_cast<const float4*>(pg.dp);
+  const float4* dp2 = reinterpret_cast<const float4*>(pg.dp2);
+  const uint32_t* ix = reinterpret_cast<const uint32_t*>(pg.idx);
+  uint32_t m[2][2];
+  float4 gq[2][2];
+#pragma unroll
+  for (int a = 0; a < 2; ++a)
+#pragma unroll
+    for (int b = 0; b < 2; ++b) {
+      const bool ok = (k + a < OH) && (j + b < OW);
+      const size_t o = (((size_t)n * OH + k + a) * OW + j + b) * C4 + q;
+      m[a][b] = ok ? __ldg(ix + o) : 0xFFFFFFFFu;
+      gq[a][b] = ok ? __ldg(dp + o) : make_float4(0.f, 0.f, 0.f, 0.f);
+      if constexpr (PG == 2) {
+        if (ok) {
+          const float4 g2 = __ldg(dp2 + o);
+          gq[a][b].x += g2.x; gq[a][b].y += g2.y; gq[a][b].z += g2.z; gq[a][b].w += g2.w;
+        }
+      }
+    }
+  const size_t p00 = (((size_t)n * 2 * OH + 2 * k) * W + 2 * j) * C4 + q;
+  const float4* xq = reinterpret_cast<const float4*>(x);
+  float4* dq = reinterpret_cast<float4*>(dx);
+  float4 xv[2][2];
+#pragma unroll
+  for (int pa = 0; pa < 2; ++pa)
+#pragma unroll
+    for (int pb = 0; pb < 2; ++pb) xv[pa][pb] = __ldg(xq + p00 + ((size_t)pa * W + pb) * C4);
+#pragma unroll
+  for (int pa = 0; pa < 2; ++pa)
+#pragma unroll
+    for (int pb = 0; pb < 2; ++pb) {
+      float4 acc = make_float4(0.f, 0.f, 0.f, 0.f);
+#pragma unroll
+      for (int a = 0; a <= pa; ++a)
+#pragma unroll
+        for (int b = 0; b <= pb; ++b) take(acc, gq[a][b], m[a][b], s2_code(pa, a, pb, b));
+      const float ge[4] = {acc.x, acc.y, acc.z, acc.w};
+      const float e[4] = {xv[pa][pb].x, xv[pa][pb].y, xv[pa][pb].z, xv[pa][pb].w};
+      float o[4];
+#pragma unroll
+      for (int s = 0; s < S::NSUB; ++s) {
+        float xi[GS], dz[GS], oi[GS];
+#pragma unroll
+        for (int c = 0; c < GS; ++c) { xi[c] = e[s * GS + c]; dz[c] = ge[s * GS + c]; }
+        apply_group<GS>(Wp[s], bp[s], xi, oi);
+#pragma unroll
+        for (int c = 0; c < GS; ++c) dz[c] = oi[c] > 0.f ? dz[c] : 0.f;
+        cf[s].apply(dz, xi, o + s * GS);
+      }
+      dq[p00 + ((size_t)pa * W + pb) * C4] = make_float4(o[0], o[1], o[2], o[3]);
+    }
+}
+
 #define CL_GS(GS_, ...)                                  \
   switch (GS_) {                                         \
     case 1: { constexpr int kGS = 1; __VA_ARGS__; break; } \
@@ -628,6 +843,9 @@
 #define CL_D2(P_, ...)                                                    \
   if (P_) { constexpr bool kD2 = true; __VA_ARGS__; }                     \
   else { constexpr bool kD2 = false; __VA_ARGS__; }
+#define CL_PG(P_, ...)                                                    \
+  if (P_) { constexpr int kPG = 2; __VA_ARGS__; }                         \
+  else { constexpr int kPG = 1; __VA_ARGS__; }
 
 inline bool use_pdl() {
   static const bool on = [] { const char* v = getenv("DWT_PDL"); return v != nullptr && v[0] == '1'; }();
@@ -690,15 +908,15 @@
 void cl_bwd_reduce(const float* x, const float* dout, const float* dout2, const Geom& gm, int nctas, int gz, int epi, const float* mean, const float* w,
                    const float* gamma, const float* beta, const uint8_t* mask, float* dz, float* partial, cudaStream_t st) {
   const float* nul = nullptr;
-  CL_GS(gm.GS, CL_D2(dout2, CL_EPI_BWD(epi, (cl_bwd_reduce_kernel<kGS, kEPI, kD2, false><<<cl_grid(gm, nctas, gz), kT, 0, st>>>(
-                                                x, dout, dout2, gm, mean, w, gamma, beta, mask, dz, partial, nul, nul, 0)))));
+  CL_GS(gm.GS, CL_D2(dout2, CL_EPI_BWD(epi, (cl_bwd_reduce_kernel<kGS, kEPI, kD2, false, 0><<<cl_grid(gm, nctas, gz), kT, 0, st>>>(
+                                                x, dout, dout2, gm, mean, w, gamma, beta, mask, dz, partial, nul, nul, 0, PoolGrad{})))));
 }
 void cl_tail2_bwd_reduce(const float* x, const float* xd, const float* dout, const float* dout2, const Geom& gm, int nctas, int gz,
                          const float* mean, const float* mean_d, const uint8_t* mask, float* dz, float* partial, size_t pstride,
                          cudaStream_t st) {
   const float* nul = nullptr;
-  CL_GS(gm.GS, CL_D2(dout2, (cl_bwd_reduce_kernel<kGS, 7, kD2, true><<<cl_grid(gm, nctas, gz), kT, 0, st>>>(
-                                x, dout, dout2, gm, mean, nul, nul, nul, mask, dz, partial, xd, mean_d, pstride))));
+  CL_GS(gm.GS, CL_D2(dout2, (cl_bwd_reduce_kernel<kGS, 7, kD2, true, 0><<<cl_grid(gm, nctas, gz), kT, 0, st>>>(
+                                x, dout, dout2, gm, mean, nul, nul, nul, mask, dz, partial, xd, mean_d, pstride, PoolGrad{}))));
 }
 void cl_bwd_finalize(const float* partial, int nrows, const Geom& gm, const BwdFin& fin, cudaStream_t st, const BwdFin* fin2, size_t pstride) {
   const dim3 b = fin_block(gm), g((gm.C / 4) / b.y, fin2 ? 2 : 1);
@@ -716,5 +934,28 @@
   CL_GS(gm.GS, (launch_k(cl_bwd_apply_kernel<kGS, 1, false, true>, cl_grid(gm, nctas, gz), dim3(kT), st, use_pdl(), x, dz, nul, dx, gm, coef,
                          nul, nul, nul, nul, xd, dxd, coef_d)));
 }
-
-}
+void cl_pool_apply(const float* x, float* pooled, uint8_t* idx, const Geom& gm, int H, int W, const float* mean, const float* w,
+                   const float* gamma, const float* beta, cudaStream_t st) {
+  const int C4 = gm.C / 4, items = (W / 4) * C4, threads = items >= 256 ? 256 : ((items + 31) / 32) * 32;
+  int c4shift = 0;
+  while ((1 << c4shift) < C4) ++c4shift;
+  const dim3 grid((items + threads - 1) / threads, gm.D * gm.N * (H / 4));
+  CL_GS(gm.GS, (launch_k(cl_pool_apply_kernel<kGS>, grid, dim3(threads), st, use_pdl(), x, pooled, idx, gm, H, W, c4shift, mean, w, gamma, beta)));
+}
+void cl_pool_bwd_reduce(const float* x, const PoolGrad& pg, const Geom& gm, int nctas, int gz, const float* mean, const float* w,
+                        const float* gamma, const float* beta, float* partial, cudaStream_t st) {
+  const float* nul = nullptr;
+  CL_GS(gm.GS, CL_PG(pg.dp2, (cl_bwd_reduce_kernel<kGS, 3, false, false, kPG><<<cl_grid(gm, nctas, gz), kT, 0, st>>>(
+                                x, nul, nul, gm, mean, w, gamma, beta, (const uint8_t*)nullptr, (float*)nullptr, partial, nul, nul, 0, pg))));
+}
+void cl_pool_bwd_apply(const float* x, const PoolGrad& pg, float* dx, const Geom& gm, const float* coef, const float* mean,
+                       const float* w, const float* gamma, const float* beta, cudaStream_t st) {
+  const int C4 = gm.C / 4, items = pg.OW * C4, threads = items >= 256 ? 256 : ((items + 31) / 32) * 32;
+  int c4shift = 0;
+  while ((1 << c4shift) < C4) ++c4shift;
+  const dim3 grid((items + threads - 1) / threads, gm.D * gm.N * pg.OH);
+  CL_GS(gm.GS, CL_PG(pg.dp2, (launch_k(cl_pool_bwd_apply_kernel<kGS, kPG>, grid, dim3(threads), st, use_pdl(), x, pg, dx, gm, c4shift, coef,
+                                       mean, w, gamma, beta))));
+}
+
+}
diff --git a/dwt-domain-adaptation_b200/dwt_b200/csrc/norm_launch.h b/dwt-domain-adaptation_b200/dwt_b200/csrc/norm_launch.h
--- a/dwt-domain-adaptation_b200/dwt_b200/csrc/norm_launch.h
+++ b/dwt-domain-adaptation_b200/dwt_b200/csrc/norm_launch.h
@@ -76,6 +76,18 @@
                          cudaStream_t st);
 void cl_tail2_bwd_apply(const float* x, const float* xd, const float* dz, float* dx, float* dxd, const Geom& gm, int nctas, int gz,
                         const float* coef, const float* coef_d, cudaStream_t st);
+struct PoolGrad {
+  const float* dp;
+  const float* dp2;
+  const uint8_t* idx;
+  int W, OH, OW;
+};
+void cl_pool_apply(const float* x, float* pooled, uint8_t* idx, const Geom& gm, int H, int W, const float* mean, const float* w,
+                   const float* gamma, const float* beta, cudaStream_t st);
+void cl_pool_bwd_reduce(const float* x, const PoolGrad& pg, const Geom& gm, int nctas, int gz, const float* mean, const float* w,
+                        const float* gamma, const float* beta, float* partial, cudaStream_t st);
+void cl_pool_bwd_apply(const float* x, const PoolGrad& pg, float* dx, const Geom& gm, const float* coef, const float* mean,
+                       const float* w, const float* gamma, const float* beta, cudaStream_t st);
 
 void maxpool_fwd_launch(const float* x, float* y, uint8_t* idx, int N, int H, int W, int C, int OH, int OW, int k, int s, int p,
                         cudaStream_t st);
diff --git a/dwt-domain-adaptation_b200/dwt_b200/csrc/pool.cu b/dwt-domain-adaptation_b200/dwt_b200/csrc/pool.cu
--- a/dwt-domain-adaptation_b200/dwt_b200/csrc/pool.cu
+++ b/dwt-domain-adaptation_b200/dwt_b200/csrc/pool.cu
@@ -1,5 +1,6 @@
 #include "dwt_common.cuh"
 #include "norm_launch.h"
+#include "pool_rule.cuh"
 
 namespace dwt {
 namespace {
@@ -13,8 +14,6 @@
   if constexpr (K > 0) { g.k = K; g.s = S; g.p = P; }
   return g;
 }
-
-__device__ __forceinline__ bool takes(float v, float best) { return (v > best) || (v != v); }
 
 template <int K, int S, int P, bool POW2>
 __global__ void __launch_bounds__(256) maxpool_fwd_kernel(const float* __restrict__ x, float* __restrict__ y,
@@ -147,13 +146,6 @@
     }
 }
 
-__device__ __forceinline__ void take(float4& acc, const float4& gq, uint32_t m, unsigned code) {
-  if ((m & 0xFFu) == code) acc.x += gq.x;
-  if (((m >> 8) & 0xFFu) == code) acc.y += gq.y;
-  if (((m >> 16) & 0xFFu) == code) acc.z += gq.z;
-  if ((m >> 24) == code) acc.w += gq.w;
-}
-
 __global__ void __launch_bounds__(256) maxpool_bwd_3s2_kernel(const float* __restrict__ dy, const uint8_t* __restrict__ idx,
                                                               float* __restrict__ dx, const PoolGeom g) {
   const int H2 = g.H >> 1, W2 = g.W >> 1;
@@ -175,10 +167,11 @@
       gq[a][b] = ok ? __ldg(dyn + o) : make_float4(0.f, 0.f, 0.f, 0.f);
     }
   float4 o00 = make_float4(0.f, 0.f, 0.f, 0.f), o01 = o00, o10 = o00, o11 = o00;
-  take(o00, gq[0][0], m[0][0], 4u);
-  take(o01, gq[0][0], m[0][0], 5u); take(o01, gq[0][1], m[0][1], 3u);
-  take(o10, gq[0][0], m[0][0], 7u); take(o10, gq[1][0], m[1][0], 1u);
-  take(o11, gq[0][0], m[0][0], 8u); take(o11, gq[0][1], m[0][1], 6u); take(o11, gq[1][0], m[1][0], 2u); take(o11, gq[1][1], m[1][1], 0u);
+  take(o00, gq[0][0], m[0][0], s2_code(0, 0, 0, 0));
+  take(o01, gq[0][0], m[0][0], s2_code(0, 0, 1, 0)); take(o01, gq[0][1], m[0][1], s2_code(0, 0, 1, 1));
+  take(o10, gq[0][0], m[0][0], s2_code(1, 0, 0, 0)); take(o10, gq[1][0], m[1][0], s2_code(1, 1, 0, 0));
+  take(o11, gq[0][0], m[0][0], s2_code(1, 0, 1, 0)); take(o11, gq[0][1], m[0][1], s2_code(1, 0, 1, 1));
+  take(o11, gq[1][0], m[1][0], s2_code(1, 1, 1, 0)); take(o11, gq[1][1], m[1][1], s2_code(1, 1, 1, 1));
   float4* r0 = reinterpret_cast<float4*>(dx) + (((size_t)n * g.H + 2 * k) * g.W + 2 * j) * g.C4 + c4;
   float4* r1 = r0 + (size_t)g.W * g.C4;
   r0[0] = o00; r0[g.C4] = o01;
diff --git a/dwt-domain-adaptation_b200/dwt_b200/csrc/pool_rule.cuh b/dwt-domain-adaptation_b200/dwt_b200/csrc/pool_rule.cuh
--- /dev/null
+++ b/dwt-domain-adaptation_b200/dwt_b200/csrc/pool_rule.cuh
@@ -0,0 +1,18 @@
+#pragma once
+#include <stdint.h>
+
+namespace dwt {
+
+__device__ __forceinline__ bool takes(float v, float best) { return (v > best) || (v != v); }
+
+__host__ __device__ constexpr unsigned s2_tap(int odd, int a) { return odd ? (a ? 0u : 2u) : 1u; }
+__host__ __device__ constexpr unsigned s2_code(int odd_h, int a, int odd_w, int b) { return s2_tap(odd_h, a) * 3u + s2_tap(odd_w, b); }
+
+__device__ __forceinline__ void take(float4& acc, const float4& gq, uint32_t m, unsigned code) {
+  if ((m & 0xFFu) == code) acc.x += gq.x;
+  if (((m >> 8) & 0xFFu) == code) acc.y += gq.y;
+  if (((m >> 16) & 0xFFu) == code) acc.z += gq.z;
+  if ((m >> 24) == code) acc.w += gq.w;
+}
+
+}
diff --git a/dwt-domain-adaptation_b200/dwt_b200/functional.py b/dwt-domain-adaptation_b200/dwt_b200/functional.py
--- a/dwt-domain-adaptation_b200/dwt_b200/functional.py
+++ b/dwt-domain-adaptation_b200/dwt_b200/functional.py
@@ -1,4 +1,6 @@
 from __future__ import annotations
+
+import ctypes
 
 import torch
 
@@ -227,6 +229,78 @@
                                    [(r, float(e), float(m), bool(u)) for r, e, m, u in sites])
 
 
+class _SitePoolFunction(torch.autograd.Function):
+
+    @staticmethod
+    def forward(ctx, x, gamma, beta, kind, group_size, n_domains, site):
+        lib = nv.lib()
+        gs = group_size if kind == "whiten" else 1
+        n_all, c, h, w = x.shape
+        if n_all % n_domains != 0:
+            raise ValueError(f"batch of {n_all} does not split into {n_domains} domains")
+        n = n_all // n_domains
+        running, eps, momentum, update = site
+        dev = nv.require_cuda(x, gamma, beta, *[t for pair in running for t in pair])
+        for d, (rm_t, rv_t) in enumerate(running):
+            _check_param(f"running mean of domain {d}", rm_t, c)
+            _check_param(f"running second moment of domain {d}", rv_t, c * gs)
+        _check_param("gamma / weight", gamma, c)
+        _check_param("beta / bias", beta, c)
+        g_c, b_c = gamma.detach().reshape(-1).contiguous(), beta.detach().reshape(-1).contiguous()
+        save_mean = torch.empty(n_domains, c, dtype=torch.float32, device=dev)
+        save_w = torch.empty(n_domains, c // gs, gs, gs, dtype=torch.float32, device=dev)
+        rm = nv.ptr_array([pr[0] for pr in running]) if update else None
+        rv = nv.ptr_array([pr[1] for pr in running]) if update else None
+        c_site = nv.TailSite(x.data_ptr(), eps, momentum, int(update), rm, rv, g_c.data_ptr(), b_c.data_ptr(), save_mean.data_ptr(),
+                             save_w.data_ptr(), None, None, None)
+        oh, ow = h // 2, w // 2
+        pooled = torch.empty((n_all, c, oh, ow), dtype=torch.float32, device=dev, memory_format=torch.channels_last)
+        argmax = torch.empty(n_all * oh * ow * c, dtype=torch.uint8, device=dev)
+        ws = nv.workspace(dev, n, c, h * w, gs, n_domains)
+        nv_kind = nv.KIND_WHITEN if kind == "whiten" else nv.KIND_BN
+        with torch.cuda.device(dev):
+            rc = lib.dwt_site_pool_fwd(nv_kind, ctypes.byref(c_site), nv.ptr(pooled), nv.ptr(argmax), n, c, h, w, gs, n_domains,
+                                       3, 2, 1, nv.ptr(ws), ws.numel(), nv.stream_ptr(dev))
+        nv.check(rc)
+        nv.poll_status(dev)
+        if update:
+            seen = set()
+            for buf in (t for pair in running for t in pair):
+                if id(buf) not in seen:
+                    seen.add(id(buf))
+                    torch.autograd.graph.increment_version(buf)
+        ctx.save_for_backward(x, save_mean, save_w, g_c, b_c, argmax)
+        ctx.cfg = (nv_kind, gs, n_domains, n, c, h, w, float(eps), gamma.shape, beta.shape)
+        return pooled
+
+    @staticmethod
+    def backward(ctx, dpooled):
+        lib = nv.lib()
+        x, save_mean, save_w, g_c, b_c, argmax = ctx.saved_tensors
+        nv_kind, gs, n_domains, n, c, h, w, eps, gshape, bshape = ctx.cfg
+        dp2 = ctx.__dict__.pop("_dwt_extra_grad", None)
+        if dp2 is not None and not (dp2.shape == dpooled.shape and dp2.dtype == torch.float32
+                                    and dp2.is_contiguous(memory_format=torch.channels_last)):
+            dpooled, dp2 = dpooled + dp2, None
+        dpooled = dpooled.contiguous(memory_format=torch.channels_last)
+        dev = nv.require_cuda(dpooled)
+        dx = torch.empty_like(x)
+        grads = torch.empty(2, c, dtype=torch.float32, device=dev)
+        c_site = nv.TailSite(x.data_ptr(), eps, 0.0, 0, None, None, g_c.data_ptr(), b_c.data_ptr(), save_mean.data_ptr(),
+                             save_w.data_ptr(), dx.data_ptr(), grads[0].data_ptr(), grads[1].data_ptr())
+        ws = nv.workspace(dev, n, c, h * w, gs, n_domains)
+        with torch.cuda.device(dev):
+            rc = lib.dwt_site_pool_bwd(nv_kind, ctypes.byref(c_site), nv.ptr(dpooled), nv.ptr(dp2), nv.ptr(argmax), n, c, h, w, gs,
+                                       n_domains, 3, 2, 1, nv.ptr(ws), ws.numel(), nv.stream_ptr(dev))
+        nv.check(rc)
+        return (dx, grads[0].view(gshape), grads[1].view(bshape)) + (None,) * 4
+
+
+def site_pool(x, gamma, beta, *, kind, group_size, n_domains, site):
+    running, eps, momentum, update = site
+    return _SitePoolFunction.apply(x, gamma, beta, kind, group_size, n_domains, (running, float(eps), float(momentum), bool(update)))
+
+
 class _ForkForSum(torch.autograd.Function):
 
     @staticmethod
@@ -247,7 +321,8 @@
 
 def fork_for_sum(y):
     fn = getattr(y, "grad_fn", None)
-    if not torch.is_grad_enabled() or fn is None or not isinstance(fn, (_NormFunction._backward_cls, _TailPairFunction._backward_cls)):
+    if not torch.is_grad_enabled() or fn is None or not isinstance(fn, (_NormFunction._backward_cls, _TailPairFunction._backward_cls,
+                                                                                _SitePoolFunction._backward_cls)):
         return y, y
     return _ForkForSum.apply(y)
 
diff --git a/dwt-domain-adaptation_b200/dwt_b200/fused.py b/dwt-domain-adaptation_b200/dwt_b200/fused.py
--- a/dwt-domain-adaptation_b200/dwt_b200/fused.py
+++ b/dwt-domain-adaptation_b200/dwt_b200/fused.py
@@ -64,6 +64,17 @@
         return F.tail_pair(x, xd, gamma, beta, down_gamma, down_beta, kind=self.kind, group_size=self.group_size,
                            n_domains=self.n_domains, sites=(site_args, down_args))
 
+    def forward_with_maxpool(self, x, domain_modules, gamma, beta, pool, count_batches=True):
+        mods = list(domain_modules)
+        fused = (self.kernel_epilogue and len(mods) == self.n_domains and x.dim() == 4 and x.dtype == torch.float32
+                 and x.is_contiguous(memory_format=torch.channels_last) and not x.is_contiguous()
+                 and x.data_ptr() % 16 == 0 and x.shape[0] % self.n_domains == 0
+                 and nv.site_pool_supported(x.shape[0], x.shape[1], x.shape[2], x.shape[3], self.group_size, pool))
+        if not fused:
+            return pool(self(x, mods, gamma, beta, relu=True, count_batches=count_batches))
+        return F.site_pool(x, gamma, beta, kind=self.kind, group_size=self.group_size, n_domains=self.n_domains,
+                           site=self._running_args(mods, count_batches))
+
     @staticmethod
     def _tensor_epilogue(y, gamma, beta, relu, residual):
         if residual is not None and not relu:
diff --git a/harness/resnet50_dwt.py b/harness/resnet50_dwt.py
--- a/harness/resnet50_dwt.py
+++ b/harness/resnet50_dwt.py
@@ -136,6 +136,7 @@
         self.conv1 = nn.Conv2d(3, 64, 7, stride=2, padding=3, bias=False)
         self._add_site(layers, "1", "bn1", 64, True, group_size, stats, site_mode)
         self.maxpool = nn.MaxPool2d(3, stride=2, padding=1)
+        object.__setattr__(self, "_pool_cls", getattr(layers, "MaxPool2d", None))
         inplanes = 64
         for li, (planes, blocks, stride) in enumerate(_STAGES, start=1):
             seq = []
@@ -203,7 +204,14 @@
             self._bump_counters()
         _BATCHED_COUNTERS[0] = batched
         try:
-            x = self.maxpool(self._site("1", self._stem(x), relu=True))
+            stem = getattr(self, "_fused_1", None) if (self.training and not _REPLICATED[0]) else None
+            if stem is not None and self._pool_cls is not None and type(self.maxpool) is self._pool_cls:
+                names, gname, bname, whiten = self._sites["1"]
+                mods = [getattr(self, n).wh if whiten else getattr(self, n) for n in names]
+                x = stem.forward_with_maxpool(self._stem(x), mods, getattr(self, gname),
+                                              getattr(self, bname), self.maxpool, count_batches=not _BATCHED_COUNTERS[0])
+            else:
+                x = self.maxpool(self._site("1", self._stem(x), relu=True))
             x = self.layer4(self.layer3(self.layer2(self.layer1(x))))
         finally:
             _BATCHED_COUNTERS[0] = False
diff --git a/include/dwt_b200.h b/include/dwt_b200.h
--- a/include/dwt_b200.h
+++ b/include/dwt_b200.h
@@ -8,7 +8,7 @@
 extern "C" {
 #endif
 
-#define DWT_B200_ABI_VERSION 6
+#define DWT_B200_ABI_VERSION 7
 #define DWT_MAX_DOMAINS 4
 #define DWT_MAX_GROUP_SIZE 64
 
@@ -88,6 +88,13 @@
                   const uint8_t *relu_mask, float *dz, int64_t N, int64_t C, int64_t HW, int group_size,
                   int n_domains, void *workspace, size_t workspace_bytes, dwt_stream_t stream);
 
+DWT_API int dwt_site_pool_fwd(int kind, const dwt_tail_site *site, float *pooled, uint8_t *argmax, int64_t N, int64_t C, int64_t H,
+                      int64_t W, int group_size, int n_domains, int kernel, int stride, int padding, void *workspace,
+                      size_t workspace_bytes, dwt_stream_t stream);
+DWT_API int dwt_site_pool_bwd(int kind, const dwt_tail_site *site, const float *dpooled, const float *dpooled2,
+                      const uint8_t *argmax, int64_t N, int64_t C, int64_t H, int64_t W, int group_size, int n_domains,
+                      int kernel, int stride, int padding, void *workspace, size_t workspace_bytes, dwt_stream_t stream);
+
 DWT_API int dwt_mec_fwd_bwd(const float *x, const float *y, int64_t N, int64_t K, float *loss, float *gx,
                     float *gy, dwt_stream_t stream);
 
```
